# google-deepmind/meltingpot

Measured on NVIDIA B200. Metric: env_steps_per_sec, higher is better.
Workload: dtype u8

## Files before the change

### include/mp_engine.h

```cpp
#ifndef MP_ENGINE_H_
#define MP_ENGINE_H_

#include <stddef.h>
#include <stdint.h>

#ifdef __cplusplus
extern "C" {
#endif

typedef struct mp_engine* mp_handle;

enum {
  MP_OK = 0,
  MP_E_INVALID = -1,
  MP_E_UNSUPPORTED = -2,
  MP_E_CUDA = -3,
  MP_E_NO_DEVICE = -4
};

enum {
  MP_FLAG_RENDER_WORLD = 1u << 0,
  MP_FLAG_RENDER_PLAYERS = 1u << 1,
  MP_FLAG_DEFAULT = 3u,
  MP_FLAG_DEBUG_NO_COMPOSE = 1u << 4,
  MP_FLAG_DEBUG_NO_STORE = 1u << 5,
  MP_FLAG_DEBUG_REUSE_RECORDS = 1u << 6,
  MP_FLAG_DEBUG_NO_FENCE = 1u << 7,
  MP_FLAG_DEBUG_TOP_SPRITE_ONLY = 1u << 8,
  MP_FLAG_DEBUG_PLAIN_LANE_MAP = 1u << 9,
  MP_FLAG_DEBUG_SCATTER_LANE_MAP = 1u << 10
};

typedef struct mp_buffers {
  int32_t num_envs, num_players;
  int32_t rgb_h, rgb_w;
  int32_t world_h, world_w;
  int32_t num_actions;
  int32_t num_scalar_obs;
  uint8_t* rgb;
  uint8_t* world_rgb;
  double* reward;
  double* discount;
  int64_t* step_type;
  double* scalar_obs;
  int32_t* avatar_state;
  uint16_t* grid;
  int32_t grid_layers, grid_cells, grid_cells_padded;
  double* timestep_packed;
  int32_t* events;
  int32_t* event_count;
  int32_t max_events;
  void* scalar_block;
  uint64_t scalar_block_bytes;
  double* gathered;
  int32_t gathered_world;
  uint8_t* gathered_rgb;
  uint8_t* gathered_world_rgb;
  uint64_t gathered_obs_slot_bytes;
} mp_buffers;

int mp_create(const void* blob, size_t blob_bytes, int num_envs, int device, uint64_t seed,
              uint64_t env_index_base, uint32_t flags, mp_handle* out);

int mp_destroy(mp_handle h);

int mp_set_flags(mp_handle h, uint32_t flags);

int mp_reset(mp_handle h, const uint8_t* env_mask, void* stream);

int mp_step(mp_handle h, const int32_t* actions, void* stream);

int mp_step_state(mp_handle h, const int32_t* actions, void* stream);
int mp_render(mp_handle h, void* stream);

int mp_get_buffers(mp_handle h, mp_buffers* out);

typedef struct mp_host_outputs {
  uint8_t* rgb;
  uint8_t* world_rgb;
  double* reward;
  double* discount;
  int64_t* step_type;
  double* scalar_obs;
  void* scalar_block;
  int32_t* events;
  int32_t* event_count;
} mp_host_outputs;
int mp_step_host(mp_handle h, const int32_t* actions_host, const mp_host_outputs* out, void* stream);
int mp_reset_host(mp_handle h, const mp_host_outputs* out, void* stream);

int mp_step_host_async(mp_handle h, const int32_t* actions_host, const mp_host_outputs* out, int slot, void* stream);
int mp_wait(mp_handle h, int slot);

int mp_exchange_create(mp_handle h, int rank, int world, void** block, uint64_t* block_bytes);
int mp_ipc_export(const void* device_ptr, void* handle64, uint64_t* offset);
int mp_ipc_open(int device, const void* handle64, uint64_t offset, void** device_ptr);
int mp_enable_peer_access(int device, int peer_device);
int mp_exchange_connect(mp_handle h, void* const* peer_blocks);
int mp_exchange_wait(mp_handle h, void* stream);
int mp_exchange_slot(mp_handle h, int* slot, uint64_t* step);

int mp_gather_obs_create(mp_handle h, int rank, int world, void** block, uint64_t* block_bytes);
int mp_gather_obs_connect(mp_handle h, void* const* peer_blocks);
int mp_gather_obs_enable(mp_handle h, int on);
int mp_gather_obs_wait(mp_handle h, void* stream);
int mp_gather_obs_slot(mp_handle h, int* slot, uint64_t* step);

int mp_launch_count(mp_handle h, uint64_t* out);

int mp_algorithmic_bytes(mp_handle h, uint64_t* per_env_step, uint64_t* render_per_env_step);

int mp_state_size(mp_handle h, uint64_t* bytes);
int mp_state_save(mp_handle h, void* host_dst, void* stream);
int mp_state_load(mp_handle h, const void* host_src, uint64_t nbytes, void* stream);

int mp_debug_render_plan(mp_handle h, int32_t out[8]);

int mp_debug_render_tables(mp_handle h, int32_t* n_total, uint8_t* pair, uint8_t* flags);

int mp_debug_observations(mp_handle h, int32_t* position, int32_t* orientation, int32_t* layer, int32_t* zap_matrix, void* stream);

int mp_debug_lane_map(int n_rows, int n_cells, int pitch_slots, int iters, int scattered, uint32_t out[32]);

const char* mp_last_error(void);
const char* mp_version(void);

#ifdef __cplusplus
}
#endif
#endif
```

### meltingpot_b200/csrc/common.cuh

```cuda
#pragma once

#include <cuda_runtime.h>
#include <stdint.h>

#define MP_MAX_PLAYERS 16
#define MP_MAX_LAYERS 16
#define MP_MAX_BEAM_CELLS 32
#define MP_FULL 0xffffffffu
#define MP_MAX_PEERS 8

enum { ENV_STEP = 0, ENV_EPISODE = 1, ENV_DONE = 2, ENV_DIRT = 3, ENV_CLEANED = 4, ENV_ATE = 5, ENV_BEAM = 6, ENV_COLS = 8 };
enum { AV_X = 0, AV_Y = 1, AV_ORIENT = 2, AV_ALIVE = 3 };
enum { TM_ZAP = 0, TM_BEAM2 = 1, TM_FRAME = 2 };
enum { RS_SCENE = 0, RS_AVATAR = 1, RS_OBJECT = 2, RS_AVATAR_RESET = 3, RS_OBJECT_RESET = 4, RS_CHOICE = 5 };
enum { SCENE_DRAW_DIRT = 0, SCENE_DRAW_EPISODE_END = 1 };

struct BeamGeom {
  int n;
  int depth;
  int8_t lat[MP_MAX_BEAM_CELLS];
  int8_t fwd[MP_MAX_BEAM_CELLS];
  int8_t parent[MP_MAX_BEAM_CELLS];
};

struct Tables {
  int W, H, cells, cells_pad, L, P, topology, max_frames;
  int view_l, view_r, view_f, view_b, n_sprites, oob_sprite, oov_sprite, n_actions, n_scalar;
  int scalar_obs[4];
  int avatar_layer, n_spawn;
  int avatar_sprite[MP_MAX_PLAYERS];
  int zap_cooldown, zap_respawn, zap_remove, zap_layer, zap_sprite, zap_hit;
  double zap_penalty, zap_reward;
  BeamGeom zap_geom;
  int nA, nD, nW, nA_pad, nD_pad, nW_pad;
  int apple_layer, apple_sprite, dirt_layer, dirt_sprite, water_layer, n_anim, anim_frames, anim_random;
  int water_sprite[8];
  int clean_cooldown, clean_layer, clean_sprite, clean_hit;
  BeamGeom clean_geom;
  int dirt_delay, end_min_frames, end_interval, taste_role, dirt_count0;
  double grow_rate, grow_depletion, grow_restoration, eat_reward, dirt_prob, end_prob, taste_amount;
  int wait_layer, wait_sprite, grass_layer, grass_sprite, dess_sprite, ch_n_wait, ch_n_probs;
  double ch_probs[4];
  int n_spawn_init[2];
  int avatar_init_group[MP_MAX_PLAYERS];
  const int32_t* spawn_init_cell[2];
  const int32_t* ch_apple;
  int nR, nR_pad, res_layer, unclaimed_sprite, tex_layer, tex_sprite, ind_layer, dmg_layer, dmg_sprite, mark_layer;
  int mark_initial_level, mark_recovery, mark_n_levels, mark_inc[3], mark_remove[3], mark_freeze[3], mark_sprite[3];
  double mark_src_reward[3], mark_tgt_reward[3];
  int claim_wait, brush_layer, claim_layer, res_health0, res_reward_delay, res_repair_delay, tr_taste_role;
  double res_reward, res_rate, res_repair_prob, tr_taste_amount, tr_taste_mult;
  int claimed_sprite[MP_MAX_PLAYERS], dry_sprite[MP_MAX_PLAYERS], brush_sprite[MP_MAX_PLAYERS], claimbeam_sprite[MP_MAX_PLAYERS];
  BeamGeom claim_geom, brush_geom;
  const int32_t* tr_res;
  const int16_t* res_of_cell;
  const uint8_t* wall;
  int n_choice;
  const int32_t* choice_n;
  const int32_t* spawn_cond;
  const int32_t* tr_res_cond;
  const int32_t* ch_nbr;
  const uint16_t* init_grid;
  const int32_t* action_table;
  const int32_t* apple;
  const int32_t* dirt;
  const int32_t* water;
  const int32_t* spawn_cell;
  const uint8_t* solid;
  const uint8_t* cell_flags;
  const int16_t* apple_of_cell;
  const int16_t* dirt_of_cell;
  const uint8_t* atlas;
  const int16_t* sprite_map;
  const uint8_t* sprite_opaque;
  const uint8_t* sprite_pair;
  int coin_sprite[2];
  int coin_type[2];
  double coin_reward[2][4];
  double coin_rate;
  int coin_terminate, coin_terminate_n;
  int ore_sprite[4];
  int mine_window, mine_length;
  double mine_rate[2];
  double mine_reward[2], extract_reward[2];
};

struct State {
  int B;
  uint64_t seed;
  uint16_t* grid;
  int32_t* avatar;
  int32_t* av_timer;
  uint8_t* apple;
  uint8_t* dirt;
  uint8_t* water;
  uint8_t* apple_count;
  uint8_t* fam_u8;
  uint16_t* fam_u16;
  int32_t* av_extra;
  int fam_u8_stride, fam_u16_stride;
  int32_t* env;
  double* reward;
  double* discount;
  int64_t* step_type;
  double* scalar_obs;
  double* packed;
  uint8_t* rgb;
  uint8_t* world_rgb;
  int32_t* events;
  int32_t* n_events;
  int max_events;
  int x_world, x_rank;
  unsigned long long x_step;
  double* x_gathered[MP_MAX_PEERS];
  unsigned long long* x_flags[MP_MAX_PEERS];
  int x_raise;
  int g_world;
  unsigned long long g_step;
  uint8_t* g_rgb[MP_MAX_PEERS];
  uint8_t* g_wrgb[MP_MAX_PEERS];
  const unsigned long long* g_flags;
};

#define MP_MIN_EVENTS 64
enum { EV_ZAP = 1, EV_EDIBLE_CONSUMED = 2, EV_PLAYER_CLEANED = 3, EV_CLAIMED_RESOURCE = 4, EV_DESTROYED_RESOURCE = 5,
       EV_SANCTIONING = 6, EV_REMOVAL = 7, EV_COIN_CONSUMED = 8 ,
       EV_MINING = 9 , EV_EXTRACTION = 10 ,
       EV_EXTRACTION_PAIR = 11  };

__device__ __forceinline__ int* event_counter() {
  __shared__ int s_event_count[4];
  return &s_event_count[(threadIdx.x >> 5) & 3];
}
__device__ __forceinline__ void event_begin(int lane) {
  if (lane == 0) *event_counter() = 0;
  __syncwarp();
}
__device__ __forceinline__ void emit_event(const State& S, int b, int type, int a0, int a1) {
  const int i = atomicAdd(event_counter(), 1);
  if (i < S.max_events) {
    int32_t* e = S.events + ((size_t)b * S.max_events + i) * 3;
    e[0] = type; e[1] = a0; e[2] = a1;
  }
}
__device__ __forceinline__ void event_end(const State& S, int b, int lane) {
  __syncwarp();
  if (lane == 0) S.n_events[b] = *event_counter();
}

__device__ __forceinline__ uint4 philox4x32_10(uint32_t c0, uint32_t c1, uint32_t c2, uint32_t c3, uint32_t k0, uint32_t k1) {
#pragma unroll
  for (int r = 0; r < 10; ++r) {
    uint32_t h0 = __umulhi(0xD2511F53u, c0), l0 = 0xD2511F53u * c0;
    uint32_t h1 = __umulhi(0xCD9E8D57u, c2), l1 = 0xCD9E8D57u * c2;
    uint32_t n0 = h1 ^ c1 ^ k0, n2 = h0 ^ c3 ^ k1;
    c0 = n0; c1 = l1; c2 = n2; c3 = l0;
    k0 += 0x9E3779B9u; k1 += 0xBB67AE85u;
  }
  return make_uint4(c0, c1, c2, c3);
}

__device__ __forceinline__ double u01(uint32_t a, uint32_t b) {
  return ((double)(a >> 5) * 67108864.0 + (double)(b >> 6)) / 9007199254740992.0;
}
__device__ __forceinline__ uint32_t pick(uint32_t w, uint32_t n) { return __umulhi(w, n); }

__device__ __forceinline__ bool choice_present(const Tables& T, int group, uint32_t mask, int episode, uint32_t k0, uint32_t k1) {
  if (group < 0) return true;
  const uint4 w = philox4x32_10(0u, (uint32_t)episode, (uint32_t)group, RS_CHOICE, k0, k1);
  return (mask >> pick(w.x, (uint32_t)T.choice_n[group])) & 1u;
}

__device__ __forceinline__ int dir_dx(int d) { return (d == 1) - (d == 3); }
__device__ __forceinline__ int dir_dy(int d) { return (d == 2) - (d == 0); }
__device__ __forceinline__ uint16_t cell_value(int sprite, int orient) { return (uint16_t)(1 + sprite * 4 + (orient & 3)); }

__device__ __forceinline__ bool wrap_or_reject(const Tables& T, int& x, int& y) {
  if (T.topology == 1) {
    x += x < 0 ? T.W : (x >= T.W ? -T.W : 0);
    y += y < 0 ? T.H : (y >= T.H ? -T.H : 0);
    return true;
  }
  return x >= 0 && x < T.W && y >= 0 && y < T.H;
}

__device__ __forceinline__ void exchange_push(const Tables& T, const State& S) {
  if (S.x_world == 0) return;
  const int lane = threadIdx.x & 31, warp = threadIdx.x >> 5, n_warps = (int)blockDim.x >> 5;
  if (blockIdx.x == 0 && threadIdx.x < S.x_world)
    asm volatile("st.relaxed.sys.global.u64 [%0], %1;" ::"l"(S.x_flags[threadIdx.x] + MP_MAX_PEERS + S.x_rank), "l"(S.x_step) : "memory");
  if (lane < S.x_world && S.x_step > 1ull) {
    const volatile unsigned long long* f = S.x_flags[S.x_rank] + MP_MAX_PEERS + lane;
    while (*f + 1ull < S.x_step) __nanosleep(100);
  }
  __syncwarp();
  const int n = T.P + 2;
  const size_t base = ((size_t)(S.x_step & 1ull) * S.x_world + (size_t)S.x_rank) * S.B;
  for (int b = (int)blockIdx.x + warp * (int)gridDim.x; b < S.B; b += n_warps * (int)gridDim.x) {
    if (lane < n) {
      const double v = S.packed[(size_t)b * n + lane];
      for (int r = 0; r < S.x_world; ++r) S.x_gathered[r][(base + b) * n + lane] = v;
    }
  }
}

__global__ void __launch_bounds__(256) k_exchange_push(Tables T, State S) {
  asm volatile("griddepcontrol.wait;" ::: "memory");
  exchange_push(T, S);
}

__global__ void __launch_bounds__(32) k_exchange_wait(State S, unsigned long long step) {
  const int lane = threadIdx.x;
  if (lane < S.x_world) {
    asm volatile("st.relaxed.sys.global.u64 [%0], %1;" ::"l"(S.x_flags[lane] + S.x_rank), "l"(step) : "memory");
    const unsigned long long* mine = S.x_flags[S.x_rank] + lane;
    unsigned long long v;
    do {
      asm volatile("ld.acquire.sys.global.u64 %0, [%1];" : "=l"(v) : "l"(mine) : "memory");
      if (v < step) __nanosleep(200);
    } while (v < step);
  }
}

__global__ void __launch_bounds__(32) k_flag_wait(const unsigned long long* flags, int world, unsigned long long step) {
  const int lane = threadIdx.x;
  if (lane < world) {
    unsigned long long v;
    do {
      asm volatile("ld.acquire.sys.global.u64 %0, [%1];" : "=l"(v) : "l"(flags + lane) : "memory");
      if (v < step) __nanosleep(200);
    } while (v < step);
  }
}

__global__ void __launch_bounds__(32) k_gather_raise(unsigned long long* const* flags, int world, int rank, unsigned long long step) {
  if (threadIdx.x < world) {
    __threadfence_system();
    asm volatile("st.release.sys.global.u64 [%0], %1;" ::"l"(flags[threadIdx.x] + rank), "l"(step) : "memory");
  }
}
```

### meltingpot_b200/csrc/engine.cu

```cuda
#include <cuda_runtime.h>

#include <algorithm>
#include <cstdarg>
#include <cstdio>
#include <cstring>
#include <string>
#include <vector>

#include "../../include/mp_engine.h"
#include "../../include/mpb_format.h"
#include "common.cuh"
#include "render.cuh"
#include "step_clean_up.cuh"
#include "step_commons.cuh"
#include "step_territory.cuh"
#include "step_coins.cuh"
#include "step_mining.cuh"

namespace {

thread_local std::string g_error;

int fail(int code, const char* fmt, ...) {
  char buf[512];
  va_list ap;
  va_start(ap, fmt);
  vsnprintf(buf, sizeof buf, fmt, ap);
  va_end(ap);
  g_error = buf;
  return code;
}

#define CUDA_TRY(expr)                                                                          \
  do {                                                                                          \
    cudaError_t e_ = (expr);                                                                    \
    if (e_ != cudaSuccess) return fail(MP_E_CUDA, "%s failed: %s", #expr, cudaGetErrorString(e_)); \
  } while (0)

template <typename T>
struct Section {
  const T* data = nullptr;
  std::vector<uint32_t> shape;
  size_t count = 0;
};

template <typename T>
bool get_section(const void* blob, size_t n, const char* name, int dtype, Section<T>* out) {
  const MpbSection* s = mpb_find(blob, n, name);
  if (!s || (int)s->dtype != dtype) return false;
  out->data = static_cast<const T*>(mpb_data(blob, s));
  out->shape.assign(s->shape, s->shape + s->ndim);
  out->count = s->nbytes / sizeof(T);
  return true;
}

int round_up(int v, int m) { return (v + m - 1) / m * m; }

constexpr int kRenderSmemLimit = 227 * 1024 - 2560;
constexpr int kMaxAtlasSprites = 96;
#define MP_MAX_DEVICES 64
#define MP_EXCHANGE_HEADER 256

bool make_beam_geom(int length, int radius, BeamGeom* g) {
  std::vector<int> lat, fwd, parent;
  int prev = -1;
  for (int i = 1; i <= length; ++i) { lat.push_back(0); fwd.push_back(i); parent.push_back(prev); prev = (int)lat.size() - 1; }
  for (int side = 0; side < 2; ++side) {
    int sign = side == 0 ? -1 : 1;
    int prev_lat = -1;
    for (int k = 1; k <= radius; ++k) {
      lat.push_back(sign * k); fwd.push_back(0); parent.push_back(prev_lat);
      prev_lat = (int)lat.size() - 1;
      int pf = prev_lat;
      for (int i = 1; i <= length - k; ++i) { lat.push_back(sign * k); fwd.push_back(i); parent.push_back(pf); pf = (int)lat.size() - 1; }
    }
  }
  if (lat.size() > MP_MAX_BEAM_CELLS) return false;
  g->n = (int)lat.size();
  g->depth = length + radius;
  for (int i = 0; i < g->n; ++i) { g->lat[i] = (int8_t)lat[i]; g->fwd[i] = (int8_t)fwd[i]; g->parent[i] = (int8_t)parent[i]; }
  return true;
}

bool make_lane_map(int n_rows, int n_cells, int pitch_slots, int iters, uint32_t out[32]) {
  const int cap = 16 / n_rows, nH = 2 * iters;
  struct Edge { int u, v, cell, col; };
  std::vector<Edge> edges;
  int cnt[16] = {};
  for (int j = 0; j < n_rows; ++j)
    for (int c = 0; c < n_cells; ++c) {
      const int r = (pitch_slots * j + 3 * c) & 15;
      edges.push_back({j * cap + c % cap, r, c, -1});
      if (++cnt[r] > nH) return false;
    }
  if (n_cells > cap * nH || iters * 6 > 32) return false;
  const int nL = n_rows * cap;
  std::vector<int> colL((size_t)nL * nH, -1), colR((size_t)16 * nH, -1);
  auto free_col = [&](const std::vector<int>& tab, int v) { for (int a = 0; a < nH; ++a) if (tab[(size_t)v * nH + a] < 0) return a; return -1; };
  for (int ei = 0; ei < (int)edges.size(); ++ei) {
    Edge& e = edges[ei];
    const int a = free_col(colL, e.u), b = free_col(colR, e.v);
    if (a < 0 || b < 0) return false;
    if (a != b) {
      std::vector<int> path;
      int cur = e.v, want = a; bool right = true;
      for (;;) {
        const int pe = right ? colR[(size_t)cur * nH + want] : colL[(size_t)cur * nH + want];
        if (pe < 0) break;
        path.push_back(pe);
        cur = right ? edges[pe].u : edges[pe].v;
        right = !right;
        want = want == a ? b : a;
      }
      for (int pe : path) { colL[(size_t)edges[pe].u * nH + edges[pe].col] = -1; colR[(size_t)edges[pe].v * nH + edges[pe].col] = -1; }
      for (int pe : path) { edges[pe].col = edges[pe].col == a ? b : a; colL[(size_t)edges[pe].u * nH + edges[pe].col] = pe; colR[(size_t)edges[pe].v * nH + edges[pe].col] = pe; }
    }
    e.col = a;
    colL[(size_t)e.u * nH + a] = ei; colR[(size_t)e.v * nH + a] = ei;
  }
  for (int l = 0; l < 32; ++l) { out[l] = 0; for (int i = 0; i < iters; ++i) out[l] |= 63u << (6 * i); }
  for (const Edge& e : edges) {
    const int j = e.u / cap, sub = e.u % cap, it = e.col / 2, half = e.col % 2;
    const int lane = 16 * half + sub * n_rows + j;
    out[lane] = (out[lane] & ~(63u << (6 * it))) | ((uint32_t)e.cell << (6 * it));
  }
  return true;
}

int make_lane_map_cells(int n_rows, int n_cells, int pitch_slots, int iters, uint32_t out[32]) {
  const int G = 32 / n_rows, n_slots = G * iters, per_half = 16 / n_rows;
  std::vector<int> slot(n_slots, -1);
  for (int c = 0; c < n_cells && c < n_slots; ++c) slot[c] = c;
  auto cost = [&]() {
    int total = 0;
    for (int it = 0; it < iters; ++it)
      for (int h = 0; h < 2; ++h) {
        int cnt[16] = {}, mx = 0;
        for (int g = h * per_half; g < (h + 1) * per_half; ++g) {
          const int c = slot[it * G + g];
          if (c < 0) continue;
          for (int j = 0; j < n_rows; ++j) mx = std::max(mx, ++cnt[(pitch_slots * j + 3 * c) & 15]);
        }
        total += mx > 1 ? mx - 1 : 0;
      }
    return total;
  };
  int best = cost();
  for (bool improved = true; improved && best > 0;) {
    improved = false;
    int bi = -1, bj = -1, bc = best;
    for (int i = 0; i < n_slots; ++i)
      for (int j = i + 1; j < n_slots; ++j) {
        if (slot[i] == slot[j]) continue;
        std::swap(slot[i], slot[j]);
        const int c = cost();
        if (c < bc) { bc = c; bi = i; bj = j; }
        std::swap(slot[i], slot[j]);
      }
    if (bi >= 0) { std::swap(slot[bi], slot[bj]); best = bc; improved = true; }
  }
  for (int l = 0; l < 32; ++l) {
    out[l] = 0;
    for (int it = 0; it < 5; ++it) {
      const int c = it < iters ? slot[it * G + l / n_rows] : -1;
      out[l] |= (uint32_t)(c < 0 ? 63 : c) << (6 * it);
    }
  }
  return best;
}

}

struct mp_engine {
  int device = 0;
  int B = 0;
  uint32_t flags = MP_FLAG_DEFAULT;
  int family = 0;
  int n_total = 0;
  Tables T{};
  State S{};
  RenderPlan R{};
  mp_buffers buffers{};
  std::vector<void*> allocs;
  int32_t* d_actions = nullptr;
  uint8_t* scalar_block = nullptr;
  size_t scalar_block_bytes = 0;
  struct AsyncSlot { uint8_t* rgb = nullptr; uint8_t* world_rgb = nullptr; int32_t* actions = nullptr; uint8_t* scalars = nullptr;
                     cudaEvent_t computed = nullptr, copied = nullptr; };
  AsyncSlot slot[2];
  cudaStream_t copy_stream = nullptr;
  bool async_ready = false;
  uint8_t* x_block = nullptr;
  uint64_t x_block_bytes = 0;
  unsigned long long x_seq = 0;
  bool x_pending_raise = false;
  int32_t* d_avatar_dbg = nullptr;
  uint64_t launches = 0;
  int sm_count = 0;
  size_t step_smem = 0;
  void (*render_fn)(Tables, State, RenderPlan, uint32_t) = nullptr;
  void (*render_gather_fn)(Tables, State, RenderPlan, uint32_t) = nullptr;
  uint8_t* g_block = nullptr;
  uint64_t g_block_bytes = 0, g_slot_bytes = 0, g_world_off = 0;
  uint8_t* g_peer[MP_MAX_PEERS] = {};
  unsigned long long** d_g_flag_ptrs = nullptr;
  int g_world = 0, g_rank = 0;
  unsigned long long g_seq = 0;
  uint64_t algo_bytes = 0, render_bytes = 0;
  std::vector<uint8_t> host_pair, host_sflags;
  int black_sprite = -1;
  std::vector<std::pair<void*, size_t>> state_spans;
  uint64_t state_bytes = 0;
  int lane_map_players = 0, lane_map_world = 0;
  uint64_t blob_hash = 0;

  template <typename T>
  int upload(const std::vector<T>& host, const T** out) {
    void* p = nullptr;
    size_t bytes = std::max<size_t>(host.size() * sizeof(T), 16);
    CUDA_TRY(cudaMalloc(&p, bytes));
    allocs.push_back(p);
    CUDA_TRY(cudaMemset(p, 0, bytes));
    if (!host.empty()) CUDA_TRY(cudaMemcpy(p, host.data(), host.size() * sizeof(T), cudaMemcpyHostToDevice));
    *out = static_cast<const T*>(p);
    return MP_OK;
  }
  template <typename T>
  int alloc(size_t count, T** out) {
    void* p = nullptr;
    size_t bytes = std::max<size_t>(count * sizeof(T), 16);
    CUDA_TRY(cudaMalloc(&p, bytes));
    allocs.push_back(p);
    CUDA_TRY(cudaMemset(p, 0, bytes));
    *out = static_cast<T*>(p);
    return MP_OK;
  }
};

namespace {

int build_tables(mp_engine* E, const void* blob, size_t n) {
  Section<int32_t> meta, states, kinds, comps, objects, hits, action_table, sprite_map, scalar_obs, av_table;
  Section<double> comps_f;
  Section<uint8_t> atlas, sprite_opaque, cell_flags;
  Section<uint16_t> init_grid;
  if (!get_section(blob, n, "meta", MPB_I32, &meta) || meta.count < MPB_META_COUNT) return fail(MP_E_INVALID, "blob: missing/invalid 'meta' (not an MPB%u blob?)", MPB_VERSION);
#define NEED(sec, dt) if (!get_section(blob, n, #sec, dt, &sec)) return fail(MP_E_INVALID, "blob: missing section '%s'", #sec);
  NEED(states, MPB_I32) NEED(kinds, MPB_I32) NEED(comps, MPB_I32) NEED(comps_f, MPB_F64) NEED(objects, MPB_I32) NEED(hits, MPB_I32)
  NEED(action_table, MPB_I32) NEED(sprite_map, MPB_I32) NEED(scalar_obs, MPB_I32) NEED(av_table, MPB_I32)
  NEED(atlas, MPB_U8) NEED(sprite_opaque, MPB_U8) NEED(cell_flags, MPB_U8) NEED(init_grid, MPB_U16)
  const int32_t* m = meta.data;
  Tables& T = E->T;
  E->family = m[MPB_META_FAMILY];
  T.W = m[MPB_META_W]; T.H = m[MPB_META_H]; T.cells = T.W * T.H; T.cells_pad = round_up(T.cells, 8);
  T.L = m[MPB_META_L]; T.P = m[MPB_META_P]; T.topology = m[MPB_META_TOPOLOGY]; T.max_frames = m[MPB_META_MAX_FRAMES];
  T.view_l = m[MPB_META_VIEW_LEFT]; T.view_r = m[MPB_META_VIEW_RIGHT]; T.view_f = m[MPB_META_VIEW_FORWARD]; T.view_b = m[MPB_META_VIEW_BACKWARD];
  T.n_sprites = m[MPB_META_N_SPRITES]; T.oob_sprite = m[MPB_META_OOB_SPRITE]; T.oov_sprite = m[MPB_META_OOV_SPRITE];
  T.n_actions = m[MPB_META_N_ACTIONS]; T.n_scalar = m[MPB_META_N_SCALAR_OBS];
  if (m[MPB_META_SPRITE_SIZE] != 8) return fail(MP_E_UNSUPPORTED, "spriteSize %d (kernels are written for 8x8 sprites)", m[MPB_META_SPRITE_SIZE]);
  if (T.P < 1 || T.P > MP_MAX_PLAYERS) return fail(MP_E_UNSUPPORTED, "%d players (max %d)", T.P, MP_MAX_PLAYERS);
  if (T.L > MP_MAX_LAYERS) return fail(MP_E_UNSUPPORTED, "%d layers (max %d)", T.L, MP_MAX_LAYERS);
  if (T.n_sprites > kMaxAtlasSprites) return fail(MP_E_UNSUPPORTED, "%d sprites (max %d)", T.n_sprites, kMaxAtlasSprites);
  if (T.n_scalar > 4) return fail(MP_E_UNSUPPORTED, "%d scalar observations (max 4)", T.n_scalar);
  if (T.n_actions < 1) return fail(MP_E_INVALID, "blob has no action table (compile with the substrate config)");
  if (T.cells >= 4096) return fail(MP_E_UNSUPPORTED, "map of %d cells (max 4095)", T.cells);
  if (T.topology == 1 && (T.view_l + T.view_r + 1 > T.W || T.view_f + T.view_b + 1 > T.H || T.view_l + T.view_r + 1 > T.H || T.view_f + T.view_b + 1 > T.W))
    return fail(MP_E_UNSUPPORTED, "TORUS map smaller than the view window");
  for (int k = 0; k < T.n_scalar; ++k) T.scalar_obs[k] = scalar_obs.data[k];
  if (E->family != MPB_FAMILY_CLEAN_UP && E->family != MPB_FAMILY_COMMONS_HARVEST && E->family != MPB_FAMILY_TERRITORY && E->family != MPB_FAMILY_COINS && E->family != MPB_FAMILY_COOP_MINING) return fail(MP_E_UNSUPPORTED, "substrate family %d has no CUDA state-transition kernel yet", E->family);

  T.avatar_layer = av_table.data[2];
  int init_groups[2] = {-1, -1};
  int respawn_group = -1;
  for (int p = 0; p < T.P; ++p) {
    const int32_t* a = av_table.data + p * 8;
    T.avatar_sprite[p] = a[1];
    if (a[2] != T.avatar_layer) return fail(MP_E_UNSUPPORTED, "per-avatar layers");
    const int post = a[4] >= 0 ? a[4] : a[3];
    if (respawn_group >= 0 && post != respawn_group) return fail(MP_E_UNSUPPORTED, "per-avatar respawn groups");
    respawn_group = post;
    int g = -1;
    for (int k = 0; k < 2; ++k) if (init_groups[k] == a[3]) g = k;
    if (g < 0) { for (int k = 0; k < 2 && g < 0; ++k) if (init_groups[k] < 0) { init_groups[k] = a[3]; g = k; } }
    if (g < 0) return fail(MP_E_UNSUPPORTED, "more than two initial spawn groups");
    T.avatar_init_group[p] = g;
  }
  char name[64];
  auto load_group = [&](int gid, std::vector<int32_t>* out) -> int {
    snprintf(name, sizeof name, "spawn_cells_%d", gid);
    Section<int32_t> sec;
    if (!get_section(blob, n, name, MPB_I32, &sec)) return fail(MP_E_INVALID, "blob: missing section '%s'", name);
    out->assign(sec.data, sec.data + sec.count);
    return MP_OK;
  };
  std::vector<int32_t> v_spawn, v_init[2];
  int rc0;
  if ((rc0 = load_group(respawn_group, &v_spawn))) return rc0;
  T.n_spawn = (int)v_spawn.size();
  for (int k = 0; k < 2; ++k) {
    T.n_spawn_init[k] = 0;
    if (init_groups[k] < 0) continue;
    if ((rc0 = load_group(init_groups[k], &v_init[k]))) return rc0;
    T.n_spawn_init[k] = (int)v_init[k].size();
    int users = 0;
    for (int p = 0; p < T.P; ++p) users += T.avatar_init_group[p] == k;
    if (T.n_spawn_init[k] < users || T.n_spawn_init[k] > 64) return fail(MP_E_UNSUPPORTED, "%d spawn points for %d avatars (need n..64)", T.n_spawn_init[k], users);
  }
  if (T.n_spawn < 1) return fail(MP_E_INVALID, "empty respawn group");

  int rc;
  std::vector<int32_t> v_apple, v_dirt, v_water;
  std::vector<std::vector<int>> hint_stacks;
  T.nA = T.nD = T.nW = 0; T.nR = 0; T.nR_pad = 16;
  T.n_anim = 1; T.anim_frames = 1; T.clean_layer = 0;
  auto zapper = [&](const int32_t* ip) -> int {
    T.zap_cooldown = ip[12]; T.zap_respawn = ip[15]; T.zap_remove = ip[16];
    T.zap_layer = ip[21]; T.zap_sprite = ip[22];
    T.zap_hit = 0;
    for (int h = 0; h < (int)hits.count / 2; ++h) if (hits.data[h * 2] == T.zap_layer) T.zap_hit = h;
    if (T.zap_cooldown <= 0) return fail(MP_E_UNSUPPORTED, "non-positive zap cooldown");
    if (!make_beam_geom(ip[13], ip[14], &T.zap_geom)) return fail(MP_E_UNSUPPORTED, "beam footprint larger than %d cells", MP_MAX_BEAM_CELLS);
    T.end_min_frames = ip[26]; T.end_interval = ip[27];
    if (T.end_interval < 1) return fail(MP_E_INVALID, "episode interval < 1");
    return MP_OK;
  };
  if (E->family == MPB_FAMILY_CLEAN_UP) {
    Section<int32_t> cu_ip, cu_apple, cu_dirt, cu_water, cu_water_sprites;
    Section<double> cu_dp;
    NEED(cu_ip, MPB_I32) NEED(cu_dp, MPB_F64) NEED(cu_apple, MPB_I32) NEED(cu_dirt, MPB_I32) NEED(cu_water, MPB_I32) NEED(cu_water_sprites, MPB_I32)
    const int32_t* ip = cu_ip.data; const double* dp = cu_dp.data;
    T.nA = ip[0]; T.nD = ip[1]; T.nW = ip[2];
    T.apple_layer = ip[3]; T.apple_sprite = ip[4]; T.dirt_layer = ip[5]; T.dirt_sprite = ip[6];
    T.water_layer = ip[8]; T.n_anim = ip[9]; T.anim_frames = ip[10]; T.anim_random = ip[11];
    if (T.n_anim < 1 || T.n_anim > 8 || T.anim_frames < 1) return fail(MP_E_UNSUPPORTED, "animation with %d states / %d frames", T.n_anim, T.anim_frames);
    for (int i = 0; i < T.n_anim; ++i) T.water_sprite[i] = cu_water_sprites.data[i];
    if ((rc = zapper(ip))) return rc;
    T.clean_cooldown = ip[18]; T.clean_layer = ip[23]; T.clean_sprite = ip[24];
    T.clean_hit = 1;
    for (int h = 0; h < (int)hits.count / 2; ++h) if (hits.data[h * 2] == T.clean_layer) T.clean_hit = h;
    if (T.clean_cooldown < 0) return fail(MP_E_UNSUPPORTED, "negative clean cooldown");
    if (!make_beam_geom(ip[19], ip[20], &T.clean_geom)) return fail(MP_E_UNSUPPORTED, "beam footprint larger than %d cells", MP_MAX_BEAM_CELLS);
    T.dirt_delay = ip[25]; T.taste_role = ip[28];
    if (T.taste_role != 0) return fail(MP_E_UNSUPPORTED, "Taste roles other than 'free'");
    T.grow_rate = dp[0]; T.grow_depletion = dp[1]; T.grow_restoration = dp[2]; T.eat_reward = dp[3];
    T.zap_penalty = dp[4]; T.zap_reward = dp[5]; T.dirt_prob = dp[6]; T.end_prob = dp[7]; T.taste_amount = dp[8];
    v_apple.assign(cu_apple.data, cu_apple.data + cu_apple.count);
    v_dirt.assign(cu_dirt.data, cu_dirt.data + cu_dirt.count);
    v_water.assign(cu_water.data, cu_water.data + cu_water.count);
    if ((rc = E->upload(v_apple, &T.apple)) || (rc = E->upload(v_dirt, &T.dirt)) || (rc = E->upload(v_water, &T.water))) return rc;
  } else if (E->family == MPB_FAMILY_COMMONS_HARVEST) {
    Section<int32_t> ch_ip, ch_apple, ch_nbr;
    Section<double> ch_dp;
    NEED(ch_ip, MPB_I32) NEED(ch_dp, MPB_F64) NEED(ch_apple, MPB_I32) NEED(ch_nbr, MPB_I32)
    const int32_t* ip = ch_ip.data; const double* dp = ch_dp.data;
    T.nA = ip[0]; T.apple_layer = ip[1]; T.apple_sprite = ip[2]; T.wait_layer = ip[3]; T.wait_sprite = ip[4];
    T.ch_n_wait = ip[5]; T.ch_n_probs = ip[6]; T.grass_layer = ip[7]; T.grass_sprite = ip[8]; T.dess_sprite = ip[9];
    if (T.ch_n_wait < 1 || T.ch_n_wait > 29 || T.ch_n_probs < 1 || T.ch_n_probs > 4) return fail(MP_E_UNSUPPORTED, "DensityRegrow with %d wait states / %d probabilities", T.ch_n_wait, T.ch_n_probs);
    if (T.nA > 2048) return fail(MP_E_UNSUPPORTED, "%d apples (max 2048)", T.nA);
    if ((rc = zapper(ip))) return rc;
    for (int i = 0; i < 4; ++i) T.ch_probs[i] = dp[i];
    T.eat_reward = dp[4]; T.zap_penalty = dp[5]; T.zap_reward = dp[6]; T.end_prob = dp[7];
    v_apple.assign(ch_apple.data, ch_apple.data + ch_apple.count);
    std::vector<int32_t> v_nbr(ch_nbr.data, ch_nbr.data + ch_nbr.count);
    if ((rc = E->upload(v_apple, &T.ch_apple)) || (rc = E->upload(v_nbr, &T.ch_nbr))) return rc;
  }
  else if (E->family == MPB_FAMILY_COINS) {
    Section<int32_t> co_ip, co_coin;
    Section<double> co_dp;
    NEED(co_ip, MPB_I32) NEED(co_dp, MPB_F64) NEED(co_coin, MPB_I32)
    const int32_t* ip = co_ip.data; const double* dp = co_dp.data;
    if (T.P != 2) return fail(MP_E_UNSUPPORTED, "coins needs exactly two players (got %d)", T.P);
    T.nA = ip[0]; T.apple_layer = ip[1]; T.coin_sprite[0] = ip[2]; T.coin_sprite[1] = ip[3];
    T.coin_terminate = ip[4]; T.coin_terminate_n = ip[5]; T.end_min_frames = ip[6]; T.end_interval = ip[7];
    T.coin_type[0] = ip[8]; T.coin_type[1] = ip[9];
    if (T.nA > 2048) return fail(MP_E_UNSUPPORTED, "%d coins (max 2048)", T.nA);
    if (T.end_interval < 1) return fail(MP_E_INVALID, "episode interval < 1");
    T.coin_rate = dp[0]; T.end_prob = dp[1];
    for (int p = 0; p < 2; ++p) for (int k = 0; k < 4; ++k) T.coin_reward[p][k] = dp[4 + p * 4 + k];
    T.zap_layer = 0; T.zap_cooldown = 1;
    v_apple.resize((size_t)T.nA * 4);
    for (int k = 0; k < T.nA; ++k) { v_apple[k * 4] = co_coin.data[k * 2]; v_apple[k * 4 + 1] = co_coin.data[k * 2 + 1]; v_apple[k * 4 + 2] = 0; v_apple[k * 4 + 3] = -1; }
    if ((rc = E->upload(v_apple, &T.ch_apple))) return rc;
  }
  else if (E->family == MPB_FAMILY_COOP_MINING) {
    Section<int32_t> cm_ip, cm_ore;
    Section<double> cm_dp;
    NEED(cm_ip, MPB_I32) NEED(cm_dp, MPB_F64) NEED(cm_ore, MPB_I32)
    const int32_t* ip = cm_ip.data; const double* dp = cm_dp.data;
    T.nA = ip[0]; T.apple_layer = ip[1];
    for (int i = 0; i < 4; ++i) T.ore_sprite[i] = ip[2 + i];
    T.mine_window = ip[6]; T.zap_cooldown = ip[7]; T.mine_length = ip[8]; T.zap_layer = ip[9]; T.zap_sprite = ip[10];
    T.end_min_frames = ip[11]; T.end_interval = ip[12]; T.zap_hit = ip[13];
    if (T.P > 8) return fail(MP_E_UNSUPPORTED, "coop_mining with %d players (max 8: miners are kept as a bit mask)", T.P);
    if (T.nA > 2048) return fail(MP_E_UNSUPPORTED, "%d ores (max 2048)", T.nA);
    if (T.zap_cooldown < 1 || T.mine_window < 1 || T.mine_window > 255 || T.mine_length < 1) return fail(MP_E_UNSUPPORTED, "MineBeam / Ore parameters out of range");
    if (T.end_interval < 1) return fail(MP_E_INVALID, "episode interval < 1");
    if (T.zap_hit < 0 || T.zap_hit > 7) return fail(MP_E_UNSUPPORTED, "mine hit id %d", T.zap_hit);
    T.mine_rate[0] = dp[0]; T.mine_rate[1] = dp[1]; T.end_prob = dp[2];
    T.mine_reward[0] = dp[4]; T.mine_reward[1] = dp[5]; T.extract_reward[0] = dp[6]; T.extract_reward[1] = dp[7];
    v_apple.resize((size_t)T.nA * 4);
    for (int k = 0; k < T.nA; ++k) { v_apple[k * 4] = cm_ore.data[k * 2]; v_apple[k * 4 + 1] = cm_ore.data[k * 2 + 1]; v_apple[k * 4 + 2] = 0; v_apple[k * 4 + 3] = -1; }
    if ((rc = E->upload(v_apple, &T.ch_apple))) return rc;
  }
  else {
    Section<int32_t> tr_ip, tr_res, tr_player_sprites;
    Section<double> tr_dp;
    Section<uint8_t> tr_wall;
    NEED(tr_ip, MPB_I32) NEED(tr_dp, MPB_F64) NEED(tr_res, MPB_I32) NEED(tr_player_sprites, MPB_I32) NEED(tr_wall, MPB_U8)
    const int32_t* ip = tr_ip.data; const double* dp = tr_dp.data;
    T.nR = ip[0]; T.nR_pad = round_up(std::max(T.nR, 64), 16);
    T.res_layer = ip[1]; T.unclaimed_sprite = ip[2]; T.tex_layer = ip[3]; T.tex_sprite = ip[4]; T.ind_layer = ip[5];
    T.dmg_layer = ip[6]; T.dmg_sprite = ip[7]; T.mark_layer = ip[8]; T.mark_initial_level = ip[9]; T.mark_recovery = ip[10]; T.mark_n_levels = ip[11];
    if (T.res_layer != T.avatar_layer) return fail(MP_E_UNSUPPORTED, "territory: resources and avatars must share a layer");
    if (T.mark_n_levels < 1 || T.mark_n_levels > 3) return fail(MP_E_UNSUPPORTED, "%d marking levels (1..3)", T.mark_n_levels);
    if ((rc = zapper(ip))) return rc;
    if (T.zap_respawn <= T.max_frames) return fail(MP_E_UNSUPPORTED, "territory kernel assumes avatars never respawn (framesTillRespawn %d)", T.zap_respawn);
    if (!make_beam_geom(ip[18], ip[19], &T.claim_geom) || !make_beam_geom(1, 0, &T.brush_geom)) return fail(MP_E_UNSUPPORTED, "beam footprint larger than %d cells", MP_MAX_BEAM_CELLS);
    T.claim_wait = ip[20]; T.brush_layer = ip[23]; T.claim_layer = ip[24];
    if (T.claim_layer != T.dmg_layer) return fail(MP_E_UNSUPPORTED, "territory: claim beam layer must be the damage indicator layer");
    T.res_health0 = ip[28]; T.res_reward_delay = ip[29]; T.res_repair_delay = ip[30]; T.tr_taste_role = ip[31];
    if (T.tr_taste_role != 0) return fail(MP_E_UNSUPPORTED, "territory Taste roles other than 'none'");
    if (T.res_health0 < 1 || T.res_health0 > 200) return fail(MP_E_UNSUPPORTED, "resource health %d", T.res_health0);
    for (int l = 0; l < T.mark_n_levels; ++l) {
      T.mark_inc[l] = ip[32 + 4 * l]; T.mark_remove[l] = ip[33 + 4 * l]; T.mark_freeze[l] = ip[34 + 4 * l]; T.mark_sprite[l] = ip[35 + 4 * l];
      T.mark_src_reward[l] = dp[8 + 2 * l]; T.mark_tgt_reward[l] = dp[9 + 2 * l];
    }
    T.res_reward = dp[0]; T.res_rate = dp[1]; T.res_repair_prob = dp[2]; T.zap_penalty = dp[3]; T.zap_reward = dp[4]; T.end_prob = dp[5];
    T.tr_taste_amount = dp[6]; T.tr_taste_mult = dp[7];
    for (int p = 0; p < T.P; ++p) {
      const int32_t* ps = tr_player_sprites.data + p * 4;
      T.claimed_sprite[p] = ps[0]; T.dry_sprite[p] = ps[1]; T.brush_sprite[p] = ps[2]; T.claimbeam_sprite[p] = ps[3];
    }
    for (int p = 0; p < T.P; ++p) {
      hint_stacks.push_back({T.tex_sprite, T.claimed_sprite[p]});
      hint_stacks.push_back({T.tex_sprite, T.claimed_sprite[p], T.dry_sprite[p]});
    }
    std::vector<int32_t> v_res(tr_res.data, tr_res.data + tr_res.count);
    std::vector<int16_t> res_of(T.cells_pad, -1);
    for (int k = 0; k < T.nR; ++k) res_of[v_res[k * 3 + 1]] = (int16_t)k;
    std::vector<uint8_t> wall(T.cells_pad, 0);
    memcpy(wall.data(), tr_wall.data, std::min<size_t>(tr_wall.count, T.cells));
    if ((rc = E->upload(v_res, &T.tr_res)) || (rc = E->upload(res_of, &T.res_of_cell)) || (rc = E->upload(wall, &T.wall))) return rc;
    Section<int32_t> tr_res_cond;
    if (get_section(blob, n, "tr_res_cond", MPB_I32, &tr_res_cond)) {
      if ((int)tr_res_cond.count != T.nR * 2) return fail(MP_E_INVALID, "blob: tr_res_cond has %zu values for %d resources", tr_res_cond.count, T.nR);
      std::vector<int32_t> v(tr_res_cond.data, tr_res_cond.data + tr_res_cond.count);
      if ((rc = E->upload(v, &T.tr_res_cond))) return rc;
    }
  }
#undef NEED
  {
    Section<int32_t> choice_groups, obj_choice, spawn_cond;
    if (get_section(blob, n, "choice_groups", MPB_I32, &choice_groups)) {
      if (E->family != MPB_FAMILY_TERRITORY) return fail(MP_E_UNSUPPORTED, "per-env 'choice' prefabs are implemented for the territory family only (compile with a build_seed)");
      T.n_choice = (int)choice_groups.count;
      for (size_t g = 0; g < choice_groups.count; ++g) if (choice_groups.data[g] < 1 || choice_groups.data[g] > 31) return fail(MP_E_INVALID, "blob: choice group with %d options", choice_groups.data[g]);
      std::vector<int32_t> v(choice_groups.data, choice_groups.data + choice_groups.count);
      if ((rc = E->upload(v, &T.choice_n))) return rc;
      snprintf(name, sizeof name, "spawn_cond_%d", respawn_group);
      if (get_section(blob, n, name, MPB_I32, &spawn_cond)) {
        if ((int)spawn_cond.count != T.n_spawn * 2 || T.n_spawn > 64) return fail(MP_E_UNSUPPORTED, "%d conditional spawn candidates (max 64)", T.n_spawn);
        std::vector<int32_t> c(spawn_cond.data, spawn_cond.data + spawn_cond.count);
        if ((rc = E->upload(c, &T.spawn_cond))) return rc;
      }
    }
  }
  T.nA_pad = round_up(std::max(T.nA, 1), 16); T.nD_pad = round_up(std::max(std::max(T.nD, T.nA), 1), 16); T.nW_pad = round_up(std::max(T.nW, 1), 16);

  std::vector<uint16_t> grid0((size_t)T.L * T.cells_pad, 0);
  for (int l = 0; l < T.L; ++l) memcpy(&grid0[(size_t)l * T.cells_pad], init_grid.data + (size_t)l * T.cells, T.cells * sizeof(uint16_t));
  if ((rc = E->upload(grid0, &T.init_grid))) return rc;
  std::vector<int32_t> act(action_table.data, action_table.data + action_table.count);
  if ((rc = E->upload(act, &T.action_table))) return rc;
  if ((rc = E->upload(v_spawn, &T.spawn_cell))) return rc;
  for (int k = 0; k < 2; ++k) {
    if (v_init[k].empty()) { T.spawn_init_cell[k] = T.spawn_cell; continue; }
    if ((rc = E->upload(v_init[k], &T.spawn_init_cell[k]))) return rc;
  }
  std::vector<uint8_t> solid(T.cells_pad, 0), flags(T.cells_pad, 0);
  for (int o = 0; o < m[MPB_META_N_OBJECTS]; ++o) {
    const int32_t* od = objects.data + o * MPB_OBJ_COLS;
    const int32_t* kd = kinds.data + od[MPB_OBJ_KIND] * MPB_KIND_COLS;
    if (kd[MPB_KIND_IS_AVATAR]) continue;
    const int32_t* st = states.data + (kd[MPB_KIND_STATE0] + od[MPB_OBJ_STATE]) * MPB_STATE_COLS;
    if (st[MPB_STATE_LAYER] == T.avatar_layer) solid[od[MPB_OBJ_Y] * T.W + od[MPB_OBJ_X]] = 255;
  }
  memcpy(flags.data(), cell_flags.data, std::min<size_t>(cell_flags.count, T.cells));
  if ((rc = E->upload(solid, &T.solid)) || (rc = E->upload(flags, &T.cell_flags))) return rc;
  std::vector<int16_t> apple_of(T.cells_pad, -1), dirt_of(T.cells_pad, -1);
  T.dirt_count0 = 0;
  const int apple_cols = E->family == MPB_FAMILY_CLEAN_UP ? 3 : 4;
  for (int k = 0; k < T.nA; ++k) apple_of[v_apple[k * apple_cols + 1]] = (int16_t)k;
  for (int j = 0; j < T.nD; ++j) { dirt_of[v_dirt[j * 3 + 1]] = (int16_t)j; T.dirt_count0 += v_dirt[j * 3 + 2]; }
  if ((rc = E->upload(apple_of, &T.apple_of_cell)) || (rc = E->upload(dirt_of, &T.dirt_of_cell))) return rc;

  if (atlas.count != (size_t)T.n_sprites * 1024) return fail(MP_E_INVALID, "atlas has %zu bytes, expected %d", atlas.count, T.n_sprites * 1024);
  std::vector<uint8_t> img(atlas.data, atlas.data + atlas.count);
  std::vector<uint8_t> opq(sprite_opaque.data, sprite_opaque.data + T.n_sprites);
  std::vector<uint8_t> remapped(T.n_sprites, 0);
  for (int v = 0; v <= T.P; ++v)
    for (int s = 0; s < T.n_sprites; ++s)
      if (sprite_map.data[(size_t)v * T.n_sprites + s] != s) { remapped[s] = 1; opq[s] = 0; }
  std::vector<std::vector<int>> pair_of;
  auto n_now = [&]() { return (int)opq.size(); };
  pair_of.assign(T.n_sprites, std::vector<int>());
  auto blend = [](uint8_t* d, const uint8_t* s_) {
    unsigned a = s_[3];
    if (a == 255) { d[0] = s_[0]; d[1] = s_[1]; d[2] = s_[2]; }
    else if (a) for (int c = 0; c < 3; ++c) d[c] = (uint8_t)((s_[c] * a + d[c] * (255u - a)) / 255u);
  };
  auto merged_id = [&](int base, int top) -> int {
    if ((int)pair_of[base].size() <= top) pair_of[base].resize(top + 1, 0);
    if (pair_of[base][top]) return pair_of[base][top];
    if (n_now() >= kMaxAtlasSprites) return 0;
    int id = n_now();
    img.resize((size_t)(id + 1) * 1024);
    for (int f = 0; f < 4; ++f)
      for (int px = 0; px < 64; ++px) {
        uint8_t* d = &img[(size_t)id * 1024 + f * 256 + px * 4];
        memcpy(d, &img[(size_t)base * 1024 + f * 256 + px * 4], 4);
        blend(d, &img[(size_t)top * 1024 + f * 256 + px * 4]);
        d[3] = 255;
      }
    opq.push_back(1); remapped.push_back(0);
    pair_of.push_back(std::vector<int>());
    pair_of[base][top] = id;
    return id;
  };
  {
    struct Opt { std::vector<int> sprites; bool absent = false; int orient = -1; bool bad = false; };
    std::vector<Opt> opts((size_t)T.cells * T.L);
    std::vector<uint8_t> has_obj((size_t)T.cells * T.L, 0);
    for (int o = 0; o < m[MPB_META_N_OBJECTS]; ++o) {
      const int32_t* od = objects.data + o * MPB_OBJ_COLS;
      const int32_t* kd = kinds.data + od[MPB_OBJ_KIND] * MPB_KIND_COLS;
      if (kd[MPB_KIND_IS_AVATAR]) continue;
      const int cell = od[MPB_OBJ_Y] * T.W + od[MPB_OBJ_X];
      const int ns = kd[MPB_KIND_NSTATES];
      for (int si = 0; si < ns; ++si) {
        const int32_t* st = states.data + (kd[MPB_KIND_STATE0] + si) * MPB_STATE_COLS;
        const int l = st[MPB_STATE_LAYER], sp = st[MPB_STATE_SPRITE];
        if (l < 0 || sp < 0) continue;
        Opt& op = opts[(size_t)cell * T.L + l];
        if (std::find(op.sprites.begin(), op.sprites.end(), sp) == op.sprites.end()) op.sprites.push_back(sp);
        if (op.orient >= 0 && op.orient != od[MPB_OBJ_ORIENT]) op.bad = true;
        op.orient = od[MPB_OBJ_ORIENT];
        for (int sj = 0; sj < ns; ++sj) {
          const int32_t* s2 = states.data + (kd[MPB_KIND_STATE0] + sj) * MPB_STATE_COLS;
          if (s2[MPB_STATE_LAYER] != l || s2[MPB_STATE_SPRITE] < 0) op.absent = true;
        }
      }
    }
    for (const auto& hs : hint_stacks) {
      if (hs.empty() || !opq[hs[0]]) continue;
      int cur = hs[0];
      for (size_t q = 1; q < hs.size() && cur; ++q) { if (remapped[hs[q]] || remapped[cur]) break; cur = merged_id(cur, hs[q]); }
    }
    std::vector<int> stack_s, stack_o;
    for (int pass = 0; pass < 2; ++pass)
    for (int cell = 0; cell < T.cells; ++cell) {
      size_t combos = 1;
      bool bad = false;
      for (int l = 0; l < T.L; ++l) {
        const Opt& op = opts[(size_t)cell * T.L + l];
        bad |= op.bad;
        combos *= std::max<size_t>(1, op.sprites.size() + ((op.absent || op.sprites.empty()) ? 1 : 0));
        if (combos > 4096) { bad = true; break; }
      }
      if (bad) continue;
      std::vector<int> idx(T.L, 0);
      for (size_t k = 0; k < combos; ++k) {
        stack_s.clear(); stack_o.clear();
        bool is_initial = true;
        for (int l = 0; l < T.L; ++l) {
          const Opt& op = opts[(size_t)cell * T.L + l];
          const int i = idx[l];
          const int init_v = init_grid.data[(size_t)l * T.cells + cell];
          const int init_sprite = init_v ? (init_v - 1) >> 2 : -1;
          if (i < (int)op.sprites.size()) { stack_s.push_back(op.sprites[i]); stack_o.push_back(op.orient); is_initial &= op.sprites[i] == init_sprite; }
          else is_initial &= init_sprite < 0;
        }
        if ((pass == 0) != is_initial) stack_s.clear();
        int j = -1;
        for (int q = (int)stack_s.size() - 1; q >= 0; --q) if (opq[stack_s[q]]) { j = q; break; }
        if (j >= 0) {
          int cur = stack_s[j];
          for (int q = j + 1; q < (int)stack_s.size(); ++q) {
            const int t = stack_s[q];
            if (stack_o[q] != stack_o[j] || remapped[t] || remapped[cur]) break;
            cur = merged_id(cur, t);
            if (!cur) break;
          }
        }
        for (int l = 0; l < T.L; ++l) {
          const Opt& op = opts[(size_t)cell * T.L + l];
          const int radix = (int)std::max<size_t>(1, op.sprites.size() + ((op.absent || op.sprites.empty()) ? 1 : 0));
          if (++idx[l] < radix) break;
          idx[l] = 0;
        }
      }
    }
  }
  const int n_total = n_now();
  E->n_total = n_total;
  std::vector<uint8_t> at((size_t)n_total * 1024);
  for (int s = 0; s < n_total * 4; ++s)
    for (int row = 0; row < 8; ++row)
      for (int half = 0; half < 2; ++half)
        memcpy(&at[(size_t)s * 256 + half * 128 + row * 16], &img[(size_t)s * 256 + row * 32 + half * 16], 16);
  if ((rc = E->upload(at, &T.atlas))) return rc;
  std::vector<int16_t> smap((size_t)(T.P + 1) * n_total);
  for (int v = 0; v <= T.P; ++v)
    for (int s = 0; s < n_total; ++s)
      smap[(size_t)v * n_total + s] = (int16_t)(s < T.n_sprites ? sprite_map.data[(size_t)v * T.n_sprites + s] : s);
  std::vector<uint8_t> pair((size_t)n_total * n_total, 0);
  for (int b = 0; b < n_total; ++b)
    for (int t = 0; t < (int)pair_of[b].size(); ++t) pair[(size_t)b * n_total + t] = (uint8_t)pair_of[b][t];
  std::vector<uint8_t> sflags(n_total);
  std::vector<uint8_t> binary_alpha(n_total, 1);
  for (int i = 0; i < n_total; ++i)
    for (int px = 0; px < 256; ++px) { const uint8_t a = img[(size_t)i * 1024 + px * 4 + 3]; if (a != 0 && a != 255) { binary_alpha[i] = 0; break; } }
  for (int i = 0; i < n_total; ++i) {
    bool bin = true;
    for (int v = 0; v <= T.P; ++v) bin = bin && binary_alpha[smap[(size_t)v * n_total + i]];
    bool invisible = true;
    for (int v = 0; v <= T.P && invisible; ++v) {
      const int t = smap[(size_t)v * n_total + i];
      for (int px = 0; px < 256 && invisible; ++px) invisible = img[(size_t)t * 1024 + px * 4 + 3] == 0;
    }
    sflags[i] = (uint8_t)((opq[i] ? 1 : 0) | (remapped[i] ? 2 : 0) | (bin ? 4 : 0) | (invisible ? 8 : 0));
  }
  E->host_pair = pair; E->host_sflags = sflags;
  E->black_sprite = -1;
  for (int i = 0; i < n_total && E->black_sprite < 0; ++i) {
    if (!opq[i] || remapped[i]) continue;
    bool black = true;
    for (int px = 0; px < 256 && black; ++px) { const uint8_t* q = &img[(size_t)i * 1024 + px * 4]; black = q[0] == 0 && q[1] == 0 && q[2] == 0; }
    if (black) E->black_sprite = i;
  }
  if ((rc = E->upload(smap, &T.sprite_map)) || (rc = E->upload(sflags, &T.sprite_opaque)) || (rc = E->upload(pair, &T.sprite_pair))) return rc;
  return MP_OK;
}

int build_plan(mp_engine* E) {
  const Tables& T = E->T;
  RenderPlan& R = E->R;
  R.view_w = T.view_l + T.view_r + 1; R.view_h = T.view_f + T.view_b + 1;
  R.player_bytes = R.view_w * R.view_h * 192;
  R.world_bytes = T.H * T.W * 192;
  R.grid_bytes = T.L * T.cells_pad * 2;
  R.n_total = E->n_total;
  R.atlas_bytes = R.n_total * 1024;
  R.rec_stride = (int)round_up(T.L + 1, 4);
  R.magic_view_h = (65536u + R.view_h - 1) / R.view_h;
  int off = 128;
  R.off_atlas = off; off += round_up(R.atlas_bytes, 128);
  R.off_pair = off; off += round_up(R.n_total * R.n_total, 128);
  R.off_map = off; off += round_up((T.P + 1) * R.n_total * 2, 128);
  R.off_team0 = off;
  R.smem_bytes = 1 << 30;
  double best = -1.0;
  for (int teams = 2; teams <= RENDER_MAX_TEAMS; ++teams)
    for (int warps = TEAM_THREADS / 32; warps >= 4; --warps) {
      if (teams * warps > RENDER_MAX_THREADS / 32) continue;
      for (int wlog = 2; wlog >= 1; --wlog) {
        const int stage = RENDER_SLOTS * round_up(std::max(R.view_w * 192, T.W * 24 * (1 << wlog)), 128);
        const int team_bytes = round_up(R.grid_bytes, 128) + round_up(T.cells * R.rec_stride * 2, 128) + warps * stage;
        const int total = R.off_team0 + teams * team_bytes;
        if (total > kRenderSmemLimit) continue;
        const double items = T.P * R.view_h + (8 >> wlog) * T.H, per_warp = items / warps;
        const double score = teams * warps * per_warp / (per_warp + 3.0) * (wlog == 2 ? 1.0 : 0.85) * (1.0 - 0.01 * teams);
        if (score > best + 1e-9) {
          best = score;
          R.n_teams = teams; R.team_threads = warps * 32; R.wstrip_log2 = wlog; R.stage_bytes = stage;
          R.toff_grid = 0; R.toff_rec = round_up(R.grid_bytes, 128);
          R.toff_stage = R.toff_rec + round_up(T.cells * R.rec_stride * 2, 128);
          R.team_stride = team_bytes; R.smem_bytes = total;
        }
      }
    }
  if (R.smem_bytes > kRenderSmemLimit) return fail(MP_E_UNSUPPORTED, "render kernel needs %d B of shared memory (> 227 KB)", R.smem_bytes);
  return MP_OK;
}

__global__ void k_debug_obs(Tables T, State S, int32_t* position, int32_t* orientation, int32_t* layer, int32_t* zap, int view_w, int view_h) {
  const int b = blockIdx.x, P = T.P;
  const int32_t* av = S.avatar + (size_t)b * P * 4;
  for (int p = threadIdx.x; p < P; p += blockDim.x) {
    if (position) { position[((size_t)b * P + p) * 2] = av[p * 4 + AV_X]; position[((size_t)b * P + p) * 2 + 1] = av[p * 4 + AV_Y]; }
    if (orientation) orientation[(size_t)b * P + p] = av[p * 4 + AV_ORIENT];
  }
  if (layer) {
    const int per_player = view_h * view_w * T.L;
    const uint16_t* grid = S.grid + (size_t)b * T.L * T.cells_pad;
    for (int i = threadIdx.x; i < P * per_player; i += blockDim.x) {
      const int p = i / per_player, r = i - p * per_player, l = r % T.L, c = r / T.L, vx = c % view_w, vy = c / view_w;
      int x = av[p * 4 + AV_X] - T.view_l + vx, y = av[p * 4 + AV_Y] - T.view_f + vy;
      int32_t v = -1;
      if (wrap_or_reject(T, x, y)) { const uint16_t g = grid[(size_t)l * T.cells_pad + y * T.W + x]; v = g ? ((g - 1) >> 2) + 1 : 0; }
      layer[(size_t)b * P * per_player + i] = v;
    }
  }
  if (zap) {
    for (int i = threadIdx.x; i < P * P; i += blockDim.x) zap[(size_t)b * P * P + i] = 0;
    __syncthreads();
    const int n = min(S.n_events[b], S.max_events);
    for (int i = threadIdx.x; i < n; i += blockDim.x) {
      const int32_t* e = S.events + ((size_t)b * S.max_events + i) * 3;
      if (e[0] == EV_ZAP && e[1] >= 1 && e[1] <= P && e[2] >= 1 && e[2] <= P) atomicAdd(&zap[(size_t)b * P * P + (e[1] - 1) * P + (e[2] - 1)], 1);
    }
  }
}

int raise_flags(mp_engine* E, cudaStream_t st) {
  E->x_pending_raise = false;
  k_exchange_push<<<std::min(E->sm_count, (E->B + 7) / 8), 256, 0, st>>>(E->T, E->S);
  ++E->launches;
  CUDA_TRY(cudaGetLastError());
  return MP_OK;
}

int launch_state(mp_engine* E, const int32_t* actions, const uint8_t* mask, int mode, cudaStream_t st, bool render_follows = true) {
  const int blocks = (E->B + 3) / 4;
  if (E->S.x_world) E->S.x_step = ++E->x_seq;
  void (*fn)(Tables, State, const int32_t*, const uint8_t*, int) =
      E->family == MPB_FAMILY_CLEAN_UP ? k_step_clean_up : E->family == MPB_FAMILY_COMMONS_HARVEST ? k_step_commons :
      E->family == MPB_FAMILY_COINS ? k_step_coins : E->family == MPB_FAMILY_COOP_MINING ? k_step_mining : k_step_territory;
  cudaLaunchConfig_t cfg = {};
  cfg.gridDim = dim3(blocks); cfg.blockDim = dim3(128); cfg.dynamicSmemBytes = E->step_smem * 4 + (E->family == MPB_FAMILY_CLEAN_UP ? clean_up_table_bytes(E->T) : E->family == MPB_FAMILY_TERRITORY ? territory_table_bytes(E->T) : 0); cfg.stream = st;
  cudaLaunchAttribute attr[1];
  attr[0].id = cudaLaunchAttributeProgrammaticStreamSerialization;
  attr[0].val.programmaticStreamSerializationAllowed = 1;
  cfg.attrs = attr; cfg.numAttrs = 1;
  CUDA_TRY(cudaLaunchKernelEx(&cfg, fn, E->T, E->S, actions, mask, mode));
  if (E->S.x_world) {
    E->x_pending_raise = true;
    if (!render_follows) { ++E->launches; return raise_flags(E, st); }
  }
  ++E->launches;
  CUDA_TRY(cudaGetLastError());
  return MP_OK;
}

int launch_render(mp_engine* E, cudaStream_t st) {
  if (!(E->flags & (MP_FLAG_RENDER_WORLD | MP_FLAG_RENDER_PLAYERS))) return E->x_pending_raise ? raise_flags(E, st) : MP_OK;
  E->S.x_raise = E->x_pending_raise ? 1 : 0;
  E->x_pending_raise = false;
  const int blocks = std::min(E->B, E->sm_count);
  RenderPlan R = E->R;
  const Tables& T = E->T;
  R.n_player_items = (E->flags & MP_FLAG_RENDER_PLAYERS) ? T.P * R.view_h : 0;
  R.n_items = R.n_player_items + ((E->flags & MP_FLAG_RENDER_WORLD) ? (8 >> R.wstrip_log2) * T.H : 0);
  R.prow_bytes = R.view_w * 24; R.wrow_bytes = T.W * 24;
  R.pitem_bytes = R.prow_bytes * 8; R.witem_bytes = R.wrow_bytes << R.wstrip_log2;
  R.h_oob = 0x8000 | (T.oob_sprite * 4); R.h_oov = 0x8000 | (T.oov_sprite * 4);
  R.h_empty = E->black_sprite >= 0 ? (0x8000 | (E->black_sprite * 4)) : 0;
  cudaLaunchConfig_t cfg = {};
  cfg.gridDim = dim3(blocks); cfg.blockDim = dim3(R.n_teams * R.team_threads); cfg.dynamicSmemBytes = R.smem_bytes; cfg.stream = st;
  cudaLaunchAttribute attr[1];
  attr[0].id = cudaLaunchAttributeProgrammaticStreamSerialization;
  attr[0].val.programmaticStreamSerializationAllowed = 1;
  cfg.attrs = attr; cfg.numAttrs = 1;
  const bool gather = E->g_world > 0 && E->S.g_world > 0;
  if (gather) {
    E->S.g_step = ++E->g_seq;
    const size_t slot = (size_t)(E->g_seq & 1ull) * E->g_slot_bytes;
    for (int r = 0; r < E->g_world; ++r) {
      uint8_t* base = E->g_peer[r] + MP_EXCHANGE_HEADER + slot;
      E->S.g_rgb[r] = base + (size_t)E->g_rank * E->B * T.P * R.player_bytes;
      E->S.g_wrgb[r] = base + E->g_world_off + (size_t)E->g_rank * E->B * R.world_bytes;
    }
  }
  CUDA_TRY(cudaLaunchKernelEx(&cfg, gather ? E->render_gather_fn : E->render_fn, E->T, E->S, R, E->flags));
  if (gather) {
    k_gather_raise<<<1, 32, 0, st>>>(E->d_g_flag_ptrs, E->g_world, E->g_rank, E->g_seq);
    ++E->launches;
  }
  ++E->launches;
  CUDA_TRY(cudaGetLastError());
  return MP_OK;
}

int copy_out(mp_engine* E, const mp_host_outputs* out, cudaStream_t st) {
  if (!out) return MP_OK;
  const mp_buffers& bf = E->buffers;
  const size_t B = E->B, P = E->T.P;
  if (out->rgb) CUDA_TRY(cudaMemcpyAsync(out->rgb, bf.rgb, B * P * E->R.player_bytes, cudaMemcpyDeviceToHost, st));
  if (out->world_rgb) CUDA_TRY(cudaMemcpyAsync(out->world_rgb, bf.world_rgb, B * E->R.world_bytes, cudaMemcpyDeviceToHost, st));
  if (out->events) CUDA_TRY(cudaMemcpyAsync(out->events, bf.events, B * (size_t)bf.max_events * 3 * sizeof(int32_t), cudaMemcpyDeviceToHost, st));
  if (out->event_count) CUDA_TRY(cudaMemcpyAsync(out->event_count, bf.event_count, B * sizeof(int32_t), cudaMemcpyDeviceToHost, st));
  if (out->scalar_block) {
    CUDA_TRY(cudaMemcpyAsync(out->scalar_block, E->scalar_block, E->scalar_block_bytes, cudaMemcpyDeviceToHost, st));
    return MP_OK;
  }
  if (out->reward) CUDA_TRY(cudaMemcpyAsync(out->reward, bf.reward, B * P * sizeof(double), cudaMemcpyDeviceToHost, st));
  if (out->discount) CUDA_TRY(cudaMemcpyAsync(out->discount, bf.discount, B * sizeof(double), cudaMemcpyDeviceToHost, st));
  if (out->step_type) CUDA_TRY(cudaMemcpyAsync(out->step_type, bf.step_type, B * sizeof(int64_t), cudaMemcpyDeviceToHost, st));
  if (out->scalar_obs && E->T.n_scalar) CUDA_TRY(cudaMemcpyAsync(out->scalar_obs, bf.scalar_obs, (size_t)E->T.n_scalar * B * P * sizeof(double), cudaMemcpyDeviceToHost, st));
  return MP_OK;
}

struct DeviceGuard {
  int prev = -1;
  explicit DeviceGuard(int dev) { cudaGetDevice(&prev); if (prev != dev) cudaSetDevice(dev); else prev = -1; }
  ~DeviceGuard() { if (prev >= 0) cudaSetDevice(prev); }
};

}

extern "C" {

const char* mp_last_error(void) { return g_error.c_str(); }
const char* mp_version(void) { return "meltingpot_b200 engine 0.1 (sm_100a)"; }

int mp_create(const void* blob, size_t blob_bytes, int num_envs, int device, uint64_t seed, uint64_t env_index_base, uint32_t flags, mp_handle* out) {
  if (!blob || !out || num_envs < 1) return fail(MP_E_INVALID, "mp_create: bad arguments");
  int n_dev = 0;
  cudaError_t e = cudaGetDeviceCount(&n_dev);
  if (e != cudaSuccess || n_dev == 0) return fail(MP_E_NO_DEVICE, "no CUDA device available (%s); this engine has no CPU path", cudaGetErrorString(e));
  if (device < 0 || device >= n_dev || device >= MP_MAX_DEVICES) return fail(MP_E_INVALID, "device %d out of range (0..%d)", device, n_dev - 1);
  cudaDeviceProp prop;
  CUDA_TRY(cudaGetDeviceProperties(&prop, device));
  if (prop.major != 10) return fail(MP_E_NO_DEVICE, "device %d is sm_%d%d; kernels are built for sm_100a only", device, prop.major, prop.minor);
  DeviceGuard guard(device);
  mp_engine* E = new mp_engine();
  E->device = device; E->B = num_envs; E->flags = flags; E->sm_count = prop.multiProcessorCount;
  {
    uint64_t hsh = 1469598103934665603ull;
    const uint8_t* bp = static_cast<const uint8_t*>(blob);
    for (size_t i = 0; i < blob_bytes; ++i) { hsh ^= bp[i]; hsh *= 1099511628211ull; }
    E->blob_hash = hsh;
  }
  int rc = build_tables(E, blob, blob_bytes);
  if (rc == MP_OK) rc = build_plan(E);
  if (rc != MP_OK) { mp_destroy(E); return rc; }
  const Tables& T = E->T;
  State& S = E->S;
  S.B = num_envs; S.seed = seed + env_index_base;
  const size_t B = num_envs, P = T.P;
  {
    const int beam_cells = T.zap_geom.n + T.clean_geom.n + T.claim_geom.n + T.brush_geom.n;
    S.max_events = round_up(std::max(MP_MIN_EVENTS, T.P * (3 * beam_cells + 4 + T.P)), 16);
  }
  S.fam_u8_stride = std::max(16, RU_COUNT * T.nR_pad); S.fam_u16_stride = std::max(16, RS_COUNT * T.nR_pad);
  if ((rc = E->alloc(B * T.L * T.cells_pad, &S.grid)) || (rc = E->alloc(B * P * 4, &S.avatar)) || (rc = E->alloc(B * P * 4, &S.av_timer)) ||
      (rc = E->alloc(B * T.nA_pad, &S.apple)) || (rc = E->alloc(B * T.nD_pad, &S.dirt)) || (rc = E->alloc(B * T.nW_pad, &S.water)) || (rc = E->alloc(B * T.nA_pad, &S.apple_count)) || (rc = E->alloc(B * (size_t)S.fam_u8_stride, &S.fam_u8)) || (rc = E->alloc(B * (size_t)S.fam_u16_stride, &S.fam_u16)) || (rc = E->alloc(B * P * 8, &S.av_extra)) || (rc = E->alloc(B * (P + 2), &S.packed)) ||
      (rc = E->alloc(B * ENV_COLS, &S.env)) ||
      (rc = E->alloc((B * P + B + B + std::max<size_t>(1, T.n_scalar) * B * P) * 8, &E->scalar_block)) ||
      (rc = E->alloc(B * P * E->R.player_bytes, &S.rgb)) || (rc = E->alloc(B * (size_t)E->R.world_bytes, &S.world_rgb)) ||
      (rc = E->alloc(B * (size_t)S.max_events * 3, &S.events)) || (rc = E->alloc(B, &S.n_events)) ||
      (rc = E->alloc(B * P, &E->d_actions))) {
    mp_destroy(E);
    return rc;
  }
  {
    E->scalar_block_bytes = (B * P + B + B + std::max<size_t>(1, T.n_scalar) * B * P) * 8;
    S.reward = reinterpret_cast<double*>(E->scalar_block);
    S.discount = S.reward + B * P;
    S.step_type = reinterpret_cast<int64_t*>(S.discount + B);
    S.scalar_obs = reinterpret_cast<double*>(S.step_type + B);
  }
  {
    const size_t ns = std::max<size_t>(1, T.n_scalar);
    auto span = [&](void* p, size_t bytes) { E->state_spans.push_back({p, bytes}); E->state_bytes += bytes; };
    span(S.grid, B * T.L * T.cells_pad * sizeof(*S.grid)); span(S.avatar, B * P * 4 * sizeof(*S.avatar));
    span(S.av_timer, B * P * 4 * sizeof(*S.av_timer)); span(S.apple, B * T.nA_pad * sizeof(*S.apple));
    span(S.dirt, B * T.nD_pad * sizeof(*S.dirt)); span(S.water, B * T.nW_pad * sizeof(*S.water));
    span(S.apple_count, B * T.nA_pad * sizeof(*S.apple_count)); span(S.fam_u8, B * (size_t)S.fam_u8_stride * sizeof(*S.fam_u8));
    span(S.fam_u16, B * (size_t)S.fam_u16_stride * sizeof(*S.fam_u16)); span(S.av_extra, B * P * 8 * sizeof(*S.av_extra));
    span(S.packed, B * (P + 2) * sizeof(*S.packed)); span(S.env, B * ENV_COLS * sizeof(*S.env));
    span(S.reward, B * P * sizeof(*S.reward)); span(S.discount, B * sizeof(*S.discount));
    span(S.step_type, B * sizeof(*S.step_type)); span(S.scalar_obs, ns * B * P * sizeof(*S.scalar_obs));
    span(S.events, B * (size_t)S.max_events * 3 * sizeof(*S.events)); span(S.n_events, B * sizeof(*S.n_events));
  }
  {
    std::vector<int32_t> env0(B * ENV_COLS, 0);
    for (size_t b = 0; b < B; ++b) { env0[b * ENV_COLS + ENV_EPISODE] = -1; env0[b * ENV_COLS + ENV_DONE] = 1; }
    cudaError_t ce = cudaMemcpy(S.env, env0.data(), env0.size() * sizeof(int32_t), cudaMemcpyHostToDevice);
    if (ce != cudaSuccess) { mp_destroy(E); return fail(MP_E_CUDA, "cudaMemcpy(env) failed: %s", cudaGetErrorString(ce)); }
  }
  E->step_smem = E->family == MPB_FAMILY_TERRITORY ? territory_scratch_bytes(T) : warp_scratch_bytes(T);
  {
    const int ncp = (E->R.view_w + 3) / 4, ncw = (T.W + (32 >> E->R.wstrip_log2) - 1) / (32 >> E->R.wstrip_log2);
    if (ncp <= 3 && ncw <= 3) { E->render_fn = k_render<3, 3, false>; E->render_gather_fn = k_render<3, 3, true>; }
    else if (ncp <= 3 && ncw <= 4) { E->render_fn = k_render<3, 4, false>; E->render_gather_fn = k_render<3, 4, true>; }
    else if (ncp <= 3 && ncw <= 5) { E->render_fn = k_render<3, 5, false>; E->render_gather_fn = k_render<3, 5, true>; }
    else if (ncp <= 4 && ncw <= 5) { E->render_fn = k_render<4, 5, false>; E->render_gather_fn = k_render<4, 5, true>; }
    else { mp_destroy(E); return fail(MP_E_UNSUPPORTED, "view of %d cells / map of %d cells wide (max 16 / 40)", E->R.view_w, T.W); }
    const int wrows = 1 << E->R.wstrip_log2;
    if (flags & MP_FLAG_DEBUG_PLAIN_LANE_MAP) {
      for (int l = 0; l < 32; ++l) { E->R.pmap[l] = 0; for (int i = 0; i < 4; ++i) E->R.pmap[l] |= (uint32_t)std::min(63, (l >> 3) + 4 * i) << (6 * i); }
      for (int l = 0; l < 32; ++l) { E->R.wmap[l] = 0; for (int i = 0; i < 5; ++i) E->R.wmap[l] |= (uint32_t)std::min(63, (l >> E->R.wstrip_log2) + (32 >> E->R.wstrip_log2) * i) << (6 * i); }
    } else if ((flags & MP_FLAG_DEBUG_SCATTER_LANE_MAP) && make_lane_map(8, E->R.view_w, 3 * E->R.view_w, ncp, E->R.pmap) &&
               make_lane_map(wrows, T.W, 3 * T.W, ncw, E->R.wmap)) {
      E->lane_map_players = E->lane_map_world = 2;
    } else {
      E->lane_map_players = 1 + 16 * make_lane_map_cells(8, E->R.view_w, 3 * E->R.view_w, ncp, E->R.pmap);
      E->lane_map_world = 1 + 16 * make_lane_map_cells(wrows, T.W, 3 * T.W, ncw, E->R.wmap);
    }
  }
  cudaError_t ce = cudaFuncSetAttribute(E->render_fn, cudaFuncAttributeMaxDynamicSharedMemorySize, kRenderSmemLimit);
  if (ce == cudaSuccess) ce = cudaFuncSetAttribute(E->render_gather_fn, cudaFuncAttributeMaxDynamicSharedMemorySize, kRenderSmemLimit);
  {
    static int step_smem_max[MP_MAX_DEVICES] = {};
    const int need = (int)(E->step_smem * 4 + (E->family == MPB_FAMILY_CLEAN_UP ? clean_up_table_bytes(T) : E->family == MPB_FAMILY_TERRITORY ? territory_table_bytes(T) : 0));
    if (ce == cudaSuccess && need > 48 * 1024 && need > step_smem_max[device]) {
      ce = cudaFuncSetAttribute(k_step_clean_up, cudaFuncAttributeMaxDynamicSharedMemorySize, need);
      if (ce == cudaSuccess) ce = cudaFuncSetAttribute(k_step_commons, cudaFuncAttributeMaxDynamicSharedMemorySize, need);
      if (ce == cudaSuccess) ce = cudaFuncSetAttribute(k_step_territory, cudaFuncAttributeMaxDynamicSharedMemorySize, need);
      if (ce == cudaSuccess) ce = cudaFuncSetAttribute(k_step_coins, cudaFuncAttributeMaxDynamicSharedMemorySize, need);
      if (ce == cudaSuccess) ce = cudaFuncSetAttribute(k_step_mining, cudaFuncAttributeMaxDynamicSharedMemorySize, need);
      if (ce == cudaSuccess) step_smem_max[device] = need;
    }
  }
  if (ce != cudaSuccess) { mp_destroy(E); return fail(MP_E_CUDA, "cudaFuncSetAttribute failed: %s", cudaGetErrorString(ce)); }
  mp_buffers& bf = E->buffers;
  bf.num_envs = num_envs; bf.num_players = T.P; bf.rgb_h = E->R.view_h * 8; bf.rgb_w = E->R.view_w * 8;
  bf.world_h = T.H * 8; bf.world_w = T.W * 8; bf.num_actions = T.n_actions; bf.num_scalar_obs = T.n_scalar;
  bf.rgb = S.rgb; bf.world_rgb = S.world_rgb; bf.reward = S.reward; bf.discount = S.discount; bf.step_type = S.step_type;
  bf.scalar_obs = S.scalar_obs; bf.avatar_state = S.avatar; bf.grid = S.grid; bf.timestep_packed = S.packed;
  bf.grid_layers = T.L; bf.grid_cells = T.cells; bf.grid_cells_padded = T.cells_pad;
  bf.events = S.events; bf.event_count = S.n_events; bf.max_events = S.max_events;
  bf.scalar_block = E->scalar_block; bf.scalar_block_bytes = E->scalar_block_bytes;
  E->render_bytes = (uint64_t)P * E->R.player_bytes + (uint64_t)E->R.world_bytes + (uint64_t)T.L * T.cells * 2;
  E->algo_bytes = (uint64_t)P * E->R.player_bytes + (uint64_t)E->R.world_bytes + 8ull * ((1 + T.n_scalar) * P + 2) + 8ull * P + 2ull * T.L * T.cells * 2;
  *out = E;
  return MP_OK;
}

int mp_destroy(mp_handle h) {
  if (!h) return MP_OK;
  {
    DeviceGuard guard(h->device);
    cudaDeviceSynchronize();
    for (auto& sl : h->slot) { if (sl.computed) cudaEventDestroy(sl.computed); if (sl.copied) cudaEventDestroy(sl.copied); }
    if (h->copy_stream) cudaStreamDestroy(h->copy_stream);
    for (void* p : h->allocs) cudaFree(p);
  }
  delete h;
  return MP_OK;
}

int mp_set_flags(mp_handle h, uint32_t flags) {
  if (!h) return fail(MP_E_INVALID, "null handle");
  h->flags = flags;
  return MP_OK;
}

int mp_reset(mp_handle h, const uint8_t* env_mask, void* stream) {
  if (!h) return fail(MP_E_INVALID, "null handle");
  DeviceGuard guard(h->device);
  int rc = launch_state(h, nullptr, env_mask, 1, (cudaStream_t)stream);
  return rc ? rc : launch_render(h, (cudaStream_t)stream);
}

int mp_step_state(mp_handle h, const int32_t* actions, void* stream) {
  if (!h || !actions) return fail(MP_E_INVALID, "mp_step_state: null handle or actions");
  DeviceGuard guard(h->device);
  return launch_state(h, actions, nullptr, 0, (cudaStream_t)stream, false);
}

int mp_render(mp_handle h, void* stream) {
  if (!h) return fail(MP_E_INVALID, "null handle");
  DeviceGuard guard(h->device);
  return launch_render(h, (cudaStream_t)stream);
}

int mp_step(mp_handle h, const int32_t* actions, void* stream) {
  int rc = mp_step_state(h, actions, stream);
  return rc ? rc : mp_render(h, stream);
}

int mp_get_buffers(mp_handle h, mp_buffers* out) {
  if (!h || !out) return fail(MP_E_INVALID, "null argument");
  *out = h->buffers;
  return MP_OK;
}

int mp_step_host(mp_handle h, const int32_t* actions_host, const mp_host_outputs* out, void* stream) {
  if (!h || !actions_host) return fail(MP_E_INVALID, "mp_step_host: null handle or actions");
  DeviceGuard guard(h->device);
  cudaStream_t st = (cudaStream_t)stream;
  CUDA_TRY(cudaMemcpyAsync(h->d_actions, actions_host, (size_t)h->B * h->T.P * sizeof(int32_t), cudaMemcpyHostToDevice, st));
  int rc = launch_state(h, h->d_actions, nullptr, 0, st);
  if (!rc) rc = launch_render(h, st);
  if (!rc) rc = copy_out(h, out, st);
  if (rc) return rc;
  CUDA_TRY(cudaStreamSynchronize(st));
  return MP_OK;
}

int mp_reset_host(mp_handle h, const mp_host_outputs* out, void* stream) {
  if (!h) return fail(MP_E_INVALID, "null handle");
  DeviceGuard guard(h->device);
  cudaStream_t st = (cudaStream_t)stream;
  int rc = launch_state(h, nullptr, nullptr, 1, st);
  if (!rc) rc = launch_render(h, st);
  if (!rc) rc = copy_out(h, out, st);
  if (rc) return rc;
  CUDA_TRY(cudaStreamSynchronize(st));
  return MP_OK;
}

namespace {
int async_setup(mp_engine* E) {
  if (E->async_ready) return MP_OK;
  const size_t B = E->B, P = E->T.P;
  int rc;
  E->slot[0].rgb = E->S.rgb; E->slot[0].world_rgb = E->S.world_rgb;
  if ((rc = E->alloc(B * P * E->R.player_bytes, &E->slot[1].rgb)) || (rc = E->alloc(B * (size_t)E->R.world_bytes, &E->slot[1].world_rgb))) return rc;
  for (auto& sl : E->slot) {
    if ((rc = E->alloc(B * P, &sl.actions)) || (rc = E->alloc(E->scalar_block_bytes, &sl.scalars))) return rc;
    CUDA_TRY(cudaEventCreateWithFlags(&sl.computed, cudaEventDisableTiming));
    CUDA_TRY(cudaEventCreateWithFlags(&sl.copied, cudaEventDisableTiming));
  }
  CUDA_TRY(cudaStreamCreateWithFlags(&E->copy_stream, cudaStreamNonBlocking));
  E->async_ready = true;
  return MP_OK;
}
}

int mp_step_host_async(mp_handle h, const int32_t* actions_host, const mp_host_outputs* out, int slot, void* stream) {
  if (!h || !actions_host || slot < 0 || slot > 1) return fail(MP_E_INVALID, "mp_step_host_async: null handle / actions or slot outside 0..1");
  DeviceGuard guard(h->device);
  int rc = async_setup(h);
  if (rc) return rc;
  cudaStream_t st = (cudaStream_t)stream;
  mp_engine::AsyncSlot& sl = h->slot[slot];
  CUDA_TRY(cudaStreamWaitEvent(st, sl.copied, 0));
  CUDA_TRY(cudaMemcpyAsync(sl.actions, actions_host, (size_t)h->B * h->T.P * sizeof(int32_t), cudaMemcpyHostToDevice, st));
  if ((rc = launch_state(h, sl.actions, nullptr, 0, st))) return rc;
  uint8_t* rgb0 = h->S.rgb; uint8_t* world0 = h->S.world_rgb;
  h->S.rgb = sl.rgb; h->S.world_rgb = sl.world_rgb;
  rc = launch_render(h, st);
  h->S.rgb = rgb0; h->S.world_rgb = world0;
  if (rc) return rc;
  CUDA_TRY(cudaMemcpyAsync(sl.scalars, h->scalar_block, h->scalar_block_bytes, cudaMemcpyDeviceToDevice, st));
  CUDA_TRY(cudaEventRecord(sl.computed, st));
  CUDA_TRY(cudaStreamWaitEvent(h->copy_stream, sl.computed, 0));
  if (out && (out->events || out->event_count)) return fail(MP_E_INVALID, "mp_step_host_async: events are not staged per slot; read them with mp_step_host");
  if (out) {
    const size_t B = h->B, P = h->T.P;
    cudaStream_t cs = h->copy_stream;
    if (out->rgb) CUDA_TRY(cudaMemcpyAsync(out->rgb, sl.rgb, B * P * h->R.player_bytes, cudaMemcpyDeviceToHost, cs));
    if (out->world_rgb) CUDA_TRY(cudaMemcpyAsync(out->world_rgb, sl.world_rgb, B * h->R.world_bytes, cudaMemcpyDeviceToHost, cs));
    if (out->scalar_block) CUDA_TRY(cudaMemcpyAsync(out->scalar_block, sl.scalars, h->scalar_block_bytes, cudaMemcpyDeviceToHost, cs));
    else {
      const uint8_t* sb = sl.scalars;
      if (out->reward) CUDA_TRY(cudaMemcpyAsync(out->reward, sb, B * P * 8, cudaMemcpyDeviceToHost, cs));
      if (out->discount) CUDA_TRY(cudaMemcpyAsync(out->discount, sb + B * P * 8, B * 8, cudaMemcpyDeviceToHost, cs));
      if (out->step_type) CUDA_TRY(cudaMemcpyAsync(out->step_type, sb + (B * P + B) * 8, B * 8, cudaMemcpyDeviceToHost, cs));
      if (out->scalar_obs && h->T.n_scalar) CUDA_TRY(cudaMemcpyAsync(out->scalar_obs, sb + (B * P + 2 * B) * 8, (size_t)h->T.n_scalar * B * P * 8, cudaMemcpyDeviceToHost, cs));
    }
  }
  CUDA_TRY(cudaEventRecord(sl.copied, h->copy_stream));
  return MP_OK;
}

int mp_wait(mp_handle h, int slot) {
  if (!h || slot < 0 || slot > 1) return fail(MP_E_INVALID, "mp_wait: null handle or slot outside 0..1");
  if (!h->async_ready) return MP_OK;
  DeviceGuard guard(h->device);
  CUDA_TRY(cudaEventSynchronize(h->slot[slot].copied));
  return MP_OK;
}

int mp_exchange_create(mp_handle h, int rank, int world, void** block, uint64_t* block_bytes) {
  if (!h || world < 1 || world > MP_MAX_PEERS || rank < 0 || rank >= world) return fail(MP_E_INVALID, "mp_exchange_create: rank %d / world %d (max %d ranks)", rank, world, MP_MAX_PEERS);
// ... 55 lines not shown
  if (!h || !peer_blocks) return fail(MP_E_INVALID, "mp_exchange_connect: null argument");
  if (!h->x_block) return fail(MP_E_INVALID, "mp_exchange_connect: call mp_exchange_create first");
  const int world = h->buffers.gathered_world;
  if (peer_blocks[h->S.x_rank] != h->x_block) return fail(MP_E_INVALID, "mp_exchange_connect: entry %d must be this rank's own block", h->S.x_rank);
  for (int r = 0; r < world; ++r) {
    if (!peer_blocks[r]) return fail(MP_E_INVALID, "mp_exchange_connect: null pointer for rank %d", r);
    h->S.x_flags[r] = static_cast<unsigned long long*>(peer_blocks[r]);
    h->S.x_gathered[r] = reinterpret_cast<double*>(static_cast<uint8_t*>(peer_blocks[r]) + MP_EXCHANGE_HEADER);
  }
  h->S.x_world = world;
  return MP_OK;
}

int mp_gather_obs_create(mp_handle h, int rank, int world, void** block, uint64_t* block_bytes) {
  if (!h || world < 1 || world > MP_MAX_PEERS || rank < 0 || rank >= world) return fail(MP_E_INVALID, "mp_gather_obs_create: rank %d / world %d (max %d ranks)", rank, world, MP_MAX_PEERS);
  if (h->g_block) return fail(MP_E_INVALID, "mp_gather_obs_create: already created for this handle");
  DeviceGuard guard(h->device);
  const size_t rgb_all = (size_t)world * h->B * h->T.P * h->R.player_bytes, world_all = (size_t)world * h->B * h->R.world_bytes;
  h->g_world_off = rgb_all;
  h->g_slot_bytes = (rgb_all + world_all + 255) / 256 * 256;
  h->g_block_bytes = MP_EXCHANGE_HEADER + 2 * h->g_slot_bytes;
  void* p = nullptr;
  CUDA_TRY(cudaMalloc(&p, h->g_block_bytes));
  h->allocs.push_back(p);
  h->g_block = static_cast<uint8_t*>(p);
  CUDA_TRY(cudaMemset(p, 0, MP_EXCHANGE_HEADER));
  CUDA_TRY(cudaDeviceSynchronize());
  h->g_world = world; h->g_rank = rank;
  h->buffers.gathered_rgb = h->g_block + MP_EXCHANGE_HEADER;
  h->buffers.gathered_world_rgb = h->g_block + MP_EXCHANGE_HEADER + h->g_world_off;
  h->buffers.gathered_obs_slot_bytes = h->g_slot_bytes;
  if (block) *block = h->g_block;
  if (block_bytes) *block_bytes = h->g_block_bytes;
  return MP_OK;
}

int mp_gather_obs_connect(mp_handle h, void* const* peer_blocks) {
  if (!h || !peer_blocks) return fail(MP_E_INVALID, "mp_gather_obs_connect: null argument");
  if (!h->g_block) return fail(MP_E_INVALID, "mp_gather_obs_connect: call mp_gather_obs_create first");
  if (peer_blocks[h->g_rank] != h->g_block) return fail(MP_E_INVALID, "mp_gather_obs_connect: entry %d must be this rank's own block", h->g_rank);
  DeviceGuard guard(h->device);
  std::vector<unsigned long long*> ptrs(MP_MAX_PEERS, nullptr);
  for (int r = 0; r < h->g_world; ++r) {
    if (!peer_blocks[r]) return fail(MP_E_INVALID, "mp_gather_obs_connect: null pointer for rank %d", r);
    h->g_peer[r] = static_cast<uint8_t*>(peer_blocks[r]);
    ptrs[r] = reinterpret_cast<unsigned long long*>(peer_blocks[r]);
  }
  int rc = h->alloc((size_t)MP_MAX_PEERS, &h->d_g_flag_ptrs);
  if (rc) return rc;
  CUDA_TRY(cudaMemcpy(h->d_g_flag_ptrs, ptrs.data(), MP_MAX_PEERS * sizeof(void*), cudaMemcpyHostToDevice));
  h->S.g_flags = reinterpret_cast<const unsigned long long*>(h->g_block);
  h->S.g_world = h->g_world;
  return MP_OK;
}

int mp_gather_obs_enable(mp_handle h, int on) {
  if (!h || !h->g_block || !h->d_g_flag_ptrs) return fail(MP_E_INVALID, "mp_gather_obs_enable: not connected");
  h->S.g_world = on ? h->g_world : 0;
  return MP_OK;
}

int mp_gather_obs_wait(mp_handle h, void* stream) {
  if (!h || !h->g_block) return fail(MP_E_INVALID, "mp_gather_obs_wait: not created");
  DeviceGuard guard(h->device);
  k_flag_wait<<<1, 32, 0, (cudaStream_t)stream>>>(reinterpret_cast<const unsigned long long*>(h->g_block), h->g_world, h->g_seq);
  ++h->launches;
  CUDA_TRY(cudaGetLastError());
  return MP_OK;
}

int mp_gather_obs_slot(mp_handle h, int* slot, uint64_t* step) {
  if (!h) return fail(MP_E_INVALID, "null handle");
  if (slot) *slot = (int)(h->g_seq & 1ull);
  if (step) *step = h->g_seq;
  return MP_OK;
}

int mp_exchange_wait(mp_handle h, void* stream) {
  if (!h) return fail(MP_E_INVALID, "null handle");
  if (!h->S.x_world) return fail(MP_E_INVALID, "mp_exchange_wait: exchange not connected");
  DeviceGuard guard(h->device);
  k_exchange_wait<<<1, 32, 0, (cudaStream_t)stream>>>(h->S, h->x_seq);
  ++h->launches;
  CUDA_TRY(cudaGetLastError());
  return MP_OK;
}

int mp_exchange_slot(mp_handle h, int* slot, uint64_t* step) {
  if (!h) return fail(MP_E_INVALID, "null handle");
  if (slot) *slot = (int)(h->x_seq & 1ull);
  if (step) *step = h->x_seq;
  return MP_OK;
}

namespace {
struct SnapshotHeader { char magic[4]; uint32_t version; uint64_t num_envs, payload_bytes, n_spans, rng_key0, blob_hash; };
}

int mp_state_size(mp_handle h, uint64_t* bytes) {
  if (!h || !bytes) return fail(MP_E_INVALID, "mp_state_size: null argument");
  *bytes = sizeof(SnapshotHeader) + h->state_bytes;
  return MP_OK;
}

int mp_state_save(mp_handle h, void* host_dst, void* stream) {
  if (!h || !host_dst) return fail(MP_E_INVALID, "mp_state_save: null argument");
  DeviceGuard guard(h->device);
  cudaStream_t st = (cudaStream_t)stream;
  SnapshotHeader hd{{'M', 'P', 'S', '2'}, 2u, (uint64_t)h->B, h->state_bytes, (uint64_t)h->state_spans.size(), h->S.seed, h->blob_hash};
  memcpy(host_dst, &hd, sizeof(hd));
  uint8_t* dst = static_cast<uint8_t*>(host_dst) + sizeof(hd);
  for (const auto& sp : h->state_spans) {
    CUDA_TRY(cudaMemcpyAsync(dst, sp.first, sp.second, cudaMemcpyDeviceToHost, st));
    dst += sp.second;
  }
  CUDA_TRY(cudaStreamSynchronize(st));
  return MP_OK;
}

int mp_state_load(mp_handle h, const void* host_src, uint64_t nbytes, void* stream) {
  if (!h || !host_src) return fail(MP_E_INVALID, "mp_state_load: null argument");
  if (nbytes < sizeof(SnapshotHeader)) return fail(MP_E_INVALID, "mp_state_load: %llu bytes is shorter than a snapshot header", (unsigned long long)nbytes);
  SnapshotHeader hd;
  memcpy(&hd, host_src, sizeof(hd));
  if (memcmp(hd.magic, "MPS2", 4) != 0 || hd.version != 2u) return fail(MP_E_INVALID, "mp_state_load: not a snapshot (or one of an older engine)");
  if (hd.num_envs != (uint64_t)h->B || hd.payload_bytes != h->state_bytes || hd.n_spans != h->state_spans.size())
    return fail(MP_E_INVALID, "mp_state_load: snapshot of %llu envs / %llu bytes does not fit this engine (%d envs / %llu bytes)",
                (unsigned long long)hd.num_envs, (unsigned long long)hd.payload_bytes, h->B, (unsigned long long)h->state_bytes);
  if (nbytes != sizeof(SnapshotHeader) + hd.payload_bytes)
    return fail(MP_E_INVALID, "mp_state_load: buffer of %llu bytes, snapshot needs %llu (truncated?)", (unsigned long long)nbytes,
                (unsigned long long)(sizeof(SnapshotHeader) + hd.payload_bytes));
  if (hd.blob_hash != h->blob_hash) return fail(MP_E_INVALID, "mp_state_load: snapshot was taken from a different compiled substrate");
  if (hd.rng_key0 != h->S.seed) return fail(MP_E_INVALID, "mp_state_load: snapshot was taken with a different seed / env_index_base (key %llu, engine %llu)",
                                            (unsigned long long)hd.rng_key0, (unsigned long long)h->S.seed);
  DeviceGuard guard(h->device);
  cudaStream_t st = (cudaStream_t)stream;
  const uint8_t* src = static_cast<const uint8_t*>(host_src) + sizeof(hd);
  for (const auto& sp : h->state_spans) {
    CUDA_TRY(cudaMemcpyAsync(sp.first, src, sp.second, cudaMemcpyHostToDevice, st));
    src += sp.second;
  }
  int rc = launch_render(h, st);
  if (rc) return rc;
  CUDA_TRY(cudaStreamSynchronize(st));
  return MP_OK;
}

int mp_launch_count(mp_handle h, uint64_t* out) {
  if (!h || !out) return fail(MP_E_INVALID, "null argument");
  *out = h->launches;
  return MP_OK;
}

int mp_debug_render_plan(mp_handle h, int32_t out[8]) {
  if (!h || !out) return fail(MP_E_INVALID, "mp_debug_render_plan: null argument");
  const RenderPlan& R = h->R;
  const int32_t v[8] = {R.n_teams, R.team_threads, R.wstrip_log2, R.smem_bytes, R.n_total, R.rec_stride, R.stage_bytes, R.grid_bytes};
  memcpy(out, v, sizeof v);
  return MP_OK;
}

int mp_debug_render_tables(mp_handle h, int32_t* n_total, uint8_t* pair, uint8_t* flags) {
  if (!h) return fail(MP_E_INVALID, "null handle");
  if (n_total) *n_total = h->n_total;
  if (pair) memcpy(pair, h->host_pair.data(), h->host_pair.size());
  if (flags) memcpy(flags, h->host_sflags.data(), h->host_sflags.size());
  return MP_OK;
}

int mp_debug_observations(mp_handle h, int32_t* position, int32_t* orientation, int32_t* layer, int32_t* zap_matrix, void* stream) {
  if (!h) return fail(MP_E_INVALID, "null handle");
  DeviceGuard guard(h->device);
  k_debug_obs<<<h->B, 128, 0, (cudaStream_t)stream>>>(h->T, h->S, position, orientation, layer, zap_matrix, h->R.view_w, h->R.view_h);
  ++h->launches;
  CUDA_TRY(cudaGetLastError());
  return MP_OK;
}

int mp_debug_lane_map(int n_rows, int n_cells, int pitch_slots, int iters, int scattered, uint32_t out[32]) {
  if (!out || (n_rows != 8 && n_rows != 4 && n_rows != 2) || n_cells < 1 || n_cells > 62 || iters < 1 || iters > 5) return fail(MP_E_INVALID, "mp_debug_lane_map: bad arguments");
  if (!scattered) { if (n_cells > (32 / n_rows) * iters) return fail(MP_E_INVALID, "mp_debug_lane_map: too few turns"); make_lane_map_cells(n_rows, n_cells, pitch_slots, iters, out); return MP_OK; }
  if (!make_lane_map(n_rows, n_cells, pitch_slots, iters, out)) return fail(MP_E_UNSUPPORTED, "no conflict-free dealing for %d rows x %d cells in %d turns", n_rows, n_cells, iters);
  return MP_OK;
}

int mp_algorithmic_bytes(mp_handle h, uint64_t* per_env_step, uint64_t* render_per_env_step) {
  if (!h) return fail(MP_E_INVALID, "null handle");
  if (per_env_step) *per_env_step = h->algo_bytes;
  if (render_per_env_step) *render_per_env_step = h->render_bytes;
  return MP_OK;
}

}
```

### meltingpot_b200/csrc/render.cuh

```cuda
#pragma once

#include <cstdio>

#include "common.cuh"

#define RENDER_MAX_TEAMS 4
#define RENDER_MAX_THREADS 1024
#ifndef TEAM_THREADS
#define TEAM_THREADS 512
#endif
#ifndef RENDER_SLOTS
#define RENDER_SLOTS 1
#endif

struct RenderPlan {
  int view_w, view_h;
  int player_bytes;
  int world_bytes;
  int grid_bytes;
  int atlas_bytes;
  int n_total;
  int rec_stride;
  uint32_t magic_view_h;
  int off_atlas, off_pair, off_map, off_team0, team_stride;
// ... 102 lines not shown
  for (int c = gtid; c < T.cells; c += gthreads) {
    uint32_t v[LMAX];
#pragma unroll
    for (int l = 0; l < LMAX; ++l) v[l] = l < T.L ? s_grid[l * T.cells_pad + c] : 0u;
    uint32_t nz = 0, oq = 0;
#pragma unroll
    for (int l = 0; l < LMAX; ++l) {
      const uint32_t f = v[l] ? s_flags[(v[l] - 1) >> 2] : 8u;
      nz |= ((f & 8u) ? 0u : 1u) << l;
      oq |= (f & 1u) << l;
    }
    oq &= ~1u;
    const int lo = oq ? 31 - __clz(oq) : 0;
    uint32_t cand = nz & (0xffffffffu << lo);
    uint16_t* r = s_rec + c * R.rec_stride;
    int n = 0;
    uint32_t cur = 0, cf = 0;
    bool merging = true;
    while (cand) {
      const int l = __ffs(cand) - 1;
      cand &= cand - 1;
      const uint32_t vl = s_grid[l * T.cells_pad + c];
      if (cur == 0) { cur = vl; cf = s_flags[(vl - 1) >> 2]; continue; }
      if (merging) {
        const uint32_t m = s_pair[((cur - 1) >> 2) * R.n_total + ((vl - 1) >> 2)];
        if (m && (((cur - 1) ^ (vl - 1)) & 3u) == 0) { cur = 1 + m * 4 + ((vl - 1) & 3u); cf = 5; continue; }
        merging = false;
      }
      r[1 + n++] = (uint16_t)((cur - 1) | (cf << ENT_SHIFT));
      cur = vl; cf = s_flags[(vl - 1) >> 2];
    }
    if (cur) r[1 + n++] = (uint16_t)((cur - 1) | (cf << ENT_SHIFT));
    if ((n == 1 && (cf & 1u)) || ((dbg & 256u) && cur)) r[0] = (uint16_t)(REC_FAST | (cur - 1));
    else r[0] = n ? (uint16_t)n : (uint16_t)R.h_empty;
  }
}

__device__ __forceinline__ void store_row(uint8_t* dst, const uint32_t px[8]) {
  uint2 a, b, c;
  a.x = __byte_perm(px[0], px[1], 0x4210); a.y = __byte_perm(px[1], px[2], 0x5421);
  b.x = __byte_perm(px[2], px[3], 0x6542); b.y = __byte_perm(px[4], px[5], 0x4210);
  c.x = __byte_perm(px[5], px[6], 0x5421); c.y = __byte_perm(px[6], px[7], 0x6542);
  uint2* d = reinterpret_cast<uint2*>(dst);
  d[0] = a; d[1] = b; d[2] = c;
}

__device__ __forceinline__ void fast_row(uint32_t px[8], const uint8_t* __restrict__ s_atlas, int h, int py) {
  const uint8_t* t = s_atlas + (h & 0x7fff) * 256 + py * 16;
  const uint4 lo = *reinterpret_cast<const uint4*>(t);
  const uint4 hi = *reinterpret_cast<const uint4*>(t + 128);
  px[0] = lo.x; px[1] = lo.y; px[2] = lo.z; px[3] = lo.w; px[4] = hi.x; px[5] = hi.y; px[6] = hi.z; px[7] = hi.w;
}

struct ViewerInfo {
  int ax, ay, ao, alive, fdx, fdy, rdx, rdy;
};

template <int NCP, int NCW, bool GATHER>
__global__ void __launch_bounds__(RENDER_MAX_THREADS, 1) k_render(Tables T, State S, RenderPlan R, uint32_t flags) {
  extern __shared__ __align__(128) uint8_t smem[];
  uint64_t* bar = reinterpret_cast<uint64_t*>(smem);
  uint8_t* s_atlas = smem + R.off_atlas;
  const uint8_t* s_pair = smem + R.off_pair;
  int16_t* s_map = reinterpret_cast<int16_t*>(smem + R.off_map);
  __shared__ uint8_t s_opaque[256];
  __shared__ ViewerInfo s_view_all[RENDER_MAX_TEAMS][MP_MAX_PLAYERS];
  __shared__ int s_next_item[RENDER_MAX_TEAMS];

  const int tid = threadIdx.x;
  int team = 0;
#pragma unroll
  for (int k = 1; k < RENDER_MAX_TEAMS; ++k) team += tid >= k * R.team_threads;
  asm volatile("" : "+r"(team));
  const int ttid = tid - team * R.team_threads;
  const int lane = tid & 31, twarp = ttid >> 5;
  uint8_t* s_team = smem + R.off_team0 + team * R.team_stride;
  uint16_t* s_grid = reinterpret_cast<uint16_t*>(s_team + R.toff_grid);
  uint16_t* s_rec = reinterpret_cast<uint16_t*>(s_team + R.toff_rec);
  uint8_t* s_stage = s_team + R.toff_stage + twarp * R.stage_bytes;
  ViewerInfo* s_view = s_view_all[team];
  uint64_t* gbar = &bar[1 + team];

  const int n_streams = gridDim.x * R.n_teams;
  const int rounds = S.B / n_streams;
  const int tail0 = rounds * n_streams;
  const int n_tail = (S.B - tail0 - (int)blockIdx.x + (int)gridDim.x - 1) / (int)gridDim.x;
  const int n_iters = rounds + (n_tail > 0 ? n_tail : 0);
  const int first = blockIdx.x * R.n_teams + team;
  if (tid == 0) {
    for (int i = 0; i < 1 + R.n_teams; ++i) mbar_init(&bar[i], 1);
    asm volatile("fence.mbarrier_init.release.cluster;" ::: "memory");
  }
  if (ttid == 0) s_next_item[team] = 0;
  asm volatile("griddepcontrol.launch_dependents;" ::: "memory");
  __syncthreads();
  if (tid == 0) {
    mbar_expect_tx(&bar[0], (uint32_t)R.atlas_bytes);
    bulk_load(s_atlas, T.atlas, (uint32_t)R.atlas_bytes, &bar[0]);
  }
  for (int i = tid; i < (T.P + 1) * R.n_total; i += (int)blockDim.x) s_map[i] = T.sprite_map[i];
  for (int i = tid; i < R.n_total; i += (int)blockDim.x) s_opaque[i] = T.sprite_opaque[i];
  for (int i = tid; i < R.n_total * R.n_total; i += (int)blockDim.x) smem[R.off_pair + i] = T.sprite_pair[i];
  asm volatile("griddepcontrol.wait;" ::: "memory");
  if (GATHER && tid == 64 && S.g_step > 1ull) {
    for (int r = 0; r < S.g_world; ++r)
      while (*(const volatile unsigned long long*)(S.g_flags + r) + 1ull < S.g_step) __nanosleep(200);
  }
  if (ttid == 0 && rounds > 0) {
    mbar_expect_tx(gbar, (uint32_t)R.grid_bytes);
    bulk_load(s_grid, S.grid + (size_t)first * T.L * T.cells_pad, (uint32_t)R.grid_bytes, gbar);
  }
  __syncthreads();
  mbar_wait(&bar[0], 0);

  const int wlog = R.wstrip_log2, wrows = 1 << wlog;
  const int slot_bytes = R.stage_bytes / RENDER_SLOTS;
  const uint64_t store_policy = make_evict_first_policy();
  uint32_t pcells = R.pmap[lane], wcells = R.wmap[lane];
  asm volatile("" : "+r"(pcells), "+r"(wcells));
  uint32_t slot = 0;
  int gtid = ttid, gthreads = R.team_threads, bar_id = 1 + team;
  int* next_ctr = &s_next_item[team];
  for (int it = 0; it < n_iters; ++it) {
    if (it == rounds) {
      __syncthreads();
      uint8_t* s_team0 = smem + R.off_team0;
      s_grid = reinterpret_cast<uint16_t*>(s_team0 + R.toff_grid);
      s_rec = reinterpret_cast<uint16_t*>(s_team0 + R.toff_rec);
      s_view = s_view_all[0];
      gbar = &bar[1];
      next_ctr = &s_next_item[0];
      gtid = tid; gthreads = (int)blockDim.x; bar_id = 0;
      if (tid == 0) {
        mbar_expect_tx(gbar, (uint32_t)R.grid_bytes);
        bulk_load(s_grid, S.grid + (size_t)(tail0 + (int)blockIdx.x) * T.L * T.cells_pad, (uint32_t)R.grid_bytes, gbar);
      }
    }
    const int b = it < rounds ? first + it * n_streams : tail0 + (int)blockIdx.x + (it - rounds) * (int)gridDim.x;
    if (gtid < T.P) {
      const int4 a = *reinterpret_cast<const int4*>(S.avatar + ((size_t)b * T.P + gtid) * 4);
      ViewerInfo vi;
      vi.ax = a.x; vi.ay = a.y; vi.ao = a.z; vi.alive = a.w;
      vi.fdx = dir_dx(a.z); vi.fdy = dir_dy(a.z); vi.rdx = dir_dx((a.z + 1) & 3); vi.rdy = dir_dy((a.z + 1) & 3);
      s_view[gtid] = vi;
    }
    mbar_wait(gbar, (uint32_t)(it & 1));
    if (!(flags & 64u) || it == 0) {
      if (T.L <= 8) cell_pass<8>(T, R, s_grid, s_rec, s_opaque, s_pair, gtid, gthreads, flags);
      else if (T.L <= 10) cell_pass<10>(T, R, s_grid, s_rec, s_opaque, s_pair, gtid, gthreads, flags);
      else if (T.L <= 12) cell_pass<12>(T, R, s_grid, s_rec, s_opaque, s_pair, gtid, gthreads, flags);
      else cell_pass<MP_MAX_LAYERS>(T, R, s_grid, s_rec, s_opaque, s_pair, gtid, gthreads, flags);
    }
    group_sync(bar_id, gthreads);
    if (gtid == 0 && it + 1 < n_iters && it + 1 != rounds) {
      const int nb = it + 1 < rounds ? b + n_streams : b + (int)gridDim.x;
      mbar_expect_tx(gbar, (uint32_t)R.grid_bytes);
      bulk_load(s_grid, S.grid + (size_t)nb * T.L * T.cells_pad, (uint32_t)R.grid_bytes, gbar);
    }

    int next_item = 0;
    if (lane == 0) next_item = atomicAdd(next_ctr, 1);
    for (;;) {
      const int item = __shfl_sync(MP_FULL, next_item, 0);
      if (item >= R.n_items) break;
      if (lane == 0) next_item = atomicAdd(next_ctr, 1);
      uint8_t* buf = s_stage + (slot % RENDER_SLOTS) * slot_bytes;
      ++slot;
      if (lane == 0) bulk_wait_read<RENDER_SLOTS - 1>();
      __syncwarp();
      if (item < R.n_player_items) {
        const int p = (int)(((uint32_t)item * R.magic_view_h) >> 16), cy = item - p * R.view_h;
        const ViewerInfo vi = s_view[p];
        const int16_t* map = s_map + p * R.n_total;
        const int py = lane & 7;
        const int df = T.view_f - cy;
        const int bx = vi.ax + vi.fdx * df - vi.rdx * T.view_l, by = vi.ay + vi.fdy * df - vi.rdy * T.view_l;
        int hdr[NCP];
        if (!(flags & 16u)) {
        int myh = R.h_oov;
        if (lane < R.view_w && vi.alive) {
          int wx = bx + vi.rdx * lane, wy = by + vi.rdy * lane;
          if (wrap_or_reject(T, wx, wy)) {
            const int cell = wy * T.W + wx, h = s_rec[cell * R.rec_stride];
            myh = (h & REC_FAST) ? ((h & ~3) | ((h - vi.ao) & 3)) : cell;
          } else {
            myh = R.h_oob;
          }
        }
#pragma unroll
        for (int i = 0; i < NCP; ++i) hdr[i] = __shfl_sync(MP_FULL, myh, (pcells >> (6 * i)) & 31);
#pragma unroll
        for (int i = 0; i < NCP; ++i) {
          const int cx = (pcells >> (6 * i)) & 63;
          uint32_t q[8];
          fast_row(q, s_atlas, (hdr[i] & REC_FAST) ? hdr[i] : 0, py);
          if (!(hdr[i] & REC_FAST)) compose_row(q, s_atlas, s_rec + hdr[i] * R.rec_stride, map, vi.ao, py);
          if (cx < R.view_w) store_row(buf + py * R.prow_bytes + cx * 24, q);
        }
        }
        if (!(flags & 128u)) fence_async_smem();
        __syncwarp();
        if (lane == 0 && !(flags & 32u)) {
          const size_t off = ((size_t)b * T.P + p) * R.player_bytes + (size_t)cy * R.pitem_bytes;
          bulk_store(S.rgb + off, buf, (uint32_t)R.pitem_bytes, store_policy);
          if (GATHER) for (int r = 0; r < S.g_world; ++r) bulk_store(S.g_rgb[r] + off, buf, (uint32_t)R.pitem_bytes, store_policy);
        }
      } else {
        const int wi = item - R.n_player_items, wy = wi >> (3 - wlog);
        const int py = ((wi & ((8 >> wlog) - 1)) << wlog) | (lane & (wrows - 1));
        const int16_t* map = s_map + T.P * R.n_total;
        const uint16_t* rowrec = s_rec + wy * T.W * R.rec_stride;
        int hdr[NCW];
        if (!(flags & 16u)) {
#pragma unroll
        for (int i = 0; i < NCW; ++i) {
          const int cx = (wcells >> (6 * i)) & 63;
          hdr[i] = cx < T.W ? (int)rowrec[cx * R.rec_stride] : R.h_oov;
        }
#pragma unroll
        for (int i = 0; i < NCW; ++i) {
          const int cx = (wcells >> (6 * i)) & 63;
          uint32_t q[8];
          fast_row(q, s_atlas, (hdr[i] & REC_FAST) ? hdr[i] : 0, py);
          if (!(hdr[i] & REC_FAST)) compose_row(q, s_atlas, rowrec + min(cx, T.W - 1) * R.rec_stride, map, 0, py);
          if (cx < T.W) store_row(buf + (py & (wrows - 1)) * R.wrow_bytes + cx * 24, q);
        }
        }
        if (!(flags & 128u)) fence_async_smem();
        __syncwarp();
        if (lane == 0 && !(flags & 32u)) {
          const size_t off = (size_t)b * R.world_bytes + (size_t)wi * R.witem_bytes;
          bulk_store(S.world_rgb + off, buf, (uint32_t)R.witem_bytes, store_policy);
          if (GATHER) for (int r = 0; r < S.g_world; ++r) bulk_store(S.g_wrgb[r] + off, buf, (uint32_t)R.witem_bytes, store_policy);
        }
      }
    }
    if (S.x_raise && it == 0) exchange_push(T, S);
    group_sync(bar_id, gthreads);
    if (gtid == 0) *next_ctr = 0;
  }
  if (lane == 0) { if (GATHER) asm volatile("cp.async.bulk.wait_group 0;" ::: "memory"); else bulk_wait_read<0>(); }
}
```

### meltingpot_b200/csrc/step_clean_up.cuh

```cuda
#pragma once

#include "common.cuh"

__host__ __device__ inline size_t scratch_round16(size_t n) { return (n + 15) & ~(size_t)15; }

struct WarpScratch {
  uint8_t* occ;
  uint8_t* apple;
  uint8_t* dirt;
  uint32_t* beam_zap;
  uint32_t* beam_2;
  int16_t* tmp;
  const int16_t* apple_of;
  const int16_t* dirt_of;
  const uint8_t* flags;
  const uint8_t* solid;
  const int32_t* act_table;
};

__host__ __device__ inline size_t clean_up_table_bytes(const Tables& T) { return scratch_round16((size_t)T.cells_pad * 6) + scratch_round16((size_t)T.n_actions * 16); }

__host__ __device__ inline size_t warp_scratch_bytes(const Tables& T) {
  size_t words = (size_t)(T.cells + 31) / 32 + 1;
  return scratch_round16(T.cells_pad) + scratch_round16(T.nA_pad) + scratch_round16(T.nD_pad) + 2 * scratch_round16(words * 4) + 64 * 2;
}

__device__ __forceinline__ WarpScratch carve_scratch(const Tables& T, uint8_t* base) {
  WarpScratch s;
  size_t words = (size_t)(T.cells + 31) / 32 + 1;
  s.occ = base; base += scratch_round16(T.cells_pad);
  s.apple = base; base += scratch_round16(T.nA_pad);
  s.dirt = base; base += scratch_round16(T.nD_pad);
  s.beam_zap = (uint32_t*)base; base += scratch_round16(words * 4);
  s.beam_2 = (uint32_t*)base; base += scratch_round16(words * 4);
  s.tmp = (int16_t*)base;
  return s;
}

__device__ void clean_up_reset(const Tables& T, const State& S, int b, int lane, WarpScratch& sc) {
  int32_t* env = S.env + (size_t)b * ENV_COLS;
  const int episode = env[ENV_EPISODE] + 1;
  const uint64_t key = S.seed + (uint64_t)b;
  const uint32_t k0 = (uint32_t)key, k1 = (uint32_t)(key >> 32);
  uint16_t* grid = S.grid + (size_t)b * T.L * T.cells_pad;
  __syncwarp();
  {
    const uint4* src = reinterpret_cast<const uint4*>(T.init_grid);
    uint4* dst = reinterpret_cast<uint4*>(grid);
    const int n16 = T.L * T.cells_pad / 8;
    for (int i = lane; i < n16; i += 32) dst[i] = src[i];
  }
  for (int k = lane; k < T.nA; k += 32) S.apple[(size_t)b * T.nA_pad + k] = (uint8_t)T.apple[k * 3 + 2];
  for (int j = lane; j < T.nD; j += 32) S.dirt[(size_t)b * T.nD_pad + j] = (uint8_t)T.dirt[j * 3 + 2];
  __syncwarp();
  for (int k = lane; k < T.nW; k += 32) {
    int phase = 0;
    if (T.anim_random) {
      uint4 w = philox4x32_10(0u, (uint32_t)episode, (uint32_t)T.water[k * 2], RS_OBJECT_RESET, k0, k1);
      phase = (int)pick(w.x, (uint32_t)T.n_anim);
    }
    S.water[(size_t)b * T.nW_pad + k] = (uint8_t)phase;
    grid[(size_t)T.water_layer * T.cells_pad + T.water[k * 2 + 1]] = cell_value(T.water_sprite[phase], 0);
  }
  for (int i = lane; i < T.n_spawn && i < 64; i += 32) sc.tmp[i] = (int16_t)T.spawn_cell[i];
  __syncwarp();
  if (lane == 0) {
    for (int p = 0; p < T.P; ++p) {
      uint4 w = philox4x32_10(0u, (uint32_t)episode, (uint32_t)p, RS_AVATAR_RESET, k0, k1);
      int r = p + (int)pick(w.x, (uint32_t)(T.n_spawn - p));
      int16_t t = sc.tmp[p]; sc.tmp[p] = sc.tmp[r]; sc.tmp[r] = t;
    }
  }
  __syncwarp();
  if (lane < T.P) {
    uint4 w = philox4x32_10(0u, (uint32_t)episode, (uint32_t)lane, RS_AVATAR_RESET, k0, k1);
    int cell = sc.tmp[lane], orient = (int)(w.y & 3u);
    int32_t* av = S.avatar + ((size_t)b * T.P + lane) * 4;
    av[AV_X] = cell % T.W; av[AV_Y] = cell / T.W; av[AV_ORIENT] = orient; av[AV_ALIVE] = 1;
    int32_t* tm = S.av_timer + ((size_t)b * T.P + lane) * 4;
    tm[TM_ZAP] = 0; tm[TM_BEAM2] = 0; tm[TM_FRAME] = 0; tm[3] = 0;
    grid[(size_t)T.avatar_layer * T.cells_pad + cell] = cell_value(T.avatar_sprite[lane], orient);
    S.reward[(size_t)b * T.P + lane] = 0.0;
    S.packed[(size_t)b * (T.P + 2) + lane] = 0.0;
    for (int k = 0; k < T.n_scalar; ++k)
      S.scalar_obs[((size_t)k * S.B + b) * T.P + lane] = T.scalar_obs[k] == 0 ? 1.0 : 0.0;
  }
  if (lane == 0) {
    env[ENV_STEP] = 0; env[ENV_EPISODE] = episode; env[ENV_DONE] = 0; env[ENV_DIRT] = T.dirt_count0;
    env[ENV_CLEANED] = 0; env[ENV_ATE] = 0; env[ENV_BEAM] = 0;
    S.discount[b] = 0.0;
    S.step_type[b] = 0;
    S.packed[(size_t)b * (T.P + 2) + T.P] = 0.0; S.packed[(size_t)b * (T.P + 2) + T.P + 1] = 0.0;
  }
  __syncwarp();
}

__device__ __forceinline__ void beam_scan(const BeamGeom& G, int lane, bool self_blocked, bool& vis) {
  bool ok = lane < G.n;
  int parent = ok ? G.parent[lane] : -1;
  vis = ok;
  bool open = ok && !self_blocked;
  for (int d = 0; d < G.depth; ++d) {
    int src = parent < 0 ? lane : parent;
    bool pv = __shfl_sync(MP_FULL, vis, src);
    bool po = __shfl_sync(MP_FULL, open, src);
    if (ok && parent >= 0) { vis = pv && po; }
    open = vis && !self_blocked;
  }
}

__device__ void clean_up_step(const Tables& T, const State& S, int b, int lane, const int32_t* __restrict__ actions, WarpScratch& sc) {
  int32_t* env = S.env + (size_t)b * ENV_COLS;
  const int n = env[ENV_STEP] + 1;
  const int episode = env[ENV_EPISODE];
  const uint64_t key = S.seed + (uint64_t)b;
  const uint32_t k0 = (uint32_t)key, k1 = (uint32_t)(key >> 32);
  uint16_t* grid = S.grid + (size_t)b * T.L * T.cells_pad;
  int dirt_count = env[ENV_DIRT];
  const unsigned cleaned_prev = (unsigned)env[ENV_CLEANED];
  unsigned cleaned_now = 0, ate_now = 0;
  const bool is_av = lane < T.P;

  int x = 0, y = 0, orient = 0, alive = 0, zap_cool = 0, clean_cool = 0, state_frame = 0;
  int act_move = 0, act_turn = 0, act_zap = 0, act_clean = 0;
  if (is_av) {
    const int4 a = *reinterpret_cast<const int4*>(S.avatar + ((size_t)b * T.P + lane) * 4);
    const int4 t = *reinterpret_cast<const int4*>(S.av_timer + ((size_t)b * T.P + lane) * 4);
    x = a.x; y = a.y; orient = a.z; alive = a.w; zap_cool = t.x; clean_cool = t.y; state_frame = t.z;
    int id = actions[(size_t)b * T.P + lane];
    if (id < 0 || id >= T.n_actions) id = 0;
    const int4 at = *reinterpret_cast<const int4*>(sc.act_table + id * 4);
    act_move = at.x; act_turn = at.y; act_zap = at.z; act_clean = at.w;
  }
  const int x0 = x, y0 = y, orient0 = orient, alive0 = alive;
  double reward = 0.0;

  for (int i = lane; i < T.cells_pad / 8; i += 32)
    reinterpret_cast<uint2*>(sc.occ)[i] = reinterpret_cast<const uint2*>(sc.solid)[i];
  for (int i = lane; i < T.nA_pad / 16; i += 32) {
    uint4 v = reinterpret_cast<const uint4*>(S.apple + (size_t)b * T.nA_pad)[i];
    v.x |= (v.x & 0x01010101u) << 3; v.y |= (v.y & 0x01010101u) << 3; v.z |= (v.z & 0x01010101u) << 3; v.w |= (v.w & 0x01010101u) << 3;
    reinterpret_cast<uint4*>(sc.apple)[i] = v;
  }
  for (int i = lane; i < T.nD_pad / 16; i += 32) {
    uint4 v = reinterpret_cast<const uint4*>(S.dirt + (size_t)b * T.nD_pad)[i];
    v.x |= (v.x & 0x01010101u) << 3; v.y |= (v.y & 0x01010101u) << 3; v.z |= (v.z & 0x01010101u) << 3; v.w |= (v.w & 0x01010101u) << 3;
    reinterpret_cast<uint4*>(sc.dirt)[i] = v;
  }
  const int words = (T.cells + 31) / 32 + 1;
  for (int i = lane; i < words; i += 32) { sc.beam_zap[i] = 0; sc.beam_2[i] = 0; }
  __syncwarp();
  if (is_av && alive) sc.occ[y * T.W + x] = (uint8_t)(lane + 1);
  if (env[ENV_BEAM]) {
    uint4 z = make_uint4(0, 0, 0, 0);
    uint4* lz = reinterpret_cast<uint4*>(grid + (size_t)T.zap_layer * T.cells_pad);
    uint4* lc = reinterpret_cast<uint4*>(grid + (size_t)T.clean_layer * T.cells_pad);
    for (int i = lane; i < T.cells_pad / 8; i += 32) { lz[i] = z; lc[i] = z; }
  }
  __syncwarp();
  int beam_dirty = 0;

  int spawn_dirt = -1;
  if (n > T.dirt_delay) {
    uint4 w = philox4x32_10((uint32_t)n, (uint32_t)episode, SCENE_DRAW_DIRT, RS_SCENE, k0, k1);
    int n_inactive = T.nD - dirt_count;
    if (u01(w.x, w.y) < T.dirt_prob && n_inactive > 0) {
      int kth = (int)pick(w.z, (uint32_t)n_inactive);
      for (int base = 0; base < T.nD; base += 32) {
        int j = base + lane;
        bool inactive = j < T.nD && !(sc.dirt[j] & 1);
        unsigned m = __ballot_sync(MP_FULL, inactive);
        int c = __popc(m);
        if (kth < c) {
          unsigned mm = m;
          for (int q = 0; q < kth; ++q) mm &= mm - 1;
          spawn_dirt = base + __ffs(mm) - 1;
          break;
        }
        kth -= c;
      }
    }
  }
  {
    const double dirt = (double)dirt_count, clean = (double)(T.nD - dirt_count);
    const double fraction = dirt / (dirt + clean);
    double interpolation = (fraction - T.grow_depletion) / (T.grow_restoration - T.grow_depletion);
    interpolation = fmin(interpolation, 1.0);
    const double probability = T.grow_rate * interpolation;
    if (probability > 0.0) {
      for (int k = lane; k < T.nA; k += 32) {
        uint4 w = philox4x32_10((uint32_t)n, (uint32_t)episode, (uint32_t)T.apple[k * 3], RS_OBJECT, k0, k1);
        if (u01(w.x, w.y) < probability && !(sc.apple[k] & 1)) sc.apple[k] |= 4;
      }
    }
  }
  __syncwarp();

  int rank = 0;
  {
    uint4 w = philox4x32_10((uint32_t)n, (uint32_t)episode, (uint32_t)lane, RS_AVATAR, k0, k1);
    uint32_t mykey = w.x;
    for (int q = 0; q < T.P; ++q) {
      uint32_t kq = __shfl_sync(MP_FULL, mykey, q);
      if (is_av && (kq < mykey || (kq == mykey && q < lane))) ++rank;
    }
    if (!is_av) rank = 99;
  }
  bool fire_zap = false, fire_clean = false;
  if (is_av && alive) {
    if (zap_cool > 0) --zap_cool; else if (act_zap == 1) { zap_cool = T.zap_cooldown; fire_zap = true; }
    if (clean_cool > 0) --clean_cool; else if (act_clean == 1) { clean_cool = T.clean_cooldown; fire_clean = true; }
  }
  const bool want_respawn = is_av && !alive && (n - state_frame) >= T.zap_respawn;
  bool cont = true;
  if (n >= T.end_min_frames && ((n + 1) % T.end_interval) == 0) {
    uint4 w = philox4x32_10((uint32_t)n, (uint32_t)episode, SCENE_DRAW_EPISODE_END, RS_SCENE, k0, k1);
    if (u01(w.x, w.y) < T.end_prob) cont = false;
  }
  const int num_others_cleaned = is_av ? __popc(cleaned_prev & ~(1u << lane)) : 0;

  if (spawn_dirt >= 0) { if (lane == 0) sc.dirt[spawn_dirt] |= 1; ++dirt_count; }
  __syncwarp();
  for (int base = 0; base < T.nA; base += 32) {
    int k = base + lane;
    bool grows = k < T.nA && (sc.apple[k] & 4);
    int eater = -1;
    if (grows) {
      sc.apple[k] = (sc.apple[k] & ~4) | 1;
      int o = sc.occ[T.apple[k * 3 + 1]];
      if (o >= 1 && o <= T.P) { eater = o - 1; sc.apple[k] |= 2; }
    }
    unsigned m = __ballot_sync(MP_FULL, eater >= 0);
    while (m) {
      int src = __ffs(m) - 1; m &= m - 1;
      int e = __shfl_sync(MP_FULL, eater, src);
      if (lane == e) { reward += T.eat_reward; emit_event(S, b, EV_EDIBLE_CONSUMED, e + 1, 0); }
      ate_now |= 1u << e;
    }
  }
  __syncwarp();
  for (int r = 0; r < T.P; ++r) {
    unsigned m = __ballot_sync(MP_FULL, is_av && rank == r);
    int src = __ffs(m) - 1;
    const uint32_t packed = __shfl_sync(MP_FULL, (uint32_t)(alive & 1) | ((uint32_t)(act_turn + 1) << 1) | ((uint32_t)act_move << 3) |
                                                     ((uint32_t)orient << 6) | ((uint32_t)y << 8) | ((uint32_t)x << 20), src);
    if (!(packed & 1u)) continue;
    const int s_turn = (int)((packed >> 1) & 3u) - 1, s_move = (int)((packed >> 3) & 7u);
    int so = (int)((packed >> 6) & 3u), sy = (int)((packed >> 8) & 0xfffu), sx = (int)(packed >> 20);
    if (s_turn != 0) so = (so + s_turn) & 3;
    bool ate = false;
    if (s_move != 0) {
      int d = (so + s_move - 1) & 3;
      int nx = sx + dir_dx(d), ny = sy + dir_dy(d);
      bool inb = wrap_or_reject(T, nx, ny);
      if (inb && sc.occ[ny * T.W + nx] == 0) {
        __syncwarp();
        if (lane == 0) { sc.occ[sy * T.W + sx] = 0; sc.occ[ny * T.W + nx] = (uint8_t)(src + 1); }
        sx = nx; sy = ny;
      }
      int fcell = sy * T.W + sx;
      int ai = sc.apple_of[fcell];
      ate = ai >= 0 && (sc.apple[ai] & 1);
      __syncwarp();
      if (ate && lane == 0) sc.apple[ai] |= 2;
    }
    if (lane == src) { x = sx; y = sy; orient = so; if (ate) { reward += T.eat_reward; emit_event(S, b, EV_EDIBLE_CONSUMED, src + 1, 0); } }
    if (ate) ate_now |= 1u << src;
    __syncwarp();
  }
  unsigned zapped = 0;
  for (int pass = 0; pass < 2; ++pass) {
    const BeamGeom& G = pass == 0 ? T.zap_geom : T.clean_geom;
    for (int r = 0; r < T.P; ++r) {
      unsigned m = __ballot_sync(MP_FULL, is_av && rank == r && (pass == 0 ? fire_zap : fire_clean));
      if (!m) continue;
      int src = __ffs(m) - 1;
      int sx = __shfl_sync(MP_FULL, x, src), sy = __shfl_sync(MP_FULL, y, src), so = __shfl_sync(MP_FULL, orient, src);
      int cell = -1; bool blocked = false; int hit_avatar = -1, hit_dirt = -1;
      if (lane < G.n) {
        int f = so, rgt = (so + 1) & 3;
        int cx = sx + dir_dx(f) * G.fwd[lane] + dir_dx(rgt) * G.lat[lane];
        int cy = sy + dir_dy(f) * G.fwd[lane] + dir_dy(rgt) * G.lat[lane];
        if (!wrap_or_reject(T, cx, cy)) { blocked = true; }
        else {
          cell = cy * T.W + cx;
          int hit = pass == 0 ? T.zap_hit : T.clean_hit;
          if (sc.flags[cell] & (1 << hit)) blocked = true;
          if (pass == 0) {
            int o = sc.occ[cell];
            if (o >= 1 && o <= T.P && o - 1 != src) { hit_avatar = o - 1; blocked = true; }
          } else {
            int dj = sc.dirt_of[cell];
            if (dj >= 0 && (sc.dirt[dj] & 1)) { hit_dirt = dj; blocked = true; }
          }
        }
      }
      bool vis;
      beam_scan(G, lane, blocked, vis);
      if (pass == 0) {
        unsigned hm = __ballot_sync(MP_FULL, vis && hit_avatar >= 0);
        while (hm) {
          int c = __ffs(hm) - 1; hm &= hm - 1;
          int t = __shfl_sync(MP_FULL, hit_avatar, c);
          if (lane == t) reward += T.zap_penalty;
          if (lane == src) { reward += T.zap_reward; emit_event(S, b, EV_ZAP, src + 1, t + 1); }
          if (T.zap_remove) zapped |= 1u << t;
        }
      } else {
        bool cleaned = vis && hit_dirt >= 0;
        if (cleaned) { sc.dirt[hit_dirt] |= 2; emit_event(S, b, EV_PLAYER_CLEANED, src + 1, 0); }
        if (__any_sync(MP_FULL, cleaned)) cleaned_now |= 1u << src;
      }
      if (vis && !blocked && cell >= 0) {
        uint32_t* bm = pass == 0 ? sc.beam_zap : sc.beam_2;
        uint32_t bit = 1u << (cell & 31);
        uint32_t old = atomicOr(&bm[cell >> 5], bit);
        if (!(old & bit)) {
          int layer = pass == 0 ? T.zap_layer : T.clean_layer, sprite = pass == 0 ? T.zap_sprite : T.clean_sprite;
          grid[(size_t)layer * T.cells_pad + cell] = cell_value(sprite, so);
        }
        beam_dirty = 1;
      }
      __syncwarp();
    }
  }
  beam_dirty = __any_sync(MP_FULL, beam_dirty);
  for (int r = 0; r < T.P; ++r) {
    unsigned m = __ballot_sync(MP_FULL, is_av && rank == r && want_respawn);
    if (!m) continue;
    int src = __ffs(m) - 1;
    uint4 w = philox4x32_10((uint32_t)n, (uint32_t)episode, (uint32_t)src, RS_AVATAR, k0, k1);
    int target = T.spawn_cell[pick(w.y, (uint32_t)T.n_spawn)];
    if (sc.occ[target] != 0) continue;
    __syncwarp();
    if (lane == 0) sc.occ[target] = (uint8_t)(src + 1);
    int ai = sc.apple_of[target];
    bool ate = ai >= 0 && (sc.apple[ai] & 1);
    __syncwarp();
    if (ate && lane == 0) sc.apple[ai] |= 2;
    if (lane == src) {
      x = target % T.W; y = target / T.W; orient = (int)(w.z & 3u); alive = 1; state_frame = n;
      if (ate) { reward += T.eat_reward; emit_event(S, b, EV_EDIBLE_CONSUMED, src + 1, 0); }
    }
    if (ate) ate_now |= 1u << src;
    __syncwarp();
  }

  if (is_av && (zapped >> lane & 1u)) { alive = 0; state_frame = n; }
  for (int k = lane; k < T.nA; k += 32) {
    uint8_t v = sc.apple[k];
    uint8_t was = (v >> 3) & 1;
    uint8_t now = (v & 1) && !(v & 2);
    if (now != was) {
      S.apple[(size_t)b * T.nA_pad + k] = now;
      grid[(size_t)T.apple_layer * T.cells_pad + T.apple[k * 3 + 1]] = now ? cell_value(T.apple_sprite, 0) : (uint16_t)0;
    }
  }
  int d_delta = 0;
  for (int j = lane; j < T.nD; j += 32) {
    uint8_t v = sc.dirt[j];
    uint8_t was = (v >> 3) & 1;
    uint8_t now = (v & 1) && !(v & 2);
    if ((v & 1) && (v & 2)) --d_delta;
    if (now != was) {
      S.dirt[(size_t)b * T.nD_pad + j] = now;
      grid[(size_t)T.dirt_layer * T.cells_pad + T.dirt[j * 3 + 1]] = now ? cell_value(T.dirt_sprite, 0) : (uint16_t)0;
    }
  }
  for (int o = 16; o > 0; o >>= 1) d_delta += __shfl_xor_sync(MP_FULL, d_delta, o);
  dirt_count += d_delta;
  if (n % T.anim_frames == 0) {
    const int turn = (n / T.anim_frames) % T.n_anim;
    for (int k = lane; k < T.nW; k += 32) {
      int phase = (int)S.water[(size_t)b * T.nW_pad + k] + turn;
      if (phase >= T.n_anim) phase -= T.n_anim;
      grid[(size_t)T.water_layer * T.cells_pad + T.water[k * 2 + 1]] = cell_value(T.water_sprite[phase], 0);
    }
  }
  const bool changed = is_av && (x != x0 || y != y0 || orient != orient0 || alive != alive0);
  if (changed && alive0) grid[(size_t)T.avatar_layer * T.cells_pad + y0 * T.W + x0] = 0;
  __syncwarp();
  if (changed && alive) grid[(size_t)T.avatar_layer * T.cells_pad + y * T.W + x] = cell_value(T.avatar_sprite[lane], orient);

  const bool done = !cont || n >= T.max_frames;
  if (is_av) {
    *reinterpret_cast<int4*>(S.avatar + ((size_t)b * T.P + lane) * 4) = make_int4(x, y, orient, alive);
    *reinterpret_cast<int4*>(S.av_timer + ((size_t)b * T.P + lane) * 4) = make_int4(zap_cool, clean_cool, state_frame, 0);
    S.reward[(size_t)b * T.P + lane] = reward;
    S.packed[(size_t)b * (T.P + 2) + lane] = reward;
    for (int k = 0; k < T.n_scalar; ++k) {
      double v;
      if (T.scalar_obs[k] == 0)
        v = alive ? fmax(1.0 - (double)zap_cool / (double)T.zap_cooldown, 0.0) : 0.0;
      else
        v = (double)num_others_cleaned;
      S.scalar_obs[((size_t)k * S.B + b) * T.P + lane] = v;
    }
  }
  if (lane == 0) {
    env[ENV_STEP] = n; env[ENV_DONE] = done ? 1 : 0; env[ENV_DIRT] = dirt_count;
    env[ENV_CLEANED] = (int)cleaned_now; env[ENV_ATE] = (int)ate_now; env[ENV_BEAM] = beam_dirty;
    S.discount[b] = done ? 0.0 : 1.0;
    S.step_type[b] = done ? 2 : 1;
    S.packed[(size_t)b * (T.P + 2) + T.P] = done ? 0.0 : 1.0;
    S.packed[(size_t)b * (T.P + 2) + T.P + 1] = done ? 2.0 : 1.0;
  }
}

__global__ void __launch_bounds__(128, 8) k_step_clean_up(Tables T, State S, const int32_t* __restrict__ actions,
                                                       const uint8_t* __restrict__ mask, int mode) {
  extern __shared__ __align__(128) uint8_t smem[];
  const int warp = threadIdx.x >> 5, lane = threadIdx.x & 31;
  asm volatile("griddepcontrol.launch_dependents;" ::: "memory");
  int16_t* s_apple_of = reinterpret_cast<int16_t*>(smem + 4 * warp_scratch_bytes(T));
  int16_t* s_dirt_of = s_apple_of + T.cells_pad;
  uint8_t* s_solid = reinterpret_cast<uint8_t*>(s_dirt_of + T.cells_pad);
  uint8_t* s_flags = s_solid + T.cells_pad;
  int32_t* s_act = reinterpret_cast<int32_t*>(smem + 4 * warp_scratch_bytes(T) + scratch_round16((size_t)T.cells_pad * 6));
  for (int i = threadIdx.x; i < T.cells_pad; i += (int)blockDim.x) { s_apple_of[i] = T.apple_of_cell[i]; s_dirt_of[i] = T.dirt_of_cell[i]; s_flags[i] = T.cell_flags[i]; s_solid[i] = T.solid[i]; }
  for (int i = threadIdx.x; i < T.n_actions * 4; i += (int)blockDim.x) s_act[i] = T.action_table[i];
  asm volatile("griddepcontrol.wait;" ::: "memory");
  __syncthreads();
  const int b = blockIdx.x * 4 + warp;
  if (b >= S.B) return;
  WarpScratch sc = carve_scratch(T, smem + warp * warp_scratch_bytes(T));
  sc.apple_of = s_apple_of; sc.dirt_of = s_dirt_of; sc.flags = s_flags; sc.solid = s_solid; sc.act_table = s_act;
  if (!(mode == 1 && !(mask == nullptr || mask[b]))) {
    event_begin(lane);
    if (mode == 1 || S.env[(size_t)b * ENV_COLS + ENV_DONE]) clean_up_reset(T, S, b, lane, sc);
    else clean_up_step(T, S, b, lane, actions, sc);
    event_end(S, b, lane);
  }
}
```

### meltingpot_b200/csrc/step_commons.cuh

```cuda
#pragma once

#include "common.cuh"
#include "step_clean_up.cuh"

__device__ __forceinline__ bool ch_is_wait(uint8_t s) { return s != 0; }

__device__ void commons_reset(const Tables& T, const State& S, int b, int lane, WarpScratch& sc) {
  int32_t* env = S.env + (size_t)b * ENV_COLS;
  const int episode = env[ENV_EPISODE] + 1;
  const uint64_t key = S.seed + (uint64_t)b;
  const uint32_t k0 = (uint32_t)key, k1 = (uint32_t)(key >> 32);
  uint16_t* grid = S.grid + (size_t)b * T.L * T.cells_pad;
  __syncwarp();
  {
    const uint4* src = reinterpret_cast<const uint4*>(T.init_grid);
    uint4* dst = reinterpret_cast<uint4*>(grid);
    const int n16 = T.L * T.cells_pad / 8;
    for (int i = lane; i < n16; i += 32) dst[i] = src[i];
  }
  for (int k = lane; k < T.nA; k += 32) {
    S.apple[(size_t)b * T.nA_pad + k] = T.ch_apple[k * 4 + 2] ? 0 : 1;
    S.apple_count[(size_t)b * T.nA_pad + k] = 0;
  }
  __syncwarp();
// ... 140 lines not shown
      const bool fresh = ate && !(s_state[ai] & 64);
      __syncwarp();
      if (fresh) {
        if (lane == 0) { s_state[ai] |= 64; s_events[n_events] = (int16_t)ai; }
        ++n_events;
      }
    }
    if (lane == src) { x = sx; y = sy; orient = so; if (ate) { reward += T.eat_reward; emit_event(S, b, EV_EDIBLE_CONSUMED, src + 1, 0); } }
    __syncwarp();
  }
  unsigned zapped = 0;
  for (int r = 0; r < T.P; ++r) {
    unsigned m = __ballot_sync(MP_FULL, is_av && rank == r && fire_zap);
    if (!m) continue;
    int src = __ffs(m) - 1;
    int sx = __shfl_sync(MP_FULL, x, src), sy = __shfl_sync(MP_FULL, y, src), so = __shfl_sync(MP_FULL, orient, src);
    const BeamGeom& G = T.zap_geom;
    int cell = -1; bool blocked = false; int hit_avatar = -1;
    if (lane < G.n) {
      int f = so, rgt = (so + 1) & 3;
      int cx = sx + dir_dx(f) * G.fwd[lane] + dir_dx(rgt) * G.lat[lane];
      int cy = sy + dir_dy(f) * G.fwd[lane] + dir_dy(rgt) * G.lat[lane];
      if (!wrap_or_reject(T, cx, cy)) blocked = true;
      else {
        cell = cy * T.W + cx;
        if (T.cell_flags[cell] & (1 << T.zap_hit)) blocked = true;
        int o = sc.occ[cell];
        if (o >= 1 && o <= T.P && o - 1 != src) { hit_avatar = o - 1; blocked = true; }
      }
    }
    bool vis;
    beam_scan(G, lane, blocked, vis);
    unsigned hm = __ballot_sync(MP_FULL, vis && hit_avatar >= 0);
    while (hm) {
      int c = __ffs(hm) - 1; hm &= hm - 1;
      int t = __shfl_sync(MP_FULL, hit_avatar, c);
      if (lane == t) reward += T.zap_penalty;
      if (lane == src) { reward += T.zap_reward; emit_event(S, b, EV_ZAP, src + 1, t + 1); }
      if (T.zap_remove) zapped |= 1u << t;
    }
    if (vis && !blocked && cell >= 0) {
      uint32_t bit = 1u << (cell & 31);
      uint32_t old = atomicOr(&sc.beam_zap[cell >> 5], bit);
      if (!(old & bit)) grid[(size_t)T.zap_layer * T.cells_pad + cell] = cell_value(T.zap_sprite, so);
      beam_dirty = 1;
    }
    __syncwarp();
  }
  beam_dirty = __any_sync(MP_FULL, beam_dirty);
  for (int r = 0; r < T.P; ++r) {
    unsigned m = __ballot_sync(MP_FULL, is_av && rank == r && want_respawn);
    if (!m) continue;
    int src = __ffs(m) - 1;
    uint4 w = philox4x32_10((uint32_t)n, (uint32_t)episode, (uint32_t)src, RS_AVATAR, k0, k1);
    int target = T.spawn_cell[pick(w.y, (uint32_t)T.n_spawn)];
    if (sc.occ[target] != 0) continue;
    __syncwarp();
    if (lane == 0) sc.occ[target] = (uint8_t)(src + 1);
    int ai = T.apple_of_cell[target];
    bool ate = ai >= 0 && (s_state[ai] & 31) == 0;
    bool fresh = ate && !(s_state[ai] & 64);
    __syncwarp();
    if (fresh && lane == 0) { s_state[ai] |= 64; s_events[n_events] = (int16_t)ai; }
    if (fresh) ++n_events;
    if (lane == src) {
      x = target % T.W; y = target / T.W; orient = (int)(w.z & 3u); alive = 1; state_frame = n;
      if (ate) { reward += T.eat_reward; emit_event(S, b, EV_EDIBLE_CONSUMED, src + 1, 0); }
    }
    __syncwarp();
  }
  for (int base = 0; base < T.nA; base += 32) {
    int k = base + lane;
    unsigned sm = __ballot_sync(MP_FULL, k < T.nA && (s_state[k] & 32));
    while (sm) {
      const int i = base + __ffs(sm) - 1; sm &= sm - 1;
      __syncwarp();
      if (lane == 0) s_state[i] = 0;
      __syncwarp();
      if (lane < 16) {
        const int j = T.ch_nbr[i * 16 + lane];
        if (j >= 0 && ch_is_wait(s_state[j] & 31)) s_count[j] += 1;
      }
      const int cell = T.ch_apple[i * 4 + 1];
      const int o = sc.occ[cell];
      if (o >= 1 && o <= T.P) {
        if (lane == o - 1) { reward += T.eat_reward; emit_event(S, b, EV_EDIBLE_CONSUMED, o, 0); }
        __syncwarp();
        if (lane == 0) { s_state[i] |= 64; s_events[n_events] = (int16_t)i; }
        ++n_events;
      }
      __syncwarp();
    }
  }

  for (int e = 0; e < n_events; ++e) {
    const int i = s_events[e];
    __syncwarp();
    if (lane == 0) s_state[i] = 1;
    __syncwarp();
    int live = 0;
    if (lane < 16) {
      const int j = T.ch_nbr[i * 16 + lane];
      if (j >= 0) {
        if (ch_is_wait(s_state[j] & 31)) s_count[j] -= 1; else live = 1;
      }
    }
    const unsigned lm = __ballot_sync(MP_FULL, live);
    if (lane == 0) s_count[i] = (uint8_t)__popc(lm);
    __syncwarp();
  }
  if (is_av && (zapped >> lane & 1u)) { alive = 0; state_frame = n; }

  for (int k = lane; k < T.nA; k += 32) {
    const uint8_t now = s_state[k] & 31;
    const uint8_t was = S.apple[(size_t)b * T.nA_pad + k];
    if (now != was) {
      S.apple[(size_t)b * T.nA_pad + k] = now;
      const int cell = T.ch_apple[k * 4 + 1];
      if ((now == 0) != (was == 0)) {
        grid[(size_t)T.apple_layer * T.cells_pad + cell] = now == 0 ? cell_value(T.apple_sprite, 0) : (uint16_t)0;
        grid[(size_t)T.wait_layer * T.cells_pad + cell] = now == 0 ? (uint16_t)0 : cell_value(T.wait_sprite, 0);
      }
    }
    S.apple_count[(size_t)b * T.nA_pad + k] = s_count[k];
  }
  const bool changed = is_av && (x != x0 || y != y0 || orient != orient0 || alive != alive0);
  if (changed && alive0) grid[(size_t)T.avatar_layer * T.cells_pad + y0 * T.W + x0] = 0;
  __syncwarp();
  if (changed && alive) grid[(size_t)T.avatar_layer * T.cells_pad + y * T.W + x] = cell_value(T.avatar_sprite[lane], orient);

  const bool done = !cont || n >= T.max_frames;
  if (is_av) {
    *reinterpret_cast<int4*>(S.avatar + ((size_t)b * T.P + lane) * 4) = make_int4(x, y, orient, alive);
    *reinterpret_cast<int4*>(S.av_timer + ((size_t)b * T.P + lane) * 4) = make_int4(zap_cool, 0, state_frame, 0);
    S.reward[(size_t)b * T.P + lane] = reward;
    S.packed[(size_t)b * (T.P + 2) + lane] = reward;
    for (int k = 0; k < T.n_scalar; ++k)
      S.scalar_obs[((size_t)k * S.B + b) * T.P + lane] = alive ? fmax(1.0 - (double)zap_cool / (double)T.zap_cooldown, 0.0) : 0.0;
  }
  if (lane == 0) {
    env[ENV_STEP] = n; env[ENV_DONE] = done ? 1 : 0; env[ENV_BEAM] = beam_dirty;
    S.discount[b] = done ? 0.0 : 1.0;
    S.step_type[b] = done ? 2 : 1;
    S.packed[(size_t)b * (T.P + 2) + T.P] = done ? 0.0 : 1.0;
    S.packed[(size_t)b * (T.P + 2) + T.P + 1] = done ? 2.0 : 1.0;
  }
}

__global__ void __launch_bounds__(128, 8) k_step_commons(Tables T, State S, const int32_t* __restrict__ actions,
                                                     const uint8_t* __restrict__ mask, int mode) {
  extern __shared__ __align__(128) uint8_t smem[];
  const int warp = threadIdx.x >> 5, lane = threadIdx.x & 31;
  asm volatile("griddepcontrol.launch_dependents;" ::: "memory");
  asm volatile("griddepcontrol.wait;" ::: "memory");
  const int b = blockIdx.x * 4 + warp;
  if (b >= S.B) return;
  WarpScratch sc = carve_scratch(T, smem + warp * warp_scratch_bytes(T));
  if (!(mode == 1 && !(mask == nullptr || mask[b]))) {
    event_begin(lane);
    if (mode == 1 || S.env[(size_t)b * ENV_COLS + ENV_DONE]) commons_reset(T, S, b, lane, sc);
    else commons_step(T, S, b, lane, actions, sc);
    event_end(S, b, lane);
  }
}
```

### meltingpot_b200/engine.py

```python

from __future__ import annotations

import ctypes
import os
from typing import Dict, Optional

import numpy as np

_HERE = os.path.dirname(os.path.abspath(__file__))
LIB_PATH = os.environ.get('MP_ENGINE_LIB') or os.path.join(_HERE, 'libmpengine.so')

MP_FLAG_RENDER_WORLD = 1
MP_FLAG_RENDER_PLAYERS = 2
MP_FLAG_DEFAULT = 3

EXPORTED_SYMBOLS = (
    'mp_create', 'mp_destroy', 'mp_set_flags', 'mp_reset', 'mp_step',
    'mp_step_state', 'mp_render', 'mp_get_buffers', 'mp_step_host',
    'mp_reset_host', 'mp_launch_count', 'mp_algorithmic_bytes', 'mp_debug_render_tables', 'mp_debug_render_plan', 'mp_state_size', 'mp_state_save', 'mp_state_load',
    'mp_step_host_async', 'mp_wait', 'mp_exchange_create', 'mp_ipc_export', 'mp_ipc_open', 'mp_enable_peer_access',
    'mp_exchange_connect', 'mp_exchange_wait', 'mp_exchange_slot', 'mp_debug_lane_map', 'mp_debug_observations',
    'mp_gather_obs_create', 'mp_gather_obs_connect', 'mp_gather_obs_enable', 'mp_gather_obs_wait', 'mp_gather_obs_slot',
    'mp_last_error', 'mp_version',
)


class MpBuffers(ctypes.Structure):
  _fields_ = [
      ('num_envs', ctypes.c_int32), ('num_players', ctypes.c_int32),
      ('rgb_h', ctypes.c_int32), ('rgb_w', ctypes.c_int32),
      ('world_h', ctypes.c_int32), ('world_w', ctypes.c_int32),
      ('num_actions', ctypes.c_int32), ('num_scalar_obs', ctypes.c_int32),
      ('rgb', ctypes.c_void_p), ('world_rgb', ctypes.c_void_p),
      ('reward', ctypes.c_void_p), ('discount', ctypes.c_void_p),
      ('step_type', ctypes.c_void_p), ('scalar_obs', ctypes.c_void_p),
      ('avatar_state', ctypes.c_void_p), ('grid', ctypes.c_void_p),
      ('grid_layers', ctypes.c_int32), ('grid_cells', ctypes.c_int32),
      ('grid_cells_padded', ctypes.c_int32),
      ('timestep_packed', ctypes.c_void_p),
      ('events', ctypes.c_void_p), ('event_count', ctypes.c_void_p), ('max_events', ctypes.c_int32),
      ('scalar_block', ctypes.c_void_p), ('scalar_block_bytes', ctypes.c_uint64),
      ('gathered', ctypes.c_void_p), ('gathered_world', ctypes.c_int32),
      ('gathered_rgb', ctypes.c_void_p), ('gathered_world_rgb', ctypes.c_void_p), ('gathered_obs_slot_bytes', ctypes.c_uint64),
  ]


class MpHostOutputs(ctypes.Structure):
  _fields_ = [
      ('rgb', ctypes.c_void_p), ('world_rgb', ctypes.c_void_p),
      ('reward', ctypes.c_void_p), ('discount', ctypes.c_void_p),
      ('step_type', ctypes.c_void_p), ('scalar_obs', ctypes.c_void_p),
      ('scalar_block', ctypes.c_void_p), ('events', ctypes.c_void_p), ('event_count', ctypes.c_void_p),
  ]


_lib = None


def load_library() -> ctypes.CDLL:
  global _lib
  if _lib is not None:
    return _lib
  if not os.path.exists(LIB_PATH):
    raise RuntimeError(
        f'{LIB_PATH} is missing: build it with `python -m meltingpot_b200.build` '
        '(the engine has no CPU or PyTorch fallback)')
  lib = ctypes.CDLL(LIB_PATH)
  vp = ctypes.c_void_p
  lib.mp_create.argtypes = [ctypes.c_char_p, ctypes.c_size_t, ctypes.c_int,
                            ctypes.c_int, ctypes.c_uint64, ctypes.c_uint64,
                            ctypes.c_uint32, ctypes.POINTER(vp)]
  lib.mp_destroy.argtypes = [vp]
  lib.mp_set_flags.argtypes = [vp, ctypes.c_uint32]
  lib.mp_reset.argtypes = [vp, vp, vp]
  lib.mp_step.argtypes = [vp, vp, vp]
  lib.mp_step_state.argtypes = [vp, vp, vp]
  lib.mp_render.argtypes = [vp, vp]
  lib.mp_get_buffers.argtypes = [vp, ctypes.POINTER(MpBuffers)]
  lib.mp_step_host.argtypes = [vp, vp, ctypes.POINTER(MpHostOutputs), vp]
  lib.mp_reset_host.argtypes = [vp, ctypes.POINTER(MpHostOutputs), vp]
  lib.mp_launch_count.argtypes = [vp, ctypes.POINTER(ctypes.c_uint64)]
  lib.mp_algorithmic_bytes.argtypes = [vp, ctypes.POINTER(ctypes.c_uint64),
                                       ctypes.POINTER(ctypes.c_uint64)]
  lib.mp_state_size.argtypes = [vp, ctypes.POINTER(ctypes.c_uint64)]
  lib.mp_state_save.argtypes = [vp, vp, vp]
  lib.mp_state_load.argtypes = [vp, vp, ctypes.c_uint64, vp]
  lib.mp_debug_render_plan.argtypes = [vp, ctypes.POINTER(ctypes.c_int32)]
  lib.mp_debug_render_tables.argtypes = [vp, ctypes.POINTER(ctypes.c_int32), vp, vp]
  lib.mp_step_host_async.argtypes = [vp, vp, ctypes.POINTER(MpHostOutputs), ctypes.c_int, vp]
  lib.mp_wait.argtypes = [vp, ctypes.c_int]
  lib.mp_exchange_create.argtypes = [vp, ctypes.c_int, ctypes.c_int, ctypes.POINTER(vp), ctypes.POINTER(ctypes.c_uint64)]
  lib.mp_ipc_export.argtypes = [vp, vp, ctypes.POINTER(ctypes.c_uint64)]
  lib.mp_ipc_open.argtypes = [ctypes.c_int, vp, ctypes.c_uint64, ctypes.POINTER(vp)]
  lib.mp_enable_peer_access.argtypes = [ctypes.c_int, ctypes.c_int]
  lib.mp_exchange_connect.argtypes = [vp, ctypes.POINTER(vp)]
  lib.mp_exchange_wait.argtypes = [vp, vp]
  lib.mp_exchange_slot.argtypes = [vp, ctypes.POINTER(ctypes.c_int), ctypes.POINTER(ctypes.c_uint64)]
  lib.mp_gather_obs_create.argtypes = [vp, ctypes.c_int, ctypes.c_int, ctypes.POINTER(vp), ctypes.POINTER(ctypes.c_uint64)]
  lib.mp_gather_obs_connect.argtypes = [vp, ctypes.POINTER(vp)]
  lib.mp_gather_obs_enable.argtypes = [vp, ctypes.c_int]
  lib.mp_gather_obs_wait.argtypes = [vp, vp]
  lib.mp_gather_obs_slot.argtypes = [vp, ctypes.POINTER(ctypes.c_int), ctypes.POINTER(ctypes.c_uint64)]
  lib.mp_debug_observations.argtypes = [vp] * 6
  lib.mp_debug_lane_map.argtypes = [ctypes.c_int] * 5 + [ctypes.POINTER(ctypes.c_uint32)]
  lib.mp_last_error.restype = ctypes.c_char_p
  lib.mp_version.restype = ctypes.c_char_p
  _lib = lib
  return lib


EVENT_NAMES = {1: 'zap', 2: 'edible_consumed', 3: 'player_cleaned', 4: 'claimed_resource',
               5: 'destroyed_resource', 6: 'sanctioning', 7: 'removal_due_to_sanctioning', 8: 'coin_consumed',
               9: 'mining', 10: 'extraction', 11: 'extraction_pair'}
EVENT_FIELDS = {1: ('source', 'target'), 2: ('player_index',), 3: ('player_index',), 4: ('player_index',),
                5: ('player_index',), 6: ('source', 'target'), 7: ('source', 'target'), 8: ('player_index', 'matched'),
                9: ('player', 'ore_type'), 10: ('player', 'ore_type'), 11: ('player_a', 'player_b_and_ore_type')}


class EngineError(RuntimeError):
  pass


def _check(rc: int) -> None:
  if rc != 0:
    msg = load_library().mp_last_error().decode('utf-8', 'replace')
    if rc in (-1, -2):
      raise ValueError(f'mp_engine error {rc}: {msg}')
    raise EngineError(f'mp_engine error {rc}: {msg}')


class _Handle:

  def __init__(self, lib, handle):
    self._lib = lib
    self.h = handle

  def __del__(self):
    try:
      if self.h:
        self._lib.mp_destroy(self.h)
        self.h = None
    except Exception:
      pass


class _CudaView:

  def __init__(self, ptr: int, shape, typestr: str, owner):
    self._owner = owner
    self.__cuda_array_interface__ = {
        'shape': tuple(int(s) for s in shape), 'typestr': typestr,
        'data': (int(ptr), False), 'version': 2, 'strides': None,
    }


class Engine:

  def __init__(self, blob: bytes, num_envs: int, device: int = 0, seed: int = 1,
               env_index_base: int = 0, flags: int = MP_FLAG_DEFAULT):
    import torch
    if not torch.cuda.is_available():
      raise EngineError('CUDA is not available: the B200 engine has no CPU path')
    self._torch = torch
    self._lib = load_library()
    self._blob = bytes(blob)
    self.device = int(device)
    self.num_envs = int(num_envs)
# ... 78 lines not shown
    if (actions.dtype != torch.int32 or not actions.is_cuda or not actions.is_contiguous()
        or actions.shape != (self.num_envs, self.num_players)
        or actions.device.index != self.device):
      raise ValueError('actions must be a contiguous int32 CUDA tensor [B, P] on the engine device')

  def make_host_outputs(self, rgb=True, world_rgb=True, events=False) -> Dict[str, 'np.ndarray']:
    torch = self._torch
    b = self.buffers
    B, P = self.num_envs, self.num_players
    ns = max(self.num_scalar_obs, 1)
    n_words = int(b.scalar_block_bytes) // 8
    assert n_words == B * P + 2 * B + ns * B * P
    block = torch.empty((n_words,), dtype=torch.float64).pin_memory()
    o = 0
    out = {'scalar_block': block}
    out['reward'] = block[o:o + B * P].view(B, P); o += B * P
    out['discount'] = block[o:o + B]; o += B
    out['step_type'] = block[o:o + B].view(torch.int64); o += B
    out['scalar_obs'] = block[o:o + ns * B * P].view(ns, B, P)
    if rgb:
      out['rgb'] = torch.empty((B, P, b.rgb_h, b.rgb_w, 3), dtype=torch.uint8).pin_memory()
    if world_rgb:
      out['world_rgb'] = torch.empty((B, b.world_h, b.world_w, 3), dtype=torch.uint8).pin_memory()
    if events:
      out['events'] = torch.empty((B, b.max_events, 3), dtype=torch.int32).pin_memory()
      out['event_count'] = torch.empty((B,), dtype=torch.int32).pin_memory()
    return out

  def make_host_actions(self):
    return self._torch.zeros((self.num_envs, self.num_players), dtype=self._torch.int32).pin_memory()

  @staticmethod
  def _host_struct(outputs) -> MpHostOutputs:
    s = MpHostOutputs()
    for name in ('rgb', 'world_rgb', 'reward', 'discount', 'step_type', 'scalar_obs', 'scalar_block', 'events', 'event_count'):
      t = outputs.get(name) if outputs else None
      setattr(s, name, ctypes.c_void_p(t.data_ptr()) if t is not None else None)
    return s

  def step_host(self, actions_host, outputs, stream=None) -> None:
    assert actions_host.dtype == self._torch.int32 and not actions_host.is_cuda
    assert actions_host.is_contiguous() and actions_host.shape == (self.num_envs, self.num_players)
    s = self._host_struct(outputs)
    _check(self._lib.mp_step_host(self._h, ctypes.c_void_p(actions_host.data_ptr()),
                                  ctypes.byref(s), self._stream(stream)))

  def step_host_async(self, actions_host, outputs, slot: int, stream=None) -> None:
    assert actions_host.dtype == self._torch.int32 and not actions_host.is_cuda
    assert actions_host.is_contiguous() and actions_host.shape == (self.num_envs, self.num_players)
    s = self._host_struct(outputs)
    _check(self._lib.mp_step_host_async(self._h, ctypes.c_void_p(actions_host.data_ptr()), ctypes.byref(s),
                                        int(slot), self._stream(stream)))

  def wait(self, slot: int) -> None:
    _check(self._lib.mp_wait(self._h, int(slot)))

  def exchange_create(self, rank: int, world: int):
    ptr, n = ctypes.c_void_p(), ctypes.c_uint64(0)
    _check(self._lib.mp_exchange_create(self._h, int(rank), int(world), ctypes.byref(ptr), ctypes.byref(n)))
    self._x_world, self._x_rank = int(world), int(rank)
    bufs = MpBuffers()
    _check(self._lib.mp_get_buffers(self._h, ctypes.byref(bufs)))
    self.buffers = bufs
    torch = self._torch
    self.gathered = torch.as_tensor(
        _CudaView(bufs.gathered, (2, world * self.num_envs, self.num_players + 2), '<f8', self._owner),
        device=torch.device('cuda', self.device), dtype=torch.float64)
    return int(ptr.value), int(n.value)

  def exchange_connect(self, peer_blocks) -> None:
    arr = (ctypes.c_void_p * len(peer_blocks))(*[ctypes.c_void_p(int(p)) for p in peer_blocks])
    _check(self._lib.mp_exchange_connect(self._h, arr))

  def exchange_wait(self, stream=None) -> None:
    _check(self._lib.mp_exchange_wait(self._h, self._stream(stream)))

  def exchange_slot(self):
    slot, step = ctypes.c_int(0), ctypes.c_uint64(0)
    _check(self._lib.mp_exchange_slot(self._h, ctypes.byref(slot), ctypes.byref(step)))
    return int(slot.value), int(step.value)

  def gathered_timestep(self):
    return self.gathered[self.exchange_slot()[0]]

  def gather_obs_create(self, rank: int, world: int):
    ptr, n = ctypes.c_void_p(), ctypes.c_uint64(0)
    _check(self._lib.mp_gather_obs_create(self._h, int(rank), int(world), ctypes.byref(ptr), ctypes.byref(n)))
    bufs = MpBuffers()
    _check(self._lib.mp_get_buffers(self._h, ctypes.byref(bufs)))
    self.buffers = bufs
    torch = self._torch
    dev = torch.device('cuda', self.device)
    B, P = self.num_envs, self.num_players
    slot = int(bufs.gathered_obs_slot_bytes)
    self.gathered_rgb = [torch.as_tensor(_CudaView(bufs.gathered_rgb + k * slot, (world * B, P, bufs.rgb_h, bufs.rgb_w, 3), '|u1', self._owner),
                                         device=dev, dtype=torch.uint8) for k in range(2)]
    self.gathered_world_rgb = [torch.as_tensor(_CudaView(bufs.gathered_world_rgb + k * slot, (world * B, bufs.world_h, bufs.world_w, 3), '|u1', self._owner),
                                               device=dev, dtype=torch.uint8) for k in range(2)]
    return int(ptr.value), int(n.value)

  def gather_obs_connect(self, peer_blocks) -> None:
    arr = (ctypes.c_void_p * len(peer_blocks))(*[ctypes.c_void_p(int(p)) for p in peer_blocks])
    _check(self._lib.mp_gather_obs_connect(self._h, arr))

  def gather_obs_enable(self, on: bool) -> None:
    _check(self._lib.mp_gather_obs_enable(self._h, int(bool(on))))

  def gather_obs_wait(self, stream=None) -> None:
    _check(self._lib.mp_gather_obs_wait(self._h, self._stream(stream)))

  def gathered_observations(self):
    slot = ctypes.c_int(0)
    _check(self._lib.mp_gather_obs_slot(self._h, ctypes.byref(slot), None))
    return self.gathered_rgb[slot.value], self.gathered_world_rgb[slot.value]

  def debug_observations(self, layer: bool = True, zap_matrix: bool = True, stream=None):
    torch = self._torch
    dev = torch.device('cuda', self.device)
    b = self.buffers
    B, P = self.num_envs, self.num_players
    out = {'POSITION': torch.empty((B, P, 2), dtype=torch.int32, device=dev),
           'ORIENTATION': torch.empty((B, P), dtype=torch.int32, device=dev)}
    if layer:
      out['LAYER'] = torch.empty((B, P, b.rgb_h // 8, b.rgb_w // 8, b.grid_layers), dtype=torch.int32, device=dev)
    if zap_matrix:
      out['ZAP_MATRIX'] = torch.empty((B, P, P), dtype=torch.int32, device=dev)
    ptr = lambda k: ctypes.c_void_p(out[k].data_ptr()) if k in out else None
    _check(self._lib.mp_debug_observations(self._h, ptr('POSITION'), ptr('ORIENTATION'), ptr('LAYER'), ptr('ZAP_MATRIX'),
                                           self._stream(stream)))
    return out

  def reset_host(self, outputs, stream=None) -> None:
    s = self._host_struct(outputs)
    _check(self._lib.mp_reset_host(self._h, ctypes.byref(s), self._stream(stream)))

  def launch_count(self) -> int:
    n = ctypes.c_uint64(0)
    _check(self._lib.mp_launch_count(self._h, ctypes.byref(n)))
    return int(n.value)

  def save_state(self, stream=None) -> bytes:
    n = ctypes.c_uint64(0)
    _check(self._lib.mp_state_size(self._h, ctypes.byref(n)))
    buf = ctypes.create_string_buffer(n.value)
    _check(self._lib.mp_state_save(self._h, buf, self._stream(stream)))
    return buf.raw

  def load_state(self, snapshot: bytes, stream=None) -> None:
    snapshot = bytes(snapshot)
    buf = ctypes.create_string_buffer(snapshot, len(snapshot))
    _check(self._lib.mp_state_load(self._h, buf, ctypes.c_uint64(len(snapshot)), self._stream(stream)))

  def render_plan(self):
    out = (ctypes.c_int32 * 8)()
    _check(self._lib.mp_debug_render_plan(self._h, out))
    keys = ('teams', 'team_threads', 'wstrip_log2', 'smem_bytes', 'atlas_sprites', 'rec_stride', 'stage_bytes', 'grid_bytes')
    return dict(zip(keys, (int(v) for v in out)))

  def render_tables(self):
    import numpy as np
    n = ctypes.c_int32(0)
    _check(self._lib.mp_debug_render_tables(self._h, ctypes.byref(n), None, None))
    pair = np.zeros((n.value, n.value), np.uint8)
    flags = np.zeros((n.value,), np.uint8)
    _check(self._lib.mp_debug_render_tables(self._h, ctypes.byref(n), pair.ctypes.data, flags.ctypes.data))
    return pair, flags

  def algorithmic_bytes(self):
    a, r = ctypes.c_uint64(0), ctypes.c_uint64(0)
    _check(self._lib.mp_algorithmic_bytes(self._h, ctypes.byref(a), ctypes.byref(r)))
    return int(a.value), int(r.value)


def ipc_export(device_ptr: int):
  handle = ctypes.create_string_buffer(64)
  off = ctypes.c_uint64(0)
  _check(load_library().mp_ipc_export(ctypes.c_void_p(int(device_ptr)), handle, ctypes.byref(off)))
  return handle.raw, int(off.value)


def ipc_open(device: int, handle: bytes, offset: int) -> int:
  ptr = ctypes.c_void_p()
  buf = ctypes.create_string_buffer(bytes(handle), 64)
  _check(load_library().mp_ipc_open(int(device), buf, ctypes.c_uint64(int(offset)), ctypes.byref(ptr)))
  return int(ptr.value)


def enable_peer_access(device: int, peer_device: int) -> None:
  _check(load_library().mp_enable_peer_access(int(device), int(peer_device)))
```

Baseline: 17.76 million.

## Overlap next step kernel with render via per-env consumed flags

Lets the step kernel for clean_up and commons_harvest start while the previous render is still running. Render publishes a per-env 'consumed' sequence flag and a completion counter, and step warps spin-wait on those flags instead of the grid dependency wait. The render plan is shrunk to leave registers and shared memory for co-resident step CTAs, and step work follows render order so early envs can proceed. Clean_up's shared tables are packed into one blob and copied with vectorized loads. The risks are spin-wait overhead, a smaller render configuration, and deadlock or ordering bugs if residency assumptions fail.

After: 17.77 million (median of 6 runs). About the same (+0.1%).

```diff
diff --git a/include/mp_engine.h b/include/mp_engine.h
--- a/include/mp_engine.h
+++ b/include/mp_engine.h
@@ -28,7 +28,8 @@
   MP_FLAG_DEBUG_NO_FENCE = 1u << 7,
   MP_FLAG_DEBUG_TOP_SPRITE_ONLY = 1u << 8,
   MP_FLAG_DEBUG_PLAIN_LANE_MAP = 1u << 9,
-  MP_FLAG_DEBUG_SCATTER_LANE_MAP = 1u << 10
+  MP_FLAG_DEBUG_SCATTER_LANE_MAP = 1u << 10,
+  MP_FLAG_DEBUG_NO_OVERLAP = 1u << 11
 };
 
 typedef struct mp_buffers {
@@ -114,7 +115,7 @@
 int mp_state_save(mp_handle h, void* host_dst, void* stream);
 int mp_state_load(mp_handle h, const void* host_src, uint64_t nbytes, void* stream);
 
-int mp_debug_render_plan(mp_handle h, int32_t out[8]);
+int mp_debug_render_plan(mp_handle h, int32_t out[10]);
 
 int mp_debug_render_tables(mp_handle h, int32_t* n_total, uint8_t* pair, uint8_t* flags);
 
diff --git a/meltingpot_b200/csrc/common.cuh b/meltingpot_b200/csrc/common.cuh
--- a/meltingpot_b200/csrc/common.cuh
+++ b/meltingpot_b200/csrc/common.cuh
@@ -2,6 +2,9 @@
 
 #include <cuda_runtime.h>
 #include <stdint.h>
+
+#include <cassert>
+#include <cstdio>
 
 #define MP_MAX_PLAYERS 16
 #define MP_MAX_LAYERS 16
@@ -70,6 +73,7 @@
   const uint8_t* cell_flags;
   const int16_t* apple_of_cell;
   const int16_t* dirt_of_cell;
+  const uint8_t* clean_up_tables;
   const uint8_t* atlas;
   const int16_t* sprite_map;
   const uint8_t* sprite_opaque;
@@ -120,7 +124,57 @@
   uint8_t* g_rgb[MP_MAX_PEERS];
   uint8_t* g_wrgb[MP_MAX_PEERS];
   const unsigned long long* g_flags;
+  uint32_t* consumed;
+  uint32_t* render_done;
+  uint32_t render_seq;
+  uint32_t wait_seq, wait_done;
+  int order_ctas, order_teams, order_k, order_front;
 };
+
+__device__ __forceinline__ int render_order_env(int B, int n_ctas, int n_teams, int r, int i) {
+  const int n_streams = n_ctas * n_teams, rounds = B / n_streams;
+  if (i < rounds * n_teams) {
+    const int it = i / n_teams;
+    return r * n_teams + (i - it * n_teams) + it * n_streams;
+  }
+  const int b = rounds * n_streams + r + (i - rounds * n_teams) * n_ctas;
+  return b < B ? b : -1;
+}
+
+__device__ __forceinline__ void wait_flag(const uint32_t* flag, uint32_t target, int b) {
+  for (uint32_t spins = 0;; ++spins) {
+    uint32_t v;
+    asm volatile("ld.acquire.gpu.global.u32 %0, [%1];" : "=r"(v) : "l"(flag) : "memory");
+    if ((int32_t)(v - target) >= 0) break;
+    if (spins == (1u << 25)) {
+      printf("wait_flag: env %d (-1: render completion) target %u flag %u never reached\n", b, target, v);
+      assert(false);
+    }
+    __nanosleep(256);
+  }
+  __syncwarp();
+}
+
+__device__ __forceinline__ int step_env(const State& S, int i, int warp) {
+  const int wpc = (int)blockDim.x >> 5;
+  if (S.wait_seq == 0) {
+    const int b = (int)blockIdx.x * wpc + warp;
+    return i == 0 && b < S.B ? b : -1;
+  }
+  const int resident = S.order_ctas * S.order_k, nq = S.order_k * wpc;
+  int r = 0, idx = -1;
+  if ((int)blockIdx.x < resident) {
+    r = (int)blockIdx.x % S.order_ctas;
+    if (i < S.order_front) idx = (int)blockIdx.x / S.order_ctas * wpc + warp + i * nq;
+  } else if (i == 0) {
+    const int g = ((int)blockIdx.x - resident) * wpc + warp;
+    r = g % S.order_ctas;
+    idx = S.order_front * nq + g / S.order_ctas;
+  }
+  const int b = idx < 0 ? -1 : render_order_env(S.B, S.order_ctas, S.order_teams, r, idx);
+  wait_flag(b >= 0 ? S.consumed + b : S.render_done, b >= 0 ? S.wait_seq : S.wait_done, b);
+  return b;
+}
 
 #define MP_MIN_EVENTS 64
 enum { EV_ZAP = 1, EV_EDIBLE_CONSUMED = 2, EV_PLAYER_CLEANED = 3, EV_CLAIMED_RESOURCE = 4, EV_DESTROYED_RESOURCE = 5,
diff --git a/meltingpot_b200/csrc/engine.cu b/meltingpot_b200/csrc/engine.cu
--- a/meltingpot_b200/csrc/engine.cu
+++ b/meltingpot_b200/csrc/engine.cu
@@ -57,6 +57,7 @@
 int round_up(int v, int m) { return (v + m - 1) / m * m; }
 
 constexpr int kRenderSmemLimit = 227 * 1024 - 2560;
+constexpr int kRenderStaticSmem = 2560, kStepStaticSmem = 128;
 constexpr int kMaxAtlasSprites = 96;
 #define MP_MAX_DEVICES 64
 #define MP_EXCHANGE_HEADER 256
@@ -213,6 +214,10 @@
   uint64_t state_bytes = 0;
   int lane_map_players = 0, lane_map_world = 0;
   uint64_t blob_hash = 0;
+  int overlap_ctas = 0, overlap_warps = 0;
+  uint32_t render_seq = 0, render_ctas = 0;
+  bool render_last = false;
+  cudaStream_t render_stream = nullptr;
 
   template <typename T>
   int upload(const std::vector<T>& host, const T** out) {
@@ -493,6 +498,16 @@
   for (int k = 0; k < T.nA; ++k) apple_of[v_apple[k * apple_cols + 1]] = (int16_t)k;
   for (int j = 0; j < T.nD; ++j) { dirt_of[v_dirt[j * 3 + 1]] = (int16_t)j; T.dirt_count0 += v_dirt[j * 3 + 2]; }
   if ((rc = E->upload(apple_of, &T.apple_of_cell)) || (rc = E->upload(dirt_of, &T.dirt_of_cell))) return rc;
+  if (E->family == MPB_FAMILY_CLEAN_UP) {
+    const size_t cp = (size_t)T.cells_pad;
+    std::vector<uint8_t> packed(clean_up_table_bytes(T), 0);
+    memcpy(&packed[0], apple_of.data(), cp * 2); memcpy(&packed[cp * 2], dirt_of.data(), cp * 2);
+    memcpy(&packed[cp * 4], solid.data(), cp); memcpy(&packed[cp * 5], flags.data(), cp);
+    memcpy(&packed[clean_up_act_offset(T)], act.data(), std::min<size_t>(act.size(), (size_t)T.n_actions * 4) * sizeof(int32_t));
+    memcpy(&packed[clean_up_apple_offset(T)], v_apple.data(), std::min<size_t>(v_apple.size() * 4, (size_t)T.nA * 12));
+    memcpy(&packed[clean_up_dirt_offset(T)], v_dirt.data(), std::min<size_t>(v_dirt.size() * 4, (size_t)T.nD * 12));
+    if ((rc = E->upload(packed, &T.clean_up_tables))) return rc;
+  }
 
   if (atlas.count != (size_t)T.n_sprites * 1024) return fail(MP_E_INVALID, "atlas has %zu bytes, expected %d", atlas.count, T.n_sprites * 1024);
   std::vector<uint8_t> img(atlas.data, atlas.data + atlas.count);
@@ -642,7 +657,7 @@
   return MP_OK;
 }
 
-int build_plan(mp_engine* E) {
+int build_plan(mp_engine* E, int max_warps, int smem_limit) {
   const Tables& T = E->T;
   RenderPlan& R = E->R;
   R.view_w = T.view_l + T.view_r + 1; R.view_h = T.view_f + T.view_b + 1;
@@ -662,12 +677,12 @@
   double best = -1.0;
   for (int teams = 2; teams <= RENDER_MAX_TEAMS; ++teams)
     for (int warps = TEAM_THREADS / 32; warps >= 4; --warps) {
-      if (teams * warps > RENDER_MAX_THREADS / 32) continue;
+      if (teams * warps > max_warps) continue;
       for (int wlog = 2; wlog >= 1; --wlog) {
         const int stage = RENDER_SLOTS * round_up(std::max(R.view_w * 192, T.W * 24 * (1 << wlog)), 128);
         const int team_bytes = round_up(R.grid_bytes, 128) + round_up(T.cells * R.rec_stride * 2, 128) + warps * stage;
         const int total = R.off_team0 + teams * team_bytes;
-        if (total > kRenderSmemLimit) continue;
+        if (total > smem_limit) continue;
         const double items = T.P * R.view_h + (8 >> wlog) * T.H, per_warp = items / warps;
         const double score = teams * warps * per_warp / (per_warp + 3.0) * (wlog == 2 ? 1.0 : 0.85) * (1.0 - 0.01 * teams);
         if (score > best + 1e-9) {
@@ -679,7 +694,39 @@
         }
       }
     }
-  if (R.smem_bytes > kRenderSmemLimit) return fail(MP_E_UNSUPPORTED, "render kernel needs %d B of shared memory (> 227 KB)", R.smem_bytes);
+  if (R.smem_bytes > smem_limit) return fail(MP_E_UNSUPPORTED, "render kernel needs %d B of shared memory (> %d B)", R.smem_bytes, smem_limit);
+  return MP_OK;
+}
+
+bool overlap_family(int family) { return family == MPB_FAMILY_CLEAN_UP || family == MPB_FAMILY_COMMONS_HARVEST; }
+void (*step_fn(int family))(Tables, State, const int32_t*, const uint8_t*, int) {
+  return family == MPB_FAMILY_CLEAN_UP ? k_step_clean_up : family == MPB_FAMILY_COMMONS_HARVEST ? k_step_commons :
+         family == MPB_FAMILY_COINS ? k_step_coins : family == MPB_FAMILY_COOP_MINING ? k_step_mining : k_step_territory;
+}
+size_t step_smem_bytes(const mp_engine* E, int warps) {
+  return E->step_smem * warps + (E->family == MPB_FAMILY_CLEAN_UP ? clean_up_table_bytes(E->T) : E->family == MPB_FAMILY_TERRITORY ? territory_table_bytes(E->T) : 0);
+}
+
+constexpr int OVERLAP_WARPS = 2;
+constexpr int OVERLAP_FRONT_PCT = 25;
+
+int plan_overlap(mp_engine* E, const cudaDeviceProp& prop) {
+  E->overlap_ctas = E->overlap_warps = 0;
+  if (!overlap_family(E->family)) return MP_OK;
+  cudaFuncAttributes fr, fs;
+  CUDA_TRY(cudaFuncGetAttributes(&fr, E->render_fn));
+  CUDA_TRY(cudaFuncGetAttributes(&fs, step_fn(E->family)));
+  const int render_warps = E->R.n_teams * E->R.team_threads / 32;
+  auto warp_regs = [](int regs) { return round_up(regs * 32, 256); };
+  const int free_regs = prop.regsPerMultiprocessor - render_warps * warp_regs(fr.numRegs);
+  const int free_warps = std::min(free_regs / warp_regs(fs.numRegs), prop.maxThreadsPerMultiProcessor / 32 - render_warps);
+  const int warps = std::min(4, free_warps);
+  if (warps < 1) return MP_OK;
+  const long free_smem = (long)prop.sharedMemPerMultiprocessor - (long)(E->R.smem_bytes + fr.sharedSizeBytes + prop.reservedSharedMemPerBlock);
+  const long cta_smem = (long)(step_smem_bytes(E, warps) + fs.sharedSizeBytes + prop.reservedSharedMemPerBlock);
+  const int ctas = (int)std::min<long>(free_warps / warps, free_smem / cta_smem);
+  if (ctas < 1) return MP_OK;
+  E->overlap_ctas = ctas; E->overlap_warps = warps;
   return MP_OK;
 }
 
@@ -720,19 +767,40 @@
   return MP_OK;
 }
 
+uint32_t overlap_seq(const mp_engine* E, int mode, cudaStream_t st) {
+  if (mode != 0 || E->overlap_ctas == 0 || (E->flags & MP_FLAG_DEBUG_NO_OVERLAP) || E->S.x_world != 0) return 0;
+  if (!E->render_last || E->render_stream != st) return 0;
+  cudaStreamCaptureStatus cs = cudaStreamCaptureStatusNone;
+  if (cudaStreamIsCapturing(st, &cs) != cudaSuccess || cs != cudaStreamCaptureStatusNone) return 0;
+  return E->render_seq;
+}
+
 int launch_state(mp_engine* E, const int32_t* actions, const uint8_t* mask, int mode, cudaStream_t st, bool render_follows = true) {
-  const int blocks = (E->B + 3) / 4;
   if (E->S.x_world) E->S.x_step = ++E->x_seq;
-  void (*fn)(Tables, State, const int32_t*, const uint8_t*, int) =
-      E->family == MPB_FAMILY_CLEAN_UP ? k_step_clean_up : E->family == MPB_FAMILY_COMMONS_HARVEST ? k_step_commons :
-      E->family == MPB_FAMILY_COINS ? k_step_coins : E->family == MPB_FAMILY_COOP_MINING ? k_step_mining : k_step_territory;
+  State S = E->S;
+  S.wait_seq = overlap_seq(E, mode, st);
+  E->render_last = false;
   cudaLaunchConfig_t cfg = {};
-  cfg.gridDim = dim3(blocks); cfg.blockDim = dim3(128); cfg.dynamicSmemBytes = E->step_smem * 4 + (E->family == MPB_FAMILY_CLEAN_UP ? clean_up_table_bytes(E->T) : E->family == MPB_FAMILY_TERRITORY ? territory_table_bytes(E->T) : 0); cfg.stream = st;
+  if (S.wait_seq) {
+    S.wait_done = E->render_ctas;
+    S.order_ctas = std::min(E->B, E->sm_count); S.order_teams = E->R.n_teams; S.order_k = E->overlap_ctas;
+    const int n_streams = S.order_ctas * S.order_teams, tail0 = E->B / n_streams * n_streams;
+    const int per_cta = tail0 / S.order_ctas + (E->B - tail0 + S.order_ctas - 1) / S.order_ctas;
+    const int nq = S.order_k * E->overlap_warps;
+    S.order_front = std::min((per_cta * OVERLAP_FRONT_PCT / 100 + nq - 1) / nq, (per_cta + nq - 1) / nq);
+    const int late_warps = S.order_ctas * std::max(0, per_cta - S.order_front * nq);
+    cfg.gridDim = dim3(S.order_ctas * S.order_k + (late_warps + E->overlap_warps - 1) / E->overlap_warps);
+    cfg.blockDim = dim3(32 * E->overlap_warps);
+    cfg.dynamicSmemBytes = step_smem_bytes(E, E->overlap_warps);
+  } else {
+    cfg.gridDim = dim3((E->B + 3) / 4); cfg.blockDim = dim3(128); cfg.dynamicSmemBytes = step_smem_bytes(E, 4);
+  }
+  cfg.stream = st;
   cudaLaunchAttribute attr[1];
   attr[0].id = cudaLaunchAttributeProgrammaticStreamSerialization;
   attr[0].val.programmaticStreamSerializationAllowed = 1;
   cfg.attrs = attr; cfg.numAttrs = 1;
-  CUDA_TRY(cudaLaunchKernelEx(&cfg, fn, E->T, E->S, actions, mask, mode));
+  CUDA_TRY(cudaLaunchKernelEx(&cfg, step_fn(E->family), E->T, S, actions, mask, mode));
   if (E->S.x_world) {
     E->x_pending_raise = true;
     if (!render_follows) { ++E->launches; return raise_flags(E, st); }
@@ -771,7 +839,16 @@
       E->S.g_wrgb[r] = base + E->g_world_off + (size_t)E->g_rank * E->B * R.world_bytes;
     }
   }
-  CUDA_TRY(cudaLaunchKernelEx(&cfg, gather ? E->render_gather_fn : E->render_fn, E->T, E->S, R, E->flags));
+  const bool publish = E->overlap_ctas > 0 && !(E->flags & MP_FLAG_DEBUG_NO_OVERLAP) && E->S.x_world == 0;
+  State S = E->S;
+  S.render_seq = 0;
+  if (publish) {
+    E->render_seq = E->render_seq == 0xffffffffu ? 1u : E->render_seq + 1u;
+    S.render_seq = E->render_seq;
+    E->render_ctas += (uint32_t)blocks;
+  }
+  CUDA_TRY(cudaLaunchKernelEx(&cfg, gather ? E->render_gather_fn : E->render_fn, E->T, S, R, E->flags));
+  E->render_last = publish; E->render_stream = st;
   if (gather) {
     k_gather_raise<<<1, 32, 0, st>>>(E->d_g_flag_ptrs, E->g_world, E->g_rank, E->g_seq);
     ++E->launches;
@@ -832,7 +909,14 @@
     E->blob_hash = hsh;
   }
   int rc = build_tables(E, blob, blob_bytes);
-  if (rc == MP_OK) rc = build_plan(E);
+  if (rc == MP_OK && overlap_family(E->family)) {
+    const int step_cta = (int)(warp_scratch_bytes(E->T) * OVERLAP_WARPS + (E->family == MPB_FAMILY_CLEAN_UP ? clean_up_table_bytes(E->T) : 0));
+    const int limit = (int)prop.sharedMemPerMultiprocessor - 2 * (int)prop.reservedSharedMemPerBlock - kRenderStaticSmem - kStepStaticSmem - step_cta;
+    rc = build_plan(E, RENDER_MAX_THREADS / 32 - OVERLAP_WARPS, std::min(kRenderSmemLimit, limit));
+    if (rc != MP_OK) rc = build_plan(E, RENDER_MAX_THREADS / 32, kRenderSmemLimit);
+  } else if (rc == MP_OK) {
+    rc = build_plan(E, RENDER_MAX_THREADS / 32, kRenderSmemLimit);
+  }
   if (rc != MP_OK) { mp_destroy(E); return rc; }
   const Tables& T = E->T;
   State& S = E->S;
@@ -849,7 +933,7 @@
       (rc = E->alloc((B * P + B + B + std::max<size_t>(1, T.n_scalar) * B * P) * 8, &E->scalar_block)) ||
       (rc = E->alloc(B * P * E->R.player_bytes, &S.rgb)) || (rc = E->alloc(B * (size_t)E->R.world_bytes, &S.world_rgb)) ||
       (rc = E->alloc(B * (size_t)S.max_events * 3, &S.events)) || (rc = E->alloc(B, &S.n_events)) ||
-      (rc = E->alloc(B * P, &E->d_actions))) {
+      (rc = E->alloc(B * P, &E->d_actions)) || (rc = E->alloc(B, &S.consumed)) || (rc = E->alloc(1, &S.render_done))) {
     mp_destroy(E);
     return rc;
   }
@@ -914,6 +998,7 @@
     }
   }
   if (ce != cudaSuccess) { mp_destroy(E); return fail(MP_E_CUDA, "cudaFuncSetAttribute failed: %s", cudaGetErrorString(ce)); }
+  if ((rc = plan_overlap(E, prop))) { mp_destroy(E); return rc; }
   mp_buffers& bf = E->buffers;
   bf.num_envs = num_envs; bf.num_players = T.P; bf.rgb_h = E->R.view_h * 8; bf.rgb_w = E->R.view_w * 8;
   bf.world_h = T.H * 8; bf.world_w = T.W * 8; bf.num_actions = T.n_actions; bf.num_scalar_obs = T.n_scalar;
@@ -1275,10 +1360,11 @@
   return MP_OK;
 }
 
-int mp_debug_render_plan(mp_handle h, int32_t out[8]) {
+int mp_debug_render_plan(mp_handle h, int32_t out[10]) {
   if (!h || !out) return fail(MP_E_INVALID, "mp_debug_render_plan: null argument");
   const RenderPlan& R = h->R;
-  const int32_t v[8] = {R.n_teams, R.team_threads, R.wstrip_log2, R.smem_bytes, R.n_total, R.rec_stride, R.stage_bytes, R.grid_bytes};
+  const int32_t v[10] = {R.n_teams, R.team_threads, R.wstrip_log2, R.smem_bytes, R.n_total, R.rec_stride, R.stage_bytes, R.grid_bytes,
+                         h->overlap_ctas, h->overlap_warps};
   memcpy(out, v, sizeof v);
   return MP_OK;
 }
diff --git a/meltingpot_b200/csrc/render.cuh b/meltingpot_b200/csrc/render.cuh
--- a/meltingpot_b200/csrc/render.cuh
+++ b/meltingpot_b200/csrc/render.cuh
@@ -278,6 +278,7 @@
       else cell_pass<MP_MAX_LAYERS>(T, R, s_grid, s_rec, s_opaque, s_pair, gtid, gthreads, flags);
     }
     group_sync(bar_id, gthreads);
+    if (gtid == 0 && S.render_seq) asm volatile("st.relaxed.gpu.global.u32 [%0], %1;" ::"l"(S.consumed + b), "r"(S.render_seq) : "memory");
     if (gtid == 0 && it + 1 < n_iters && it + 1 != rounds) {
       const int nb = it + 1 < rounds ? b + n_streams : b + (int)gridDim.x;
       mbar_expect_tx(gbar, (uint32_t)R.grid_bytes);
@@ -365,5 +366,10 @@
     group_sync(bar_id, gthreads);
     if (gtid == 0) *next_ctr = 0;
   }
-  if (lane == 0) { if (GATHER) asm volatile("cp.async.bulk.wait_group 0;" ::: "memory"); else bulk_wait_read<0>(); }
-}
+  if (lane == 0) { if (GATHER || S.render_seq) asm volatile("cp.async.bulk.wait_group 0;" ::: "memory"); else bulk_wait_read<0>(); }
+  if (S.render_seq) {
+    if (lane == 0) asm volatile("fence.proxy.async.global;" ::: "memory");
+    __syncthreads();
+    if (tid == 0) asm volatile("red.release.gpu.global.add.u32 [%0], 1;" ::"l"(S.render_done) : "memory");
+  }
+}
diff --git a/meltingpot_b200/csrc/step_clean_up.cuh b/meltingpot_b200/csrc/step_clean_up.cuh
--- a/meltingpot_b200/csrc/step_clean_up.cuh
+++ b/meltingpot_b200/csrc/step_clean_up.cuh
@@ -16,9 +16,14 @@
   const uint8_t* flags;
   const uint8_t* solid;
   const int32_t* act_table;
+  const int32_t* apple_tab;
+  const int32_t* dirt_tab;
 };
 
-__host__ __device__ inline size_t clean_up_table_bytes(const Tables& T) { return scratch_round16((size_t)T.cells_pad * 6) + scratch_round16((size_t)T.n_actions * 16); }
+__host__ __device__ inline size_t clean_up_act_offset(const Tables& T) { return scratch_round16((size_t)T.cells_pad * 6); }
+__host__ __device__ inline size_t clean_up_apple_offset(const Tables& T) { return clean_up_act_offset(T) + scratch_round16((size_t)T.n_actions * 16); }
+__host__ __device__ inline size_t clean_up_dirt_offset(const Tables& T) { return clean_up_apple_offset(T) + scratch_round16((size_t)T.nA * 12); }
+__host__ __device__ inline size_t clean_up_table_bytes(const Tables& T) { return clean_up_dirt_offset(T) + scratch_round16((size_t)T.nD * 12); }
 
 __host__ __device__ inline size_t warp_scratch_bytes(const Tables& T) {
   size_t words = (size_t)(T.cells + 31) / 32 + 1;
@@ -95,9 +100,8 @@
   __syncwarp();
 }
 
-__device__ __forceinline__ void beam_scan(const BeamGeom& G, int lane, bool self_blocked, bool& vis) {
+__device__ __forceinline__ void beam_scan(const BeamGeom& G, int lane, int parent, bool self_blocked, bool& vis) {
   bool ok = lane < G.n;
-  int parent = ok ? G.parent[lane] : -1;
   vis = ok;
   bool open = ok && !self_blocked;
   for (int d = 0; d < G.depth; ++d) {
@@ -107,6 +111,9 @@
     if (ok && parent >= 0) { vis = pv && po; }
     open = vis && !self_blocked;
   }
+}
+__device__ __forceinline__ void beam_scan(const BeamGeom& G, int lane, bool self_blocked, bool& vis) {
+  beam_scan(G, lane, lane < G.n ? (int)G.parent[lane] : -1, self_blocked, vis);
 }
 
 __device__ void clean_up_step(const Tables& T, const State& S, int b, int lane, const int32_t* __restrict__ actions, WarpScratch& sc) {
@@ -189,7 +196,7 @@
     const double probability = T.grow_rate * interpolation;
     if (probability > 0.0) {
       for (int k = lane; k < T.nA; k += 32) {
-        uint4 w = philox4x32_10((uint32_t)n, (uint32_t)episode, (uint32_t)T.apple[k * 3], RS_OBJECT, k0, k1);
+        uint4 w = philox4x32_10((uint32_t)n, (uint32_t)episode, (uint32_t)sc.apple_tab[k * 3], RS_OBJECT, k0, k1);
         if (u01(w.x, w.y) < probability && !(sc.apple[k] & 1)) sc.apple[k] |= 4;
       }
     }
@@ -227,7 +234,7 @@
     int eater = -1;
     if (grows) {
       sc.apple[k] = (sc.apple[k] & ~4) | 1;
-      int o = sc.occ[T.apple[k * 3 + 1]];
+      int o = sc.occ[sc.apple_tab[k * 3 + 1]];
       if (o >= 1 && o <= T.P) { eater = o - 1; sc.apple[k] |= 2; }
     }
     unsigned m = __ballot_sync(MP_FULL, eater >= 0);
@@ -271,6 +278,7 @@
   unsigned zapped = 0;
   for (int pass = 0; pass < 2; ++pass) {
     const BeamGeom& G = pass == 0 ? T.zap_geom : T.clean_geom;
+    const int g_fwd = lane < G.n ? G.fwd[lane] : 0, g_lat = lane < G.n ? G.lat[lane] : 0, g_parent = lane < G.n ? G.parent[lane] : -1;
     for (int r = 0; r < T.P; ++r) {
       unsigned m = __ballot_sync(MP_FULL, is_av && rank == r && (pass == 0 ? fire_zap : fire_clean));
       if (!m) continue;
@@ -279,8 +287,8 @@
       int cell = -1; bool blocked = false; int hit_avatar = -1, hit_dirt = -1;
       if (lane < G.n) {
         int f = so, rgt = (so + 1) & 3;
-        int cx = sx + dir_dx(f) * G.fwd[lane] + dir_dx(rgt) * G.lat[lane];
-        int cy = sy + dir_dy(f) * G.fwd[lane] + dir_dy(rgt) * G.lat[lane];
+        int cx = sx + dir_dx(f) * g_fwd + dir_dx(rgt) * g_lat;
+        int cy = sy + dir_dy(f) * g_fwd + dir_dy(rgt) * g_lat;
         if (!wrap_or_reject(T, cx, cy)) { blocked = true; }
         else {
           cell = cy * T.W + cx;
@@ -296,7 +304,7 @@
         }
       }
       bool vis;
-      beam_scan(G, lane, blocked, vis);
+      beam_scan(G, lane, g_parent, blocked, vis);
       if (pass == 0) {
         unsigned hm = __ballot_sync(MP_FULL, vis && hit_avatar >= 0);
         while (hm) {
@@ -353,7 +361,7 @@
     uint8_t now = (v & 1) && !(v & 2);
     if (now != was) {
       S.apple[(size_t)b * T.nA_pad + k] = now;
-      grid[(size_t)T.apple_layer * T.cells_pad + T.apple[k * 3 + 1]] = now ? cell_value(T.apple_sprite, 0) : (uint16_t)0;
+      grid[(size_t)T.apple_layer * T.cells_pad + sc.apple_tab[k * 3 + 1]] = now ? cell_value(T.apple_sprite, 0) : (uint16_t)0;
     }
   }
   int d_delta = 0;
@@ -364,7 +372,7 @@
     if ((v & 1) && (v & 2)) --d_delta;
     if (now != was) {
       S.dirt[(size_t)b * T.nD_pad + j] = now;
-      grid[(size_t)T.dirt_layer * T.cells_pad + T.dirt[j * 3 + 1]] = now ? cell_value(T.dirt_sprite, 0) : (uint16_t)0;
+      grid[(size_t)T.dirt_layer * T.cells_pad + sc.dirt_tab[j * 3 + 1]] = now ? cell_value(T.dirt_sprite, 0) : (uint16_t)0;
     }
   }
   for (int o = 16; o > 0; o >>= 1) d_delta += __shfl_xor_sync(MP_FULL, d_delta, o);
@@ -412,23 +420,38 @@
   extern __shared__ __align__(128) uint8_t smem[];
   const int warp = threadIdx.x >> 5, lane = threadIdx.x & 31;
   asm volatile("griddepcontrol.launch_dependents;" ::: "memory");
-  int16_t* s_apple_of = reinterpret_cast<int16_t*>(smem + 4 * warp_scratch_bytes(T));
+  uint8_t* s_tables = smem + (blockDim.x >> 5) * warp_scratch_bytes(T);
+  int16_t* s_apple_of = reinterpret_cast<int16_t*>(s_tables);
   int16_t* s_dirt_of = s_apple_of + T.cells_pad;
   uint8_t* s_solid = reinterpret_cast<uint8_t*>(s_dirt_of + T.cells_pad);
   uint8_t* s_flags = s_solid + T.cells_pad;
-  int32_t* s_act = reinterpret_cast<int32_t*>(smem + 4 * warp_scratch_bytes(T) + scratch_round16((size_t)T.cells_pad * 6));
-  for (int i = threadIdx.x; i < T.cells_pad; i += (int)blockDim.x) { s_apple_of[i] = T.apple_of_cell[i]; s_dirt_of[i] = T.dirt_of_cell[i]; s_flags[i] = T.cell_flags[i]; s_solid[i] = T.solid[i]; }
-  for (int i = threadIdx.x; i < T.n_actions * 4; i += (int)blockDim.x) s_act[i] = T.action_table[i];
-  asm volatile("griddepcontrol.wait;" ::: "memory");
+  int32_t* s_act = reinterpret_cast<int32_t*>(s_tables + clean_up_act_offset(T));
+  {
+    const uint4* __restrict__ src = reinterpret_cast<const uint4*>(T.clean_up_tables);
+    uint4* dst = reinterpret_cast<uint4*>(s_tables);
+    const int n16 = (int)(clean_up_table_bytes(T) / 16), step = (int)blockDim.x;
+    for (int i = threadIdx.x; i < n16; i += 4 * step) {
+      uint4 v[4];
+#pragma unroll
+      for (int k = 0; k < 4; ++k) if (i + k * step < n16) v[k] = __ldg(src + i + k * step);
+#pragma unroll
+      for (int k = 0; k < 4; ++k) if (i + k * step < n16) dst[i + k * step] = v[k];
+    }
+  }
+  if (S.wait_seq == 0) asm volatile("griddepcontrol.wait;" ::: "memory");
   __syncthreads();
-  const int b = blockIdx.x * 4 + warp;
-  if (b >= S.B) return;
   WarpScratch sc = carve_scratch(T, smem + warp * warp_scratch_bytes(T));
   sc.apple_of = s_apple_of; sc.dirt_of = s_dirt_of; sc.flags = s_flags; sc.solid = s_solid; sc.act_table = s_act;
-  if (!(mode == 1 && !(mask == nullptr || mask[b]))) {
-    event_begin(lane);
-    if (mode == 1 || S.env[(size_t)b * ENV_COLS + ENV_DONE]) clean_up_reset(T, S, b, lane, sc);
-    else clean_up_step(T, S, b, lane, actions, sc);
-    event_end(S, b, lane);
-  }
-}
+  sc.apple_tab = reinterpret_cast<const int32_t*>(s_tables + clean_up_apple_offset(T));
+  sc.dirt_tab = reinterpret_cast<const int32_t*>(s_tables + clean_up_dirt_offset(T));
+  for (int i = 0;; ++i) {
+    const int b = step_env(S, i, warp);
+    if (b < 0) return;
+    if (!(mode == 1 && !(mask == nullptr || mask[b]))) {
+      event_begin(lane);
+      if (mode == 1 || S.env[(size_t)b * ENV_COLS + ENV_DONE]) clean_up_reset(T, S, b, lane, sc);
+      else clean_up_step(T, S, b, lane, actions, sc);
+      event_end(S, b, lane);
+    }
+  }
+}
diff --git a/meltingpot_b200/csrc/step_commons.cuh b/meltingpot_b200/csrc/step_commons.cuh
--- a/meltingpot_b200/csrc/step_commons.cuh
+++ b/meltingpot_b200/csrc/step_commons.cuh
@@ -316,14 +316,16 @@
   extern __shared__ __align__(128) uint8_t smem[];
   const int warp = threadIdx.x >> 5, lane = threadIdx.x & 31;
   asm volatile("griddepcontrol.launch_dependents;" ::: "memory");
-  asm volatile("griddepcontrol.wait;" ::: "memory");
-  const int b = blockIdx.x * 4 + warp;
-  if (b >= S.B) return;
+  if (S.wait_seq == 0) asm volatile("griddepcontrol.wait;" ::: "memory");
   WarpScratch sc = carve_scratch(T, smem + warp * warp_scratch_bytes(T));
-  if (!(mode == 1 && !(mask == nullptr || mask[b]))) {
-    event_begin(lane);
-    if (mode == 1 || S.env[(size_t)b * ENV_COLS + ENV_DONE]) commons_reset(T, S, b, lane, sc);
-    else commons_step(T, S, b, lane, actions, sc);
-    event_end(S, b, lane);
+  for (int i = 0;; ++i) {
+    const int b = step_env(S, i, warp);
+    if (b < 0) return;
+    if (!(mode == 1 && !(mask == nullptr || mask[b]))) {
+      event_begin(lane);
+      if (mode == 1 || S.env[(size_t)b * ENV_COLS + ENV_DONE]) commons_reset(T, S, b, lane, sc);
+      else commons_step(T, S, b, lane, actions, sc);
+      event_end(S, b, lane);
+    }
   }
 }
diff --git a/meltingpot_b200/engine.py b/meltingpot_b200/engine.py
--- a/meltingpot_b200/engine.py
+++ b/meltingpot_b200/engine.py
@@ -13,6 +13,7 @@
 MP_FLAG_RENDER_WORLD = 1
 MP_FLAG_RENDER_PLAYERS = 2
 MP_FLAG_DEFAULT = 3
+MP_FLAG_DEBUG_NO_OVERLAP = 1 << 11
 
 EXPORTED_SYMBOLS = (
     'mp_create', 'mp_destroy', 'mp_set_flags', 'mp_reset', 'mp_step',
@@ -397,10 +398,13 @@
     _check(self._lib.mp_state_load(self._h, buf, ctypes.c_uint64(len(snapshot)), self._stream(stream)))
 
   def render_plan(self):
-    out = (ctypes.c_int32 * 8)()
+    out = (ctypes.c_int32 * 10)()
     _check(self._lib.mp_debug_render_plan(self._h, out))
-    keys = ('teams', 'team_threads', 'wstrip_log2', 'smem_bytes', 'atlas_sprites', 'rec_stride', 'stage_bytes', 'grid_bytes')
-    return dict(zip(keys, (int(v) for v in out)))
+    keys = ('teams', 'team_threads', 'wstrip_log2', 'smem_bytes', 'atlas_sprites', 'rec_stride', 'stage_bytes', 'grid_bytes',
+            'overlap_ctas', 'overlap_warps')
+    plan = dict(zip(keys, (int(v) for v in out)))
+    plan['overlap'] = plan['overlap_ctas'] > 0
+    return plan
 
   def render_tables(self):
     import numpy as np
```
